# krispy-kenay/WebDGS

Measured on AMD Instinct MI355X. Metric: training iters/sec (fwd+bwd+Adam), 1M Gaussians @1080p SH3, higher is better.
Workload: dtype f32

## Files before the change

bindings/napi/webdgs_napi.cc:

```cpp
#include <node_api.h>

#include <cstdint>
#include <cstring>
#include <string>

#include "../../include/webdgs.h"

#define NAPI_OK(call)                                                         \
    do {                                                                      \
        if ((call) != napi_ok) {                                              \
            napi_throw_error(env, nullptr, "N-API call failed: " #call);      \
            return nullptr;                                                   \
        }                                                                     \
    } while (0)

static napi_value throw_wdgs(napi_env env, int code) {
    std::string msg = "[wdgs " + std::to_string(code) + "] " + wdgs_last_error();
    napi_throw_error(env, code == WDGS_E_CAPACITY ? "WDGS_E_CAPACITY" : (code == WDGS_E_STATE ? "WDGS_E_STATE" : "WDGS_E"), msg.c_str());
    return nullptr;
}
#define WDGS_OK_OR_THROW(expr)                      \
    do {                                            \
        int _rc = (expr);                           \
        if (_rc != WDGS_OK) return throw_wdgs(env, _rc); \
// ... 183 lines not shown
}
static napi_value tiledRasterizerDestroy(napi_env env, napi_callback_info info) { ARGS(1); wdgs_tiled_rasterizer_destroy((wdgs_tiled_rasterizer*)get_ptr(env, argv[0])); return js_undefined(env); }
static napi_value tiledBackwardCreate(napi_env env, napi_callback_info info) {
    ARGS(2);
    wdgs_tiled_backward_config c; std::memset(&c, 0, sizeof(c));
    c.num_points = (uint32_t)prop_f64(env, argv[1], "numPoints", 0);
    c.sh_deg = (uint32_t)prop_f64(env, argv[1], "shDeg", 0);
    c.viewport_width = (uint32_t)prop_f64(env, argv[1], "viewportWidth", 1);
    c.viewport_height = (uint32_t)prop_f64(env, argv[1], "viewportHeight", 1);
    c.training.lambda_l1 = (float)prop_f64(env, argv[1], "lambda_l1", 0.8);
    c.training.lambda_l2 = (float)prop_f64(env, argv[1], "lambda_l2", 0.0);
    c.training.lambda_dssim = (float)prop_f64(env, argv[1], "lambda_dssim", 0.2);
    c.training.c1 = (float)prop_f64(env, argv[1], "c1", 0.0001);
    c.training.c2 = (float)prop_f64(env, argv[1], "c2", 0.0009);
    c.max_splat_radius_px = (float)prop_f64(env, argv[1], "maxSplatRadiusPx", 128.0);
    uint32_t mode = 0;
    if (!prop_dssim_mode(env, argv[1], &mode)) return nullptr;
    wdgs_tiled_backward* op = nullptr;
    WDGS_OK_OR_THROW(wdgs_tiled_backward_create((wdgs_device*)get_ptr(env, argv[0]), &c, &op));
    const int r = wdgs_tiled_backward_set_dssim_mode(op, mode);
    if (r != WDGS_OK) { wdgs_tiled_backward_destroy(op); WDGS_OK_OR_THROW(r); }
    return make_ptr(env, op);
}
static napi_value tiledBackwardEncode(napi_env env, napi_callback_info info) {
    ARGS(5);
    wdgs_tiled_backward_resources r;
    r.splat_buffer = prop_ptr(env, argv[3], "splatBuffer");
    r.tile_offsets_buffer = prop_ptr(env, argv[3], "tileOffsetsBuffer");
    r.tile_indices_buffer = prop_ptr(env, argv[3], "tileIndicesBuffer");
    r.camera_buffer = prop_ptr(env, argv[3], "cameraBuffer");
    r.alpha_texture = prop_ptr(env, argv[3], "alphaTexture");
    r.n_contrib_texture = prop_ptr(env, argv[3], "nContribTexture");
    WDGS_OK_OR_THROW(wdgs_tiled_backward_encode((wdgs_tiled_backward*)get_ptr(env, argv[0]), get_ptr(env, argv[1]), get_ptr(env, argv[2]), &r, get_ptr(env, argv[4])));
    return js_undefined(env);
}
static napi_value tiledBackwardGradients(napi_env env, napi_callback_info info) { ARGS(1); return make_ptr(env, wdgs_tiled_backward_gradients((wdgs_tiled_backward*)get_ptr(env, argv[0]))); }
static napi_value tiledBackwardDestroy(napi_env env, napi_callback_info info) { ARGS(1); wdgs_tiled_backward_destroy((wdgs_tiled_backward*)get_ptr(env, argv[0])); return js_undefined(env); }
static napi_value optimizerCreate(napi_env env, napi_callback_info info) {
    ARGS(4);
    wdgs_optimizer* op = nullptr;
    WDGS_OK_OR_THROW(wdgs_optimizer_create((wdgs_device*)get_ptr(env, argv[0]), get_u32(env, argv[1]), nullptr, get_ptr(env, argv[2]), get_ptr(env, argv[3]), nullptr, 1, 0, &op));
    return make_ptr(env, op);
}
static napi_value optimizerStep(napi_env env, napi_callback_info info) {
    ARGS(5);
    WDGS_OK_OR_THROW(wdgs_optimizer_step((wdgs_optimizer*)get_ptr(env, argv[0]), get_ptr(env, argv[1]), get_ptr(env, argv[2]), get_ptr(env, argv[3]), get_ptr(env, argv[4])));
    return js_undefined(env);
}
static napi_value optimizerGetIteration(napi_env env, napi_callback_info info) { ARGS(1); return make_u32(env, wdgs_optimizer_get_iteration((wdgs_optimizer*)get_ptr(env, argv[0]))); }
static napi_value optimizerDestroy(napi_env env, napi_callback_info info) { ARGS(1); wdgs_optimizer_destroy((wdgs_optimizer*)get_ptr(env, argv[0])); return js_undefined(env); }

static napi_value tiledForwardSet(napi_env env, napi_callback_info info) {
    ARGS(3);
    wdgs_tiled_forward* op = (wdgs_tiled_forward*)get_ptr(env, argv[0]);
    switch (get_u32(env, argv[1])) {
        case 0: WDGS_OK_OR_THROW(wdgs_tiled_forward_set_render_mode(op, get_u32(env, argv[2]))); break;
        case 1: WDGS_OK_OR_THROW(wdgs_tiled_forward_set_point_size(op, (float)get_f64(env, argv[2]))); break;
        default: WDGS_OK_OR_THROW(wdgs_tiled_forward_set_gaussian_scale(op, (float)get_f64(env, argv[2]))); break;
    }
    return js_undefined(env);
}
static napi_value tiledForwardCheck(napi_env env, napi_callback_info info) {
    ARGS(1);
    uint32_t st[4] = {0, 0, 0, 0};
    WDGS_OK_OR_THROW(wdgs_tiled_forward_check((wdgs_tiled_forward*)get_ptr(env, argv[0]), st));
    napi_value o; napi_create_object(env, &o);
    set_prop(env, o, "totalTileEntries", make_u32(env, st[0]));
    set_prop(env, o, "visibleCount", make_u32(env, st[1]));
    return o;
}
static napi_value tiledForwardSetLongLists(napi_env env, napi_callback_info info) {
    ARGS(4);
    WDGS_OK_OR_THROW(wdgs_tiled_forward_set_long_lists((wdgs_tiled_forward*)get_ptr(env, argv[0]), get_u32(env, argv[1]), get_u32(env, argv[2]), get_u32(env, argv[3])));
    return js_undefined(env);
}
static napi_value tiledForwardLongListStats(napi_env env, napi_callback_info info) {
    ARGS(1);
    uint32_t st[12] = {0};
    WDGS_OK_OR_THROW(wdgs_tiled_forward_long_list_stats((wdgs_tiled_forward*)get_ptr(env, argv[0]), st));
    static const char* const keys[12] = {"blocksWanted", "itemsWanted", "forwardQueue", "backwardQueue", "rowsUsed", "rowsWanted", "stalled", nullptr, "maxItems", "maxBlocks", "maxRows", "threshold"};
    napi_value o; napi_create_object(env, &o);
    for (int i = 0; i < 12; i++) if (keys[i]) set_prop(env, o, keys[i], make_u32(env, st[i]));
    return o;
}
static napi_value tiledRasterizerBlit(napi_env env, napi_callback_info info) {
    ARGS(4);
    WDGS_OK_OR_THROW(wdgs_tiled_rasterizer_blit((wdgs_tiled_rasterizer*)get_ptr(env, argv[0]), get_ptr(env, argv[1]), get_u32(env, argv[2]), get_u32(env, argv[3])));
    return js_undefined(env);
}
static napi_value tiledRasterizerEncodeDepth(napi_env env, napi_callback_info info) {
    ARGS(2);
    WDGS_OK_OR_THROW(wdgs_tiled_rasterizer_encode_depth((wdgs_tiled_rasterizer*)get_ptr(env, argv[0]), get_u32(env, argv[1])));
    return js_undefined(env);
}
static napi_value tiledRasterizerGetDepth(napi_env env, napi_callback_info info) {
    ARGS(2);
    void* p = nullptr;
    WDGS_OK_OR_THROW(wdgs_tiled_rasterizer_get_depth((wdgs_tiled_rasterizer*)get_ptr(env, argv[0]), get_u32(env, argv[1]), &p));
    return make_ptr(env, p);
}
static napi_value depthToRgba8(napi_env env, napi_callback_info info) {
    ARGS(7);
    WDGS_OK_OR_THROW(wdgs_depth_to_rgba8((wdgs_device*)get_ptr(env, argv[0]), get_ptr(env, argv[1]), get_u32(env, argv[2]), get_u32(env, argv[3]), (float)get_f64(env, argv[4]),
                                         (float)get_f64(env, argv[5]), get_ptr(env, argv[6])));
    return js_undefined(env);
}
static napi_value bufferClear(napi_env env, napi_callback_info info) {
    ARGS(3);
    WDGS_OK_OR_THROW(wdgs_memset((wdgs_device*)get_ptr(env, argv[0]), get_ptr(env, argv[1]), 0, (size_t)get_f64(env, argv[2])));
    return js_undefined(env);
}
static napi_value encoderBegin(napi_env env, napi_callback_info info) { ARGS(1); WDGS_OK_OR_THROW(wdgs_encoder_begin((wdgs_device*)get_ptr(env, argv[0]))); return js_undefined(env); }
static napi_value encoderFinish(napi_env env, napi_callback_info info) {
    ARGS(1);
    wdgs_command_buffer* c = nullptr;
    WDGS_OK_OR_THROW(wdgs_encoder_finish((wdgs_device*)get_ptr(env, argv[0]), &c));
    return make_ptr(env, c);
}
static napi_value queueSubmit(napi_env env, napi_callback_info info) {
    ARGS(2);
    WDGS_OK_OR_THROW(wdgs_queue_submit((wdgs_device*)get_ptr(env, argv[0]), (wdgs_command_buffer*)get_ptr(env, argv[1])));
    return js_undefined(env);
}
static napi_value commandBufferDestroy(napi_env env, napi_callback_info info) { ARGS(1); wdgs_command_buffer_destroy((wdgs_command_buffer*)get_ptr(env, argv[0])); return js_undefined(env); }

struct DoneCtx { napi_deferred deferred; napi_threadsafe_function tsfn; };
static void done_call_js(napi_env env, napi_value, void* context, void*) {
    DoneCtx* c = static_cast<DoneCtx*>(context);
    if (env) { napi_value u; napi_get_undefined(env, &u); napi_resolve_deferred(env, c->deferred, u); }
    napi_release_threadsafe_function(c->tsfn, napi_tsfn_release);
    delete c;
}
static void done_from_runtime_thread(void* user) {
    DoneCtx* c = static_cast<DoneCtx*>(user);
    napi_call_threadsafe_function(c->tsfn, nullptr, napi_tsfn_blocking);
}
static napi_value queueOnSubmittedWorkDone(napi_env env, napi_callback_info info) {
    ARGS(1);
    DoneCtx* c = new DoneCtx();
    napi_value promise, name;
    NAPI_OK(napi_create_promise(env, &c->deferred, &promise));
    napi_create_string_utf8(env, "wdgs onSubmittedWorkDone", NAPI_AUTO_LENGTH, &name);
    NAPI_OK(napi_create_threadsafe_function(env, nullptr, nullptr, name, 0, 1, nullptr, nullptr, c, done_call_js, &c->tsfn));
    int rc = wdgs_queue_on_done((wdgs_device*)get_ptr(env, argv[0]), done_from_runtime_thread, c);
    if (rc != WDGS_OK) { napi_release_threadsafe_function(c->tsfn, napi_tsfn_abort); delete c; return throw_wdgs(env, rc); }
    return promise;
}

static void read_backward_resources(napi_env env, napi_value o, wdgs_tiled_backward_resources* r) {
    r->splat_buffer = prop_ptr(env, o, "splatBuffer");
    r->tile_offsets_buffer = prop_ptr(env, o, "tileOffsetsBuffer");
    r->tile_indices_buffer = prop_ptr(env, o, "tileIndicesBuffer");
    r->camera_buffer = prop_ptr(env, o, "cameraBuffer");
    r->alpha_texture = prop_ptr(env, o, "alphaTexture");
    r->n_contrib_texture = prop_ptr(env, o, "nContribTexture");
}
static napi_value tiledBackwardMetric(napi_env env, napi_callback_info info) {
    ARGS(5);
    wdgs_tiled_backward* op = (wdgs_tiled_backward*)get_ptr(env, argv[0]);
    switch (get_u32(env, argv[1])) {
        case 0: WDGS_OK_OR_THROW(wdgs_tiled_backward_compute_loss_only(op, get_ptr(env, argv[2]), get_ptr(env, argv[3]))); break;
        case 1: WDGS_OK_OR_THROW(wdgs_tiled_backward_compute_metric_map(op, get_ptr(env, argv[2]), get_ptr(env, argv[3]), (float)get_f64(env, argv[4]))); break;
        case 2: {
            wdgs_tiled_backward_resources r;
            read_backward_resources(env, argv[2], &r);
            WDGS_OK_OR_THROW(wdgs_tiled_backward_compute_metric_counts(op, &r, get_u32(env, argv[3]), (int)get_u32(env, argv[4])));
// ... 407 lines not shown
    uint32_t n = 0;
    napi_get_array_length(env, arr, &n);
    if (n > WDGS_MAX_BATCH_VIEWS) n = WDGS_MAX_BATCH_VIEWS + 1;
    for (uint32_t i = 0; i < n && i < WDGS_MAX_BATCH_VIEWS; i++) { napi_value v; napi_get_element(env, arr, i, &v); out[i] = get_ptr(env, v); }
    return n;
}
static napi_value tiledForwardProjectViews(napi_env env, napi_callback_info info) {
    ARGS(4);
    void* ops[WDGS_MAX_BATCH_VIEWS]; void* cams[WDGS_MAX_BATCH_VIEWS];
    const uint32_t n = read_ptr_array(env, argv[0], ops), m = read_ptr_array(env, argv[1], cams);
    if (n != m || n == 0 || n > WDGS_MAX_BATCH_VIEWS) { napi_throw_range_error(env, nullptr, "projectViews: 1..16 passes and as many cameras"); return nullptr; }
    WDGS_OK_OR_THROW(wdgs_tiled_forward_project_views((wdgs_tiled_forward* const*)ops, (const void* const*)cams, n, get_ptr(env, argv[2]), get_ptr(env, argv[3])));
    return js_undefined(env);
}
static napi_value tiledForwardEncodeProjected(napi_env env, napi_callback_info info) { ARGS(1); WDGS_OK_OR_THROW(wdgs_tiled_forward_encode_projected((wdgs_tiled_forward*)get_ptr(env, argv[0]))); return js_undefined(env); }
static napi_value tiledForwardIsProjected(napi_env env, napi_callback_info info) { ARGS(1); return make_u32(env, (uint32_t)wdgs_tiled_forward_is_projected((const wdgs_tiled_forward*)get_ptr(env, argv[0]))); }
static napi_value tiledBackwardGeometryViews(napi_env env, napi_callback_info info) {
    ARGS(10);
    void* ops[WDGS_MAX_BATCH_VIEWS]; void* cams[WDGS_MAX_BATCH_VIEWS]; void* counts[WDGS_MAX_BATCH_VIEWS]; void* words[WDGS_MAX_BATCH_VIEWS];
    const uint32_t n = read_ptr_array(env, argv[0], ops);
    if (n == 0 || n > WDGS_MAX_BATCH_VIEWS || read_ptr_array(env, argv[1], cams) != n || read_ptr_array(env, argv[2], counts) != n || read_ptr_array(env, argv[3], words) != n) {
        napi_throw_range_error(env, nullptr, "geometryViews: 1..16 passes and as many cameras, tile counts and overflow words");
        return nullptr;
    }
    WDGS_OK_OR_THROW(wdgs_tiled_backward_encode_geometry_views((wdgs_tiled_backward* const*)ops, (const void* const*)cams, (const void* const*)counts, (const void* const*)words, n,
                                                               get_ptr(env, argv[4]), get_ptr(env, argv[5]), get_ptr(env, argv[6]), get_ptr(env, argv[7]),
                                                               (int)get_u32(env, argv[8]), (int)get_u32(env, argv[9])));
    return js_undefined(env);
}
static napi_value deviceLaneMark(napi_env env, napi_callback_info info) {
    ARGS(3);
    WDGS_OK_OR_THROW(wdgs_device_lane_mark((wdgs_device*)get_ptr(env, argv[0]), (int)get_u32(env, argv[1]), (int)get_u32(env, argv[2])));
    return js_undefined(env);
}
static napi_value deviceLaneWaitMark(napi_env env, napi_callback_info info) {
    ARGS(3);
    WDGS_OK_OR_THROW(wdgs_device_lane_wait_mark((wdgs_device*)get_ptr(env, argv[0]), (int)get_u32(env, argv[1]), (int)get_u32(env, argv[2])));
    return js_undefined(env);
}
static napi_value deviceKernelTimes(napi_env env, napi_callback_info info) {
    ARGS(2);
    wdgs_device* d = (wdgs_device*)get_ptr(env, argv[0]);
    const uint32_t op = get_u32(env, argv[1]);
    if (op <= 1) { WDGS_OK_OR_THROW(wdgs_device_set_profiling(d, (int)op)); return js_undefined(env); }
    if (op == 2) { WDGS_OK_OR_THROW(wdgs_device_reset_kernel_times(d)); return js_undefined(env); }
    static wdgs_kernel_time recs[128];
    uint32_t n = 0;
    WDGS_OK_OR_THROW(wdgs_device_get_kernel_times(d, recs, 128, &n));
    napi_value o; napi_create_object(env, &o);
    for (uint32_t i = 0; i < n && i < 128; i++) {
        napi_value r, ms; napi_create_object(env, &r);
        set_prop(env, r, "launches", make_u32(env, recs[i].launches));
        napi_create_double(env, recs[i].total_ms, &ms); set_prop(env, r, "totalMs", ms);
        char name[49]; std::memcpy(name, recs[i].name, 48); name[48] = 0;
        set_prop(env, o, name, r);
    }
    return o;
}
static napi_value copyBufferToBuffer(napi_env env, napi_callback_info info) {
    ARGS(4);
    WDGS_OK_OR_THROW(wdgs_copy_buffer_to_buffer((wdgs_device*)get_ptr(env, argv[0]), get_ptr(env, argv[1]), get_ptr(env, argv[2]), (size_t)get_f64(env, argv[3])));
    return js_undefined(env);
}
static napi_value commGroup(napi_env env, napi_callback_info info) {
    ARGS(1);
    if (get_u32(env, argv[0])) WDGS_OK_OR_THROW(wdgs_comm_group_end()); else WDGS_OK_OR_THROW(wdgs_comm_group_start());
    return js_undefined(env);
}

#define EXPORT_FN(name)                                                              \
    do {                                                                             \
        napi_value fn;                                                               \
        napi_create_function(env, #name, NAPI_AUTO_LENGTH, name, nullptr, &fn);      \
        napi_set_named_property(env, exports, #name, fn);                            \
    } while (0)

static napi_value Init(napi_env env, napi_value exports) {
    EXPORT_FN(abiVersion); EXPORT_FN(deviceCreate); EXPORT_FN(deviceDestroy); EXPORT_FN(deviceSynchronize); EXPORT_FN(deviceMemoryInfo);
    EXPORT_FN(bufferCreate); EXPORT_FN(bufferDestroy); EXPORT_FN(copyToDevice); EXPORT_FN(copyToHost);
    EXPORT_FN(tiledForwardCreate); EXPORT_FN(tiledForwardEncode); EXPORT_FN(tiledForwardSetViewport); EXPORT_FN(tiledForwardGetResources); EXPORT_FN(tiledForwardDestroy);
    EXPORT_FN(tiledRasterizerCreate); EXPORT_FN(tiledRasterizerEncode); EXPORT_FN(tiledRasterizerGet); EXPORT_FN(tiledRasterizerDestroy);
    EXPORT_FN(tiledBackwardCreate); EXPORT_FN(tiledBackwardEncode); EXPORT_FN(tiledBackwardGradients); EXPORT_FN(tiledBackwardDestroy);
    EXPORT_FN(optimizerCreate); EXPORT_FN(optimizerStep); EXPORT_FN(optimizerGetIteration); EXPORT_FN(optimizerDestroy);
    EXPORT_FN(tiledForwardSet); EXPORT_FN(tiledForwardCheck); EXPORT_FN(tiledForwardSetLongLists); EXPORT_FN(tiledForwardLongListStats); EXPORT_FN(tiledRasterizerBlit); EXPORT_FN(bufferClear);
    EXPORT_FN(tiledRasterizerEncodeDepth); EXPORT_FN(tiledRasterizerGetDepth); EXPORT_FN(depthToRgba8);
    EXPORT_FN(encoderBegin); EXPORT_FN(encoderFinish); EXPORT_FN(queueSubmit); EXPORT_FN(commandBufferDestroy); EXPORT_FN(queueOnSubmittedWorkDone);
    EXPORT_FN(tiledBackwardMetric); EXPORT_FN(tiledBackwardGet); EXPORT_FN(downsampleRGBA8); EXPORT_FN(imageSSE); EXPORT_FN(imageSSIM);
    EXPORT_FN(optimizerStateSizes); EXPORT_FN(optimizerCreateWithState); EXPORT_FN(optimizerState); EXPORT_FN(optimizerHyperparameters);
    EXPORT_FN(optimizerAdvanceIteration); EXPORT_FN(optimizerStepF32); EXPORT_FN(accumulateGradients);
    EXPORT_FN(densifyCreate); EXPORT_FN(densifySetConfig); EXPORT_FN(densifyEncodePrepare); EXPORT_FN(densifyReadTotal); EXPORT_FN(densifyEncodeScatter);
    EXPORT_FN(densifyStage);
    EXPORT_FN(densifyDestroy);
    EXPORT_FN(commUniqueId); EXPORT_FN(commCreate); EXPORT_FN(commAllreduceGradients); EXPORT_FN(commAllreduceCounts); EXPORT_FN(commDestroy);
    EXPORT_FN(encoderAbort); EXPORT_FN(hostAlloc); EXPORT_FN(bufferReadAsync); EXPORT_FN(prefixScanner); EXPORT_FN(dynamicSorter);
    EXPORT_FN(optimizerDeferredSH); EXPORT_FN(optimizerFlushSH); EXPORT_FN(tiledForwardSetDcSource);
    EXPORT_FN(optimizerSetGuard); EXPORT_FN(optimizerStepF32Range); EXPORT_FN(optimizerStateChanged); EXPORT_FN(storeGradients); EXPORT_FN(guardAccumulate);
    EXPORT_FN(deviceSelectLane); EXPORT_FN(deviceLaneOrder); EXPORT_FN(queueMark); EXPORT_FN(queueWait); EXPORT_FN(tiledForwardResize); EXPORT_FN(tiledBackwardResize);
    EXPORT_FN(applyRepackedRows); EXPORT_FN(commExchangeGradients); EXPORT_FN(commAllgatherRows); EXPORT_FN(commBroadcast); EXPORT_FN(commInfo);
    EXPORT_FN(optimizerStepWithGeometry); EXPORT_FN(optimizerApplyRepackedRows); EXPORT_FN(tiledBackwardEncodeRaster); EXPORT_FN(tiledBackwardEncodeGeometry);
    EXPORT_FN(tiledBackwardSetGradientOutput); EXPORT_FN(tiledBackwardSetMetricCountsTarget); EXPORT_FN(tiledForwardProjectViews); EXPORT_FN(tiledForwardEncodeProjected); EXPORT_FN(tiledForwardIsProjected);
    EXPORT_FN(tiledBackwardGeometryViews); EXPORT_FN(deviceLaneMark); EXPORT_FN(deviceLaneWaitMark); EXPORT_FN(deviceKernelTimes); EXPORT_FN(commGroup); EXPORT_FN(copyBufferToBuffer);
    return exports;
}
NAPI_MODULE(webdgs_napi, Init)
```

include/webdgs.h:

```cpp
#ifndef WEBDGS_H
#define WEBDGS_H

#include <stddef.h>
#include <stdint.h>

#ifdef __cplusplus
extern "C" {
#endif

#define WDGS_OK 0
#define WDGS_E_INVALID (-1)
#define WDGS_E_HIP (-2)
#define WDGS_E_CAPACITY (-3)
#define WDGS_E_STATE (-4)

typedef struct wdgs_device wdgs_device;
typedef struct wdgs_buffer wdgs_buffer;
typedef struct wdgs_prefix_scanner wdgs_prefix_scanner;
typedef struct wdgs_sorter wdgs_sorter;
typedef struct wdgs_tiled_forward wdgs_tiled_forward;
typedef struct wdgs_tiled_rasterizer wdgs_tiled_rasterizer;
typedef struct wdgs_tiled_backward wdgs_tiled_backward;
typedef struct wdgs_optimizer wdgs_optimizer;
typedef struct wdgs_densify_prune wdgs_densify_prune;
// ... 20 lines not shown
int wdgs_device_lane_order(wdgs_device* dev, int waiter_lane, int signal_lane);
int wdgs_device_lane_mark(wdgs_device* dev, int lane, int mark);
int wdgs_device_lane_wait_mark(wdgs_device* dev, int lane, int mark);

int wdgs_encoder_begin(wdgs_device* dev);
int wdgs_encoder_finish(wdgs_device* dev, wdgs_command_buffer** out);
int wdgs_encoder_abort(wdgs_device* dev);
int wdgs_queue_submit(wdgs_device* dev, wdgs_command_buffer* cmd);
int wdgs_command_buffer_destroy(wdgs_command_buffer* cmd);
typedef void (*wdgs_done_callback)(void* user);
int wdgs_queue_on_done(wdgs_device* dev, wdgs_done_callback fn, void* user);
#define WDGS_TICKET_RING 8
int wdgs_queue_mark(wdgs_device* dev, uint64_t* ticket);
int wdgs_queue_wait(wdgs_device* dev, uint64_t ticket);

int wdgs_copy_to_host(wdgs_device* dev, void* dst_host, const void* src_dev, size_t bytes);
int wdgs_copy_to_device(wdgs_device* dev, void* dst_dev, const void* src_host, size_t bytes);
int wdgs_memset(wdgs_device* dev, void* dst_dev, int value, size_t bytes);
int wdgs_copy_buffer_to_buffer(wdgs_device* dev, void* dst_dev, const void* src_dev, size_t bytes);

int wdgs_buffer_create(wdgs_device* dev, size_t bytes, wdgs_buffer** out);
int wdgs_buffer_destroy(wdgs_buffer* buf);
void* wdgs_buffer_ptr(const wdgs_buffer* buf);
size_t wdgs_buffer_size(const wdgs_buffer* buf);
int wdgs_buffer_write(wdgs_device* dev, wdgs_buffer* buf, size_t offset, const void* src_host, size_t bytes);
int wdgs_buffer_read(wdgs_device* dev, const wdgs_buffer* buf, size_t offset, void* dst_host, size_t bytes);
int wdgs_buffer_read_async(wdgs_device* dev, const wdgs_buffer* buf, size_t offset, void* dst_host, size_t bytes);
int wdgs_host_alloc(size_t bytes, void** out_host);
int wdgs_host_free(void* host);

int wdgs_prefix_scanner_create(wdgs_device* dev, uint32_t max_elements, wdgs_prefix_scanner** out);
int wdgs_prefix_scanner_destroy(wdgs_prefix_scanner* s);
void* wdgs_prefix_scanner_input(wdgs_prefix_scanner* s);
void* wdgs_prefix_scanner_output(wdgs_prefix_scanner* s);
int wdgs_prefix_scanner_set_count(wdgs_prefix_scanner* s, uint32_t count);
int wdgs_prefix_scanner_scan(wdgs_prefix_scanner* s);
int wdgs_prefix_scanner_scan_ptr(wdgs_prefix_scanner* s, const void* in_dev, void* out_dev, uint32_t count);

int wdgs_sorter_create(wdgs_device* dev, uint32_t max_capacity, const void* stats_dev, wdgs_sorter** out);
int wdgs_sorter_destroy(wdgs_sorter* s);
void* wdgs_sorter_keys(wdgs_sorter* s, int ping_pong_index);
void* wdgs_sorter_values(wdgs_sorter* s, int ping_pong_index);
int wdgs_sorter_sort(wdgs_sorter* s, uint32_t key_bits);
int wdgs_sorter_final_out_index(wdgs_sorter* s);
uint32_t wdgs_sorter_capacity(wdgs_sorter* s);

typedef struct wdgs_tiled_forward_config {
    uint32_t num_points;
    uint32_t sh_deg;
    uint32_t viewport_width;
    uint32_t viewport_height;
    float gaussian_scale;
    float point_size_px;
    float max_splat_radius_px;
    uint32_t render_mode;
    uint32_t max_tile_entries;
    uint32_t compat_caps;
} wdgs_tiled_forward_config;

typedef struct wdgs_tiled_forward_resources {
    void* splat_buffer;
    void* depths_buffer;
    void* tile_keys_buffer;
    void* tile_indices_buffer;
    void* tile_offsets_buffer;
    void* tile_counts_buffer;
    void* stats_buffer;
    uint32_t num_tiles_x, num_tiles_y, total_tiles, max_tile_entries;
    float settings[7];
} wdgs_tiled_forward_resources;

int wdgs_tiled_forward_create(wdgs_device* dev, const wdgs_tiled_forward_config* cfg, wdgs_tiled_forward** out);
int wdgs_tiled_forward_destroy(wdgs_tiled_forward* op);
int wdgs_tiled_forward_resize(wdgs_tiled_forward* op, uint32_t num_points);
int wdgs_tiled_forward_encode(wdgs_tiled_forward* op, const void* gaussians_dev, const void* sh_dev, const void* camera_dev, int skip_sort);
int wdgs_tiled_forward_set_viewport(wdgs_tiled_forward* op, uint32_t width, uint32_t height);
int wdgs_tiled_forward_set_render_mode(wdgs_tiled_forward* op, uint32_t render_mode);
int wdgs_tiled_forward_set_point_size(wdgs_tiled_forward* op, float point_size_px);
int wdgs_tiled_forward_set_gaussian_scale(wdgs_tiled_forward* op, float scale);
int wdgs_tiled_forward_get_resources(wdgs_tiled_forward* op, wdgs_tiled_forward_resources* out);
int wdgs_tiled_forward_check(wdgs_tiled_forward* op, uint32_t* stats_out);
int wdgs_tiled_forward_set_long_lists(wdgs_tiled_forward* op, uint32_t threshold, uint32_t max_items, uint32_t max_rows);
int wdgs_tiled_forward_long_list_stats(wdgs_tiled_forward* op, uint32_t stats_out[12]);

int wdgs_tiled_rasterizer_create(wdgs_device* dev, wdgs_tiled_forward* forward, uint32_t compat_caps, wdgs_tiled_rasterizer** out);
int wdgs_tiled_rasterizer_destroy(wdgs_tiled_rasterizer* op);
int wdgs_tiled_rasterizer_encode(wdgs_tiled_rasterizer* op, uint32_t width, uint32_t height);
int wdgs_tiled_rasterizer_get_output(wdgs_tiled_rasterizer* op, void** rgba8_dev);
int wdgs_tiled_rasterizer_get_alpha(wdgs_tiled_rasterizer* op, void** final_t_dev);
int wdgs_tiled_rasterizer_get_n_contrib(wdgs_tiled_rasterizer* op, void** n_contrib_dev);
int wdgs_tiled_rasterizer_get_tile_offsets(wdgs_tiled_rasterizer* op, void** ranges_dev);
int wdgs_tiled_rasterizer_blit(wdgs_tiled_rasterizer* op, void* target_rgba8_dev, uint32_t target_width, uint32_t target_height);

#define WDGS_DEPTH_EXPECTED   1u
#define WDGS_DEPTH_MEDIAN     2u
#define WDGS_DEPTH_WEIGHT_SUM 4u
int wdgs_tiled_rasterizer_encode_depth(wdgs_tiled_rasterizer* op, uint32_t kinds);
int wdgs_tiled_rasterizer_get_depth(wdgs_tiled_rasterizer* op, uint32_t kind, void** f32_dev);
int wdgs_depth_to_rgba8(wdgs_device* dev, const void* depth_f32_dev, uint32_t width, uint32_t height, float near_z, float far_z, void* rgba8_dev);

typedef struct wdgs_training_config {
    float lambda_l1, lambda_l2, lambda_dssim, c1, c2;
} wdgs_training_config;
typedef struct wdgs_tiled_backward_config {
    uint32_t num_points;
    uint32_t sh_deg;
    uint32_t viewport_width, viewport_height;
    wdgs_training_config training;
    float gaussian_scale, point_size_px, max_splat_radius_px;
} wdgs_tiled_backward_config;
typedef struct wdgs_tiled_backward_resources {
    const void* splat_buffer;
    const void* tile_offsets_buffer;
    const void* tile_indices_buffer;
    const void* camera_buffer;
    const void* alpha_texture;
    const void* n_contrib_texture;
} wdgs_tiled_backward_resources;

int wdgs_tiled_backward_create(wdgs_device* dev, const wdgs_tiled_backward_config* cfg, wdgs_tiled_backward** out);
int wdgs_tiled_backward_resize(wdgs_tiled_backward* op, uint32_t num_points);
int wdgs_tiled_backward_destroy(wdgs_tiled_backward* op);
int wdgs_tiled_backward_encode(wdgs_tiled_backward* op, const void* predicted_rgba8_dev, const void* target_rgba8_dev,
                               const wdgs_tiled_backward_resources* res, const void* gaussians_dev);
typedef struct wdgs_view_accumulate {
    void* sums;
    void* visible;
    const void* tile_counts;
    void* guard;
    const void* overflow_word;
    int first;
} wdgs_view_accumulate;
int wdgs_tiled_backward_encode_raster(wdgs_tiled_backward* op, const void* predicted_rgba8_dev, const void* target_rgba8_dev,
                                      const wdgs_tiled_backward_resources* res);
int wdgs_tiled_backward_encode_geometry(wdgs_tiled_backward* op, const void* camera_dev, const void* gaussians_dev, const wdgs_view_accumulate* into);
int wdgs_tiled_backward_compute_loss_only(wdgs_tiled_backward* op, const void* predicted_rgba8_dev, const void* target_rgba8_dev);
int wdgs_tiled_backward_compute_metric_map(wdgs_tiled_backward* op, const void* predicted_rgba8_dev, const void* target_rgba8_dev, float threshold);
int wdgs_tiled_backward_compute_metric_counts(wdgs_tiled_backward* op, const wdgs_tiled_backward_resources* res, uint32_t num_instances, int clear);
int wdgs_tiled_backward_normalize_metric_counts(wdgs_tiled_backward* op, uint32_t divisor);
int wdgs_tiled_backward_set_viewport(wdgs_tiled_backward* op, uint32_t width, uint32_t height);
int wdgs_tiled_backward_set_training_config(wdgs_tiled_backward* op, const wdgs_training_config* cfg);
#define WDGS_DSSIM_REFERENCE 0
#define WDGS_DSSIM_GAUSSIAN 1
int wdgs_tiled_backward_set_dssim_mode(wdgs_tiled_backward* op, uint32_t mode);
int wdgs_tiled_backward_get_dssim_mode(const wdgs_tiled_backward* op, uint32_t* out);
void* wdgs_tiled_backward_gradients(wdgs_tiled_backward* op);
void* wdgs_tiled_backward_metric_counts(wdgs_tiled_backward* op);
int wdgs_tiled_backward_set_metric_counts_target(wdgs_tiled_backward* op, void* counts_dev);
void* wdgs_tiled_backward_loss_image(wdgs_tiled_backward* op);
void* wdgs_tiled_backward_metric_map(wdgs_tiled_backward* op);
int wdgs_tiled_backward_set_gradient_output(wdgs_tiled_backward* op, int enabled);
void* wdgs_tiled_backward_accumulators(wdgs_tiled_backward* op);
void* wdgs_tiled_backward_metric_minmax(wdgs_tiled_backward* op);
int wdgs_downsample_rgba8(wdgs_device* dev, const void* src_dev, uint32_t src_w, uint32_t src_h, void* dst_dev, uint32_t dst_w, uint32_t dst_h);

int wdgs_image_sse_rgb8(wdgs_device* dev, const void* a_rgba8_dev, const void* b_rgba8_dev, uint32_t num_pixels, void* out_u64_dev);

int wdgs_image_ssim_rgb8(wdgs_device* dev, const void* a_rgba8_dev, const void* b_rgba8_dev, uint32_t width, uint32_t height, void* out_f64_dev,
                         void* map_f32_dev);

int wdgs_debug_eval_math(wdgs_device* dev, uint32_t which, uint32_t count, const void* in_u32_dev, void* out_u32_dev);

int wdgs_debug_sort_tiles(wdgs_sorter* s, uint32_t route, uint32_t num_tiles_x, uint32_t num_tiles_y, void* ranges_u32_dev);

typedef struct wdgs_adam_hyperparameters {
    float lr_pos, lr_color, lr_opacity, lr_scale, lr_rot, beta1, beta2, epsilon;
// ... 103 lines not shown
```

webdgs_amd/_lib.py:

```python
from __future__ import annotations

import ctypes as C
import os

_HERE = os.path.dirname(os.path.abspath(__file__))
LIB_PATH = os.environ.get("WDGS_LIB_PATH") or os.path.join(_HERE, "lib", "libwebdgs_hip.so")

WDGS_OK, WDGS_E_INVALID, WDGS_E_HIP, WDGS_E_CAPACITY, WDGS_E_STATE = 0, -1, -2, -3, -4


class WdgsError(RuntimeError):

    def __init__(self, code: int, message: str):
        super().__init__(f"[wdgs {code}] {message}")
        self.code = code


class CapacityError(WdgsError):
    pass


class StateError(WdgsError):
    pass

# ... 77 lines not shown
    "wdgs_device_lane_order": (_I, [_P, _I, _I]),
    "wdgs_device_lane_mark": (_I, [_P, _I, _I]),
    "wdgs_device_lane_wait_mark": (_I, [_P, _I, _I]),
    "wdgs_encoder_begin": (_I, [_P]),
    "wdgs_encoder_finish": (_I, [_P, C.POINTER(_P)]),
    "wdgs_encoder_abort": (_I, [_P]),
    "wdgs_queue_submit": (_I, [_P, _P]),
    "wdgs_command_buffer_destroy": (_I, [_P]),
    "wdgs_queue_on_done": (_I, [_P, DoneCallback, _P]),
    "wdgs_buffer_read_async": (_I, [_P, _P, _Z, _P, _Z]),
    "wdgs_host_alloc": (_I, [_Z, C.POINTER(_P)]),
    "wdgs_host_free": (_I, [_P]),
    "wdgs_tiled_rasterizer_blit": (_I, [_P, _P, _U, _U]),
    "wdgs_densify_prune_encode_decision": (_I, [_P, _U, _P, _P]),
    "wdgs_densify_prune_encode_prefix_sum": (_I, [_P, _U]),
    "wdgs_densify_prune_encode_cap_to_max": (_I, [_P, _U, _U]),
    "wdgs_densify_prune_encode_total_out": (_I, [_P, _U]),
    "wdgs_densify_prune_compute_max_out_points": (_I, [_P, _U, C.POINTER(_U)]),
    "wdgs_densify_prune_get_buffers": (_I, [_P, C.POINTER(DensifyPrepared)]),
    "wdgs_debug_eval_math": (_I, [_P, _U, _U, _P, _P]),
    "wdgs_debug_sort_tiles": (_I, [_P, _U, _U, _U, _P]),
    "wdgs_comm_get_unique_id": (_I, [C.POINTER(C.c_uint8)]),
    "wdgs_comm_create": (_I, [_P, C.POINTER(C.c_uint8), _I, _I, C.POINTER(_P)]),
    "wdgs_comm_destroy": (_I, [_P]),
    "wdgs_comm_world_size": (_I, [_P]),
    "wdgs_comm_rank": (_I, [_P]),
    "wdgs_comm_allreduce_gradients": (_I, [_P, _P, _P, _U]),
    "wdgs_comm_allreduce_counts": (_I, [_P, _P, _U]),
    "wdgs_comm_exchange_gradients": (_I, [_P, _P, _P, _P, _U]),
    "wdgs_comm_allgather_rows": (_I, [_P, _P, _U]),
    "wdgs_comm_broadcast": (_I, [_P, _P, _Z, _I]),
    "wdgs_comm_group_start": (_I, []),
    "wdgs_comm_group_end": (_I, []),
    "wdgs_optimizer_step_f32_range": (_I, [_P, _P, _P, _P, _P, _U, _U, _P]),
    "wdgs_apply_repacked_rows": (_I, [_P, _U, _P, _U, _U, _P, _P, _P]),
    "wdgs_optimizer_set_guard": (_I, [_P, _P]),
    "wdgs_optimizer_set_deferred_sh": (_I, [_P, _P, _I]),
    "wdgs_optimizer_dc_words": (_P, [_P]),
    "wdgs_optimizer_flush_sh": (_I, [_P, _P]),
    "wdgs_optimizer_apply_repacked_rows": (_I, [_P, _P, _U, _U, _P, _P, _P]),
    "wdgs_tiled_forward_set_dc_source": (_I, [_P, _P]),
    "wdgs_tiled_forward_project_views": (_I, [_P, _P, _U, _P, _P]),
    "wdgs_tiled_forward_encode_projected": (_I, [_P]),
    "wdgs_tiled_forward_is_projected": (_I, [_P]),
    "wdgs_tiled_backward_encode_geometry_views": (_I, [_P, _P, _P, _P, _U, _P, _P, _P, _P, _I, _I]),
    "wdgs_guard_accumulate": (_I, [_P, _P, _P, _I]),
    "wdgs_optimizer_state_changed": (_I, [_P]),
    "wdgs_copy_to_host": (_I, [_P, _P, _P, _Z]),
    "wdgs_copy_to_device": (_I, [_P, _P, _P, _Z]),
    "wdgs_memset": (_I, [_P, _P, _I, _Z]),
    "wdgs_copy_buffer_to_buffer": (_I, [_P, _P, _P, _Z]),
    "wdgs_buffer_create": (_I, [_P, _Z, C.POINTER(_P)]),
    "wdgs_buffer_destroy": (_I, [_P]),
    "wdgs_buffer_ptr": (_P, [_P]),
    "wdgs_buffer_size": (_Z, [_P]),
    "wdgs_buffer_write": (_I, [_P, _P, _Z, _P, _Z]),
    "wdgs_buffer_read": (_I, [_P, _P, _Z, _P, _Z]),
    "wdgs_prefix_scanner_create": (_I, [_P, _U, C.POINTER(_P)]),
    "wdgs_prefix_scanner_destroy": (_I, [_P]),
    "wdgs_prefix_scanner_input": (_P, [_P]),
    "wdgs_prefix_scanner_output": (_P, [_P]),
    "wdgs_prefix_scanner_set_count": (_I, [_P, _U]),
    "wdgs_prefix_scanner_scan": (_I, [_P]),
    "wdgs_prefix_scanner_scan_ptr": (_I, [_P, _P, _P, _U]),
    "wdgs_sorter_create": (_I, [_P, _U, _P, C.POINTER(_P)]),
    "wdgs_sorter_destroy": (_I, [_P]),
    "wdgs_sorter_keys": (_P, [_P, _I]),
    "wdgs_sorter_values": (_P, [_P, _I]),
    "wdgs_sorter_sort": (_I, [_P, _U]),
    "wdgs_sorter_final_out_index": (_I, [_P]),
    "wdgs_sorter_capacity": (_U, [_P]),
    "wdgs_tiled_forward_create": (_I, [_P, C.POINTER(TiledForwardConfig), C.POINTER(_P)]),
    "wdgs_tiled_forward_destroy": (_I, [_P]),
    "wdgs_tiled_forward_resize": (_I, [_P, _U]),
    "wdgs_tiled_forward_encode": (_I, [_P, _P, _P, _P, _I]),
    "wdgs_tiled_forward_set_viewport": (_I, [_P, _U, _U]),
    "wdgs_tiled_forward_set_render_mode": (_I, [_P, _U]),
    "wdgs_tiled_forward_set_point_size": (_I, [_P, _F]),
    "wdgs_tiled_forward_set_gaussian_scale": (_I, [_P, _F]),
    "wdgs_tiled_forward_get_resources": (_I, [_P, C.POINTER(TiledForwardResources)]),
    "wdgs_tiled_forward_check": (_I, [_P, C.POINTER(_U)]),
    "wdgs_tiled_forward_set_long_lists": (_I, [_P, _U, _U, _U]),
    "wdgs_tiled_forward_long_list_stats": (_I, [_P, C.POINTER(_U)]),
    "wdgs_tiled_rasterizer_create": (_I, [_P, _P, _U, C.POINTER(_P)]),
    "wdgs_tiled_rasterizer_destroy": (_I, [_P]),
    "wdgs_tiled_rasterizer_encode": (_I, [_P, _U, _U]),
    "wdgs_tiled_rasterizer_get_output": (_I, [_P, C.POINTER(_P)]),
    "wdgs_tiled_rasterizer_get_alpha": (_I, [_P, C.POINTER(_P)]),
    "wdgs_tiled_rasterizer_get_n_contrib": (_I, [_P, C.POINTER(_P)]),
    "wdgs_tiled_rasterizer_get_tile_offsets": (_I, [_P, C.POINTER(_P)]),
    "wdgs_tiled_rasterizer_encode_depth": (_I, [_P, _U]),
    "wdgs_tiled_rasterizer_get_depth": (_I, [_P, _U, C.POINTER(_P)]),
    "wdgs_depth_to_rgba8": (_I, [_P, _P, _U, _U, _F, _F, _P]),
    "wdgs_tiled_backward_create": (_I, [_P, C.POINTER(TiledBackwardConfig), C.POINTER(_P)]),
    "wdgs_tiled_backward_resize": (_I, [_P, _U]),
    "wdgs_tiled_backward_destroy": (_I, [_P]),
    "wdgs_tiled_backward_encode": (_I, [_P, _P, _P, C.POINTER(TiledBackwardResources), _P]),
    "wdgs_tiled_backward_encode_raster": (_I, [_P, _P, _P, C.POINTER(TiledBackwardResources)]),
    "wdgs_tiled_backward_encode_geometry": (_I, [_P, _P, _P, C.POINTER(ViewAccumulate)]),
    "wdgs_tiled_backward_compute_loss_only": (_I, [_P, _P, _P]),
    "wdgs_tiled_backward_compute_metric_map": (_I, [_P, _P, _P, _F]),
    "wdgs_tiled_backward_compute_metric_counts": (_I, [_P, C.POINTER(TiledBackwardResources), _U, _I]),
    "wdgs_tiled_backward_normalize_metric_counts": (_I, [_P, _U]),
    "wdgs_tiled_backward_set_viewport": (_I, [_P, _U, _U]),
    "wdgs_tiled_backward_set_training_config": (_I, [_P, C.POINTER(TrainingConfig)]),
    "wdgs_tiled_backward_set_dssim_mode": (_I, [_P, _U]),
    "wdgs_tiled_backward_get_dssim_mode": (_I, [_P, C.POINTER(_U)]),
    "wdgs_tiled_backward_gradients": (_P, [_P]),
    "wdgs_tiled_backward_metric_counts": (_P, [_P]),
    "wdgs_tiled_backward_set_metric_counts_target": (_I, [_P, _P]),
    "wdgs_tiled_backward_loss_image": (_P, [_P]),
    "wdgs_tiled_backward_metric_map": (_P, [_P]),
    "wdgs_tiled_backward_accumulators": (_P, [_P]),
    "wdgs_tiled_backward_set_gradient_output": (_I, [_P, _I]),
    "wdgs_tiled_backward_metric_minmax": (_P, [_P]),
    "wdgs_downsample_rgba8": (_I, [_P, _P, _U, _U, _P, _U, _U]),
    "wdgs_image_sse_rgb8": (_I, [_P, _P, _P, _U, _P]),
    "wdgs_image_ssim_rgb8": (_I, [_P, _P, _P, _U, _U, _P, _P]),
    "wdgs_optimizer_state_sizes": (_I, [_U, C.POINTER(_Z * 6)]),
    "wdgs_optimizer_create": (_I, [_P, _U, C.POINTER(AdamHyperparameters), _P, _P, C.POINTER(OptimizerState), _I, _U, C.POINTER(_P)]),
    "wdgs_optimizer_destroy": (_I, [_P]),
    "wdgs_optimizer_init_from_point_cloud": (_I, [_P, _P, _P]),
    "wdgs_optimizer_step": (_I, [_P, _P, _P, _P, _P]),
    "wdgs_optimizer_step_with_geometry": (_I, [_P, _P, _P, _P, _P, _P]),
    "wdgs_optimizer_step_f32": (_I, [_P, _P, _P, _P, _P]),
    "wdgs_accumulate_gradients": (_I, [_P, _U, _P, _P, _P, _P]),
    "wdgs_store_gradients": (_I, [_P, _U, _P, _P, _P, _P]),
    "wdgs_optimizer_get_iteration": (_U, [_P]),
    "wdgs_optimizer_advance_iteration": (_I, [_P, _U]),
    "wdgs_optimizer_get_hyperparameters": (_I, [_P, C.POINTER(AdamHyperparameters)]),
    "wdgs_optimizer_set_hyperparameters": (_I, [_P, C.POINTER(AdamHyperparameters)]),
    "wdgs_optimizer_get_state": (_I, [_P, C.POINTER(OptimizerState)]),
    "wdgs_optimizer_release_state": (_I, [_P, C.POINTER(OptimizerState)]),
    "wdgs_densify_prune_create": (_I, [_P, C.POINTER(DensifyConfig), C.POINTER(_P)]),
    "wdgs_densify_prune_destroy": (_I, [_P]),
    "wdgs_densify_prune_set_config": (_I, [_P, C.POINTER(DensifyConfig)]),
    "wdgs_densify_prune_ensure_size": (_I, [_P, _U]),
    "wdgs_densify_prune_encode_prepare": (_I, [_P, _U, _P, _P, C.POINTER(DensifyPrepared)]),
    "wdgs_densify_prune_read_total": (_I, [_P, C.POINTER(_U)]),
    "wdgs_densify_prune_encode_scatter": (_I, [_P, _U, _P, _P, C.POINTER(OptimizerState), _U, _I, _P, _P, C.POINTER(OptimizerState)]),
}

_lib = None


def load() -> C.CDLL:
    global _lib
    if _lib is not None:
        return _lib
    if not os.path.exists(LIB_PATH):
        raise ImportError(f"{LIB_PATH} is missing: build it with `python -c 'import __graft_entry__ as g; g.build()'` "
                          "or `make -C webdgs_amd/csrc` (hipcc --offload-arch=gfx950). There is no CPU fallback.")
    lib = C.CDLL(LIB_PATH)
    for name, (res, args) in SIGNATURES.items():
        fn = getattr(lib, name)
        fn.restype = res
        fn.argtypes = args
    _lib = lib
    return lib


def check(code: int) -> None:
    if code == WDGS_OK:
        return
    msg = load().wdgs_last_error().decode("utf-8", "replace")
    if code == WDGS_E_CAPACITY:
# ... 5 lines not shown
```

webdgs_amd/csrc/api.hip:

```cpp
#include <cstdarg>
#include <cstdio>
#include <cstdlib>
#include <cstring>
#include <algorithm>
#include <mutex>
#include <map>
#include <set>
#include <unordered_map>
#include <vector>

#include "common.h"
#include "alloc_cache.h"
#include "longlist.h"

int launch_project_count(wdgs_device*, u32, const void*, const void*, const void*, const RenderSettings&, const TileInfo&, void*, void*, void*, void*, void*, void*,
                         const void*, void*, const void*);
int launch_emit_scatter(wdgs_device*, u32, const void*, const void*, const void*, void*, const void*, const RenderSettings&, const TileInfo&, const void*, const void*, void*, void*, u32);
int sorter_sort_rows(wdgs_sorter* s, u32 num_tiles_x, u32 num_tiles_y, u32* ranges, const LongWork* lw);
extern "C" void sorter_set_final_out_index(wdgs_sorter* s, int i);
int launch_update_stats(wdgs_device*, u32, const void*, const void*, u32, void*, void*, void*);
int launch_emit(wdgs_device*, u32, const void*, const void*, const void*, void*, const void*, const RenderSettings&, const TileInfo&, void*, void*, u32);
int launch_tile_ranges(wdgs_device*, const void*, const void*, u32, void*);
int launch_depth_composite(wdgs_device*, const RenderSettings&, const TileInfo&, const void*, u32, const void*, const void*, const void*, const void*, const void*, u32,
                           void*, void*, void*, const void*, const void*);
// ... 62 lines not shown
        if (cur != device && hipSetDevice(device) != hipSuccess) return nullptr;
        void* p = nullptr;
        const hipError_t e = hipMalloc(&p, bytes);
        if (cur != device) (void)hipSetDevice(cur);
        if (e != hipSuccess) { (void)hipGetLastError(); return nullptr; }
        return p;
    }
    void free(void* p) { (void)hipFree(p); }
    bool sync(int device) {
        int cur = 0;
        if (hipGetDevice(&cur) != hipSuccess) return false;
        if (cur != device && hipSetDevice(device) != hipSuccess) return false;
        const hipError_t e = hipDeviceSynchronize();
        if (cur != device) (void)hipSetDevice(cur);
        return e == hipSuccess;
    }
};
wdgs::AllocCache<HipBackend> g_alloc_cache;
size_t g_cache_limit = 0;
std::mutex g_cache_limit_mutex;
bool alloc_cache_enabled() {
    static const bool on = !(std::getenv("WDGS_ALLOC_CACHE") && std::getenv("WDGS_ALLOC_CACHE")[0] == '0');
    return on;
}
}

int wdgs_alloc(void** p, size_t bytes, bool zero, hipStream_t stream) {
    *p = nullptr;
    if (bytes == 0) bytes = 16;
    if (!alloc_cache_enabled()) {
        WDGS_CHECK_HIP(hipMalloc(p, bytes));
    } else {
        int device = 0;
        WDGS_CHECK_HIP(hipGetDevice(&device));
        hipStreamCaptureStatus capture = hipStreamCaptureStatusNone;
        const bool recording = stream && hipStreamIsCapturing(stream, &capture) == hipSuccess && capture != hipStreamCaptureStatusNone;
        *p = g_alloc_cache.alloc(device, bytes, !recording);
        WDGS_REQUIRE(*p, WDGS_E_HIP, "device allocation of %zu bytes failed (device %d)", bytes, device);
    }
    if (zero) WDGS_CHECK_HIP(hipMemsetAsync(*p, 0, bytes, stream));
    return WDGS_OK;
}

void wdgs_free(void* p) {
    if (!p) return;
    if (alloc_cache_enabled()) {
        size_t limit;
        {
            std::lock_guard<std::mutex> lock(g_cache_limit_mutex);
            if (g_cache_limit == 0) {
                size_t free_b = 0, total_b = 0;
                g_cache_limit = (hipMemGetInfo(&free_b, &total_b) == hipSuccess && total_b) ? total_b / 4 : ((size_t)8 << 30);
            }
            limit = g_cache_limit;
        }
        if (g_alloc_cache.free(p, limit)) return;
    }
    (void)hipFree(p);
}
static void free_dev(void* p) { wdgs_free(p); }

struct wdgs_buffer {
    void* ptr;
    size_t size;
};

struct wdgs_prefix_scanner {
    wdgs_device* dev;
    u32 max_elements, count;
    u32 *input, *output;
    ScanScratch scratch;
};

struct wdgs_tiled_forward {
    wdgs_device* dev;
    wdgs_tiled_forward_config cfg;
    RenderSettings settings;
    TileInfo tile_info;
    u32* stats;
    u32* nf_stamp;
    u32 nf_capacity;
    LongWork long_lists;
    u32 long_flags_capacity;
    u32* host_stats;
    u32* splats;
    u32* depths;
    u32* block_counts;
    u32* column_counts;
    u32* column_totals;
    const void* dc_source;
    u32 points_capacity;
    wdgs_prefix_scanner* scanner;
    wdgs_sorter* sorter;
    u32* ranges;
    u32 ranges_capacity;
    bool ranges_valid;
    bool encoded;
    bool projected;
    bool projected_columns;
};

constexpr u32 FRAME_WORD = 4u + 64u;
constexpr size_t FORWARD_STATS_BYTES = 16 + 64 * 4 + 16;

struct wdgs_tiled_rasterizer {
    wdgs_device* dev;
    wdgs_tiled_forward* fwd;
    u32 compat_caps;
    u32 width, height;
    u32 ranges_capacity;
    u32* ranges;
    u32* ranges_used;
    u32* rgba8;
    float* alpha;
    u32* n_contrib;
    bool encoded;
    float* depth[3];
    u32 depth_width, depth_height;
    u32 depth_encoded;
};

struct wdgs_tiled_backward {
    wdgs_device* dev;
    wdgs_tiled_backward_config cfg;
    RenderSettings settings;
    int* acc;
    u32* acc_dirty;
    u32* gradients;
    bool gradient_output;
    float* loss_image;
    u32 dssim_mode;
    u32* metric_counts;
    u32* metric_counts_into;
    u32* metric_err;
    u32* metric_flags;
    u32* metric_minmax;
    u32 img_capacity;
    u32 points_capacity;
};

struct wdgs_optimizer {
    wdgs_device* dev;
    u32 num_points;
    wdgs_adam_hyperparameters params;
    wdgs_optimizer_state state;
    bool owns_state;
    u32 iteration;
    float* dc;
    static u32 cs_pitch(u32 n) { return (std::max(n, 1u) + 15u) & ~15u; }
    CsView cs() const { return CsView{reinterpret_cast<float4*>(dc), cs_pitch(num_points)}; }
    bool dc_dirty;
    const void* guard;
    u32* dc_words;
    bool deferred_sh;
    bool sh_stale;
};

static int optimizer_flush_dc(wdgs_optimizer* op) {
    if (!op->dc_dirty) return WDGS_OK;
    WDGS_TRY(launch_cs_flush(op->dev, op->num_points, op->cs(), op->state));
    op->dc_dirty = false;
    return WDGS_OK;
}

extern "C" {

// ... 137 lines not shown
}

int wdgs_queue_wait(wdgs_device* d, uint64_t ticket) {
    WDGS_REQUIRE(d, WDGS_E_INVALID, "wdgs_queue_wait: null device");
    WDGS_REQUIRE(ticket != 0 && ticket < d->ticket_next, WDGS_E_INVALID, "wdgs_queue_wait: ticket %llu was never issued", (unsigned long long)ticket);
    WDGS_REQUIRE(!d->capturing, WDGS_E_STATE, "wdgs_queue_wait while recording a command buffer");
    WDGS_CHECK_HIP(hipEventSynchronize(d->ticket_events[ticket % WDGS_TICKET_RING]));
    if (!d->pending.empty()) collect_profile(d);
    return deferred_checks(d);
}

int wdgs_device_memory_info(wdgs_device* d, size_t* free_bytes, size_t* total_bytes, size_t* cached_bytes) {
    WDGS_REQUIRE(d, WDGS_E_INVALID, "wdgs_device_memory_info: null device");
    size_t f = 0, t = 0;
    WDGS_CHECK_HIP(hipSetDevice(d->ordinal));
    WDGS_CHECK_HIP(hipMemGetInfo(&f, &t));
    if (free_bytes) *free_bytes = f;
    if (total_bytes) *total_bytes = t;
    if (cached_bytes) *cached_bytes = g_alloc_cache.held(d->ordinal);
    return WDGS_OK;
}
static void reap_command_buffers(wdgs_device* d, size_t at_most);
int wdgs_device_destroy(wdgs_device* d) {
    if (!d) return WDGS_OK;
    {
        std::lock_guard<std::mutex> lock(g_live_mutex);
        if (!g_live_devices.erase(d)) return WDGS_OK;
    }
    (void)hipSetDevice(d->ordinal);
    if (d->capturing) {
        hipGraph_t g = nullptr;
        (void)hipStreamEndCapture(d->stream, &g);
        if (g) (void)hipGraphDestroy(g);
        d->capturing = false;
    }
    (void)wdgs_sync_lanes(d);
    collect_profile(d);
    reap_command_buffers(d, (size_t)-1);
    g_alloc_cache.release(d->ordinal);
    for (hipEvent_t e : d->event_pool) (void)hipEventDestroy(e);
    for (hipEvent_t e : d->lane_events) if (e) (void)hipEventDestroy(e);
    for (hipEvent_t e : d->lane_marks) if (e) (void)hipEventDestroy(e);
    for (hipEvent_t e : d->ticket_events) if (e) (void)hipEventDestroy(e);
    if (d->host_guard) (void)hipHostFree(d->host_guard);
    if (d->ssim_partials) (void)hipFree(d->ssim_partials);
    for (int l = 1; l < WDGS_MAX_LANES; l++)
        if (d->lanes[l]) (void)hipStreamDestroy(d->lanes[l]);
    if (d->own_stream) (void)hipStreamDestroy(d->lanes[0]);
    delete d;
    return WDGS_OK;
}

int wdgs_device_set_profiling(wdgs_device* d, int enabled) {
    WDGS_REQUIRE(d, WDGS_E_INVALID, "null device");
    d->profiling = enabled != 0;
    return WDGS_OK;
}

int wdgs_device_get_kernel_times(wdgs_device* d, wdgs_kernel_time* out, uint32_t cap, uint32_t* count) {
    WDGS_REQUIRE(d && count, WDGS_E_INVALID, "null argument");
    if (!d->pending.empty() && !d->capturing) collect_profile(d);
    u32 i = 0;
    for (auto& kv : d->totals) {
        if (out && i < cap) {
            std::memset(&out[i], 0, sizeof(out[i]));
            std::strncpy(out[i].name, kv.first.c_str(), sizeof(out[i].name) - 1);
            out[i].launches = kv.second.launches;
            out[i].total_ms = kv.second.ms;
        }
        i++;
    }
    *count = i;
    return WDGS_OK;
}

int wdgs_device_reset_kernel_times(wdgs_device* d) {
    WDGS_REQUIRE(d, WDGS_E_INVALID, "null device");
    d->totals.clear();
    return WDGS_OK;
}

static bool forward_holds_projection(const wdgs_tiled_forward* f);
static void forward_consume_projection(wdgs_tiled_forward* f);
struct wdgs_command_buffer_impl { hipGraph_t graph; hipGraphExec_t exec; std::vector<wdgs_tiled_forward*> consumes; wdgs_device* dev; };
static void command_buffer_release(wdgs_command_buffer_impl* c) {
    (void)hipGraphExecDestroy(c->exec);
    (void)hipGraphDestroy(c->graph);
    delete c;
}
static void reap_command_buffers(wdgs_device* d, size_t at_most) {
    while (at_most-- && !d->dead_command_buffers.empty()) {
        command_buffer_release(static_cast<wdgs_command_buffer_impl*>(d->dead_command_buffers.back()));
        d->dead_command_buffers.pop_back();
    }
}

int wdgs_encoder_begin(wdgs_device* d) {
    WDGS_REQUIRE(d, WDGS_E_INVALID, "null device");
    WDGS_REQUIRE(!d->capturing, WDGS_E_STATE, "wdgs_encoder_begin: a recording is already open on this device");
    WDGS_CHECK_HIP(hipStreamBeginCapture(d->stream, hipStreamCaptureModeRelaxed));
    d->capturing = true;
    d->capture_consumes.clear();
    return WDGS_OK;
}
int wdgs_encoder_finish(wdgs_device* d, wdgs_command_buffer** out) {
    WDGS_REQUIRE(d && out, WDGS_E_INVALID, "null argument");
    WDGS_REQUIRE(d->capturing, WDGS_E_STATE, "wdgs_encoder_finish without wdgs_encoder_begin");
    d->capturing = false;
    hipGraph_t graph = nullptr;
    WDGS_CHECK_HIP(hipStreamEndCapture(d->stream, &graph));
    hipGraphExec_t exec = nullptr;
    hipError_t e = hipGraphInstantiate(&exec, graph, nullptr, nullptr, 0);
    if (e != hipSuccess) { (void)hipGraphDestroy(graph); d->capture_consumes.clear(); wdgs_set_error("hipGraphInstantiate failed: %s", hipGetErrorString(e)); return WDGS_E_HIP; }
    auto* c = new wdgs_command_buffer_impl{graph, exec, std::move(d->capture_consumes), d};
    d->capture_consumes.clear();
    *out = reinterpret_cast<wdgs_command_buffer*>(c);
    return WDGS_OK;
}
int wdgs_encoder_abort(wdgs_device* d) {
    WDGS_REQUIRE(d, WDGS_E_INVALID, "null device");
    if (!d->capturing) return WDGS_OK;
    d->capturing = false;
    d->capture_consumes.clear();
    hipGraph_t graph = nullptr;
    const hipError_t e = hipStreamEndCapture(d->stream, &graph);
    if (graph) (void)hipGraphDestroy(graph);
    (void)hipGetLastError();
    (void)e;
    return WDGS_OK;
}
int wdgs_queue_submit(wdgs_device* d, wdgs_command_buffer* cmd) {
    WDGS_REQUIRE(d && cmd, WDGS_E_INVALID, "null argument");
    WDGS_REQUIRE(!d->capturing, WDGS_E_STATE, "wdgs_queue_submit while recording");
    auto* c = reinterpret_cast<wdgs_command_buffer_impl*>(cmd);
    for (wdgs_tiled_forward* f : c->consumes) {
        WDGS_REQUIRE(std::find(d->forwards.begin(), d->forwards.end(), f) != d->forwards.end(), WDGS_E_STATE,
                     "wdgs_queue_submit: the command buffer was recorded against a forward pass that has been destroyed");
        WDGS_REQUIRE(forward_holds_projection(f), WDGS_E_STATE,
                     "wdgs_queue_submit: the command buffer starts at the scan of a projected forward pass (wdgs_tiled_forward_encode_projected), but the pass holds no "
                     "projection: run wdgs_tiled_forward_project_views before every submit, and no other encode of the pass in between");
    }
    WDGS_CHECK_HIP(hipGraphLaunch(c->exec, d->stream));
    for (wdgs_tiled_forward* f : c->consumes) forward_consume_projection(f);
    reap_command_buffers(d, 1);
    return WDGS_OK;
}
namespace {
struct DoneThunk { wdgs_done_callback fn; void* user; };
void done_trampoline(void* p) {
    DoneThunk* t = static_cast<DoneThunk*>(p);
    t->fn(t->user);
    delete t;
}
}
int wdgs_queue_on_done(wdgs_device* d, wdgs_done_callback fn, void* user) {
    WDGS_REQUIRE(d && fn, WDGS_E_INVALID, "wdgs_queue_on_done: null argument");
    WDGS_REQUIRE(!d->capturing, WDGS_E_STATE, "wdgs_queue_on_done while recording a command buffer");
    DoneThunk* t = new DoneThunk{fn, user};
    hipError_t e = hipLaunchHostFunc(d->stream, done_trampoline, t);
    if (e != hipSuccess) { delete t; wdgs_set_error("hipLaunchHostFunc failed: %s", hipGetErrorString(e)); return WDGS_E_HIP; }
    return WDGS_OK;
}
int wdgs_command_buffer_destroy(wdgs_command_buffer* cmd) {
    if (!cmd) return WDGS_OK;
    auto* c = reinterpret_cast<wdgs_command_buffer_impl*>(cmd);
    static const bool lazy = !(std::getenv("WDGS_LAZY_GRAPH_DESTROY") && std::getenv("WDGS_LAZY_GRAPH_DESTROY")[0] == '0');
    if (lazy && wdgs_device_alive(c->dev)) {
        c->dev->dead_command_buffers.push_back(c);
        if (c->dev->dead_command_buffers.size() > 64u) reap_command_buffers(c->dev, 32u);
    } else command_buffer_release(c);
    return WDGS_OK;
}

int wdgs_copy_to_host(wdgs_device* d, void* dst, const void* src, size_t bytes) {
    WDGS_REQUIRE(d && (bytes == 0 || (dst && src)), WDGS_E_INVALID, "wdgs_copy_to_host: null argument");
    WDGS_REQUIRE(!d->capturing, WDGS_E_STATE, "wdgs_copy_to_host while recording a command buffer");
    if (bytes == 0) return WDGS_OK;
    WDGS_CHECK_HIP(hipMemcpyAsync(dst, src, bytes, hipMemcpyDeviceToHost, d->stream));
    WDGS_CHECK_HIP(wdgs_sync_lanes(d));
    return WDGS_OK;
}

int wdgs_copy_to_device(wdgs_device* d, void* dst, const void* src, size_t bytes) {
    WDGS_REQUIRE(d && (bytes == 0 || (dst && src)), WDGS_E_INVALID, "wdgs_copy_to_device: null argument");
    WDGS_REQUIRE(!d->capturing, WDGS_E_STATE, "wdgs_copy_to_device while recording a command buffer");
    if (bytes == 0) return WDGS_OK;
    WDGS_CHECK_HIP(hipMemcpyAsync(dst, src, bytes, hipMemcpyHostToDevice, d->stream));
    return WDGS_OK;
}

int wdgs_memset(wdgs_device* d, void* dst, int value, size_t bytes) {
    WDGS_REQUIRE(d && (bytes == 0 || dst), WDGS_E_INVALID, "wdgs_memset: null argument");
    if (bytes == 0) return WDGS_OK;
    WDGS_CHECK_HIP(hipMemsetAsync(dst, value, bytes, d->stream));
    return WDGS_OK;
}

int wdgs_copy_buffer_to_buffer(wdgs_device* d, void* dst, const void* src, size_t bytes) {
    WDGS_REQUIRE(d && (bytes == 0 || (dst && src)), WDGS_E_INVALID, "wdgs_copy_buffer_to_buffer: null argument");
    if (bytes == 0) return WDGS_OK;
    WDGS_CHECK_HIP(hipMemcpyAsync(dst, src, bytes, hipMemcpyDeviceToDevice, d->stream));
    return WDGS_OK;
}

int wdgs_buffer_create(wdgs_device* d, size_t bytes, wdgs_buffer** out) {
    WDGS_REQUIRE(d && out, WDGS_E_INVALID, "wdgs_buffer_create: null argument");
    wdgs_buffer* b = new wdgs_buffer{nullptr, bytes};
    int r = wdgs_alloc(&b->ptr, bytes, true, d->stream);
    if (r != WDGS_OK) { delete b; return r; }
    *out = b;
    return WDGS_OK;
}
int wdgs_buffer_destroy(wdgs_buffer* b) {
    if (!b) return WDGS_OK;
    free_dev(b->ptr);
    delete b;
    return WDGS_OK;
}
void* wdgs_buffer_ptr(const wdgs_buffer* b) { return b ? b->ptr : nullptr; }
size_t wdgs_buffer_size(const wdgs_buffer* b) { return b ? b->size : 0; }
int wdgs_buffer_write(wdgs_device* d, wdgs_buffer* b, size_t off, const void* src, size_t bytes) {
    WDGS_REQUIRE(d && b, WDGS_E_INVALID, "wdgs_buffer_write: null argument");
    WDGS_REQUIRE(off + bytes <= b->size, WDGS_E_INVALID, "wdgs_buffer_write: range [%zu, %zu) exceeds buffer size %zu", off, off + bytes, b->size);
    return wdgs_copy_to_device(d, (char*)b->ptr + off, src, bytes);
// ... 24 lines not shown
int wdgs_prefix_scanner_create(wdgs_device* d, uint32_t max_elements, wdgs_prefix_scanner** out) {
    WDGS_REQUIRE(d && out, WDGS_E_INVALID, "wdgs_prefix_scanner_create: null argument");
    wdgs_prefix_scanner* s = new wdgs_prefix_scanner();
    s->dev = d;
    s->max_elements = max_elements > 0 ? max_elements : 1;
    s->count = s->max_elements;
    s->input = s->output = nullptr;
    int r = wdgs_alloc((void**)&s->input, sizeof(u32) * (size_t)s->max_elements, true, d->stream);
    if (r == WDGS_OK) r = wdgs_alloc((void**)&s->output, sizeof(u32) * (size_t)s->max_elements, true, d->stream);
    if (r == WDGS_OK) r = scan_scratch_create(&s->scratch, s->max_elements);
    if (r != WDGS_OK) { wdgs_prefix_scanner_destroy(s); return r; }
    *out = s;
    return WDGS_OK;
}
int wdgs_prefix_scanner_destroy(wdgs_prefix_scanner* s) {
    if (!s) return WDGS_OK;
    free_dev(s->input);
    free_dev(s->output);
    scan_scratch_destroy(&s->scratch);
    delete s;
    return WDGS_OK;
}
void* wdgs_prefix_scanner_input(wdgs_prefix_scanner* s) { return s ? s->input : nullptr; }
void* wdgs_prefix_scanner_output(wdgs_prefix_scanner* s) { return s ? s->output : nullptr; }
int wdgs_prefix_scanner_set_count(wdgs_prefix_scanner* s, uint32_t count) {
    WDGS_REQUIRE(s, WDGS_E_INVALID, "null scanner");
    WDGS_REQUIRE(count <= s->max_elements, WDGS_E_CAPACITY, "scan count %u exceeds max_elements %u", count, s->max_elements);
    s->count = count;
    return WDGS_OK;
}
int wdgs_prefix_scanner_scan(wdgs_prefix_scanner* s) {
    WDGS_REQUIRE(s, WDGS_E_INVALID, "null scanner");
    return scan_exclusive_u32(s->dev, &s->scratch, s->input, s->output, s->count, nullptr);
}
int wdgs_prefix_scanner_scan_ptr(wdgs_prefix_scanner* s, const void* in, void* out, uint32_t count) {
    WDGS_REQUIRE(s && in && out, WDGS_E_INVALID, "null argument");
    WDGS_REQUIRE(count <= s->max_elements, WDGS_E_CAPACITY, "scan count %u exceeds max_elements %u", count, s->max_elements);
    return scan_exclusive_u32(s->dev, &s->scratch, (const u32*)in, (u32*)out, count, nullptr);
}

static uint64_t forward_tile_entry_cap(const wdgs_tiled_forward_config& cfg, u32 n) {
    uint64_t cap;
    if (cfg.compat_caps) {
        uint64_t base = std::min<uint64_t>((uint64_t)n * 30, (uint64_t)n * 2048);
        cap = std::min<uint64_t>(std::min<uint64_t>(base, 32ull * 1024 * 1024), 2097152ull);
        cap = (cap + 3839) / 3840 * 3840;
    } else if (cfg.max_tile_entries) {
        cap = cfg.max_tile_entries;
    } else {
        cap = std::max<uint64_t>((uint64_t)n * 30, 1ull << 20);
    }
    return std::min<uint64_t>(align_up(cap, 4096), 0xFFFFF000ull);
}
static int forward_alloc_per_point(wdgs_tiled_forward* op, u32 capacity) {
    wdgs_device* d = op->dev;
    int r = wdgs_alloc((void**)&op->splats, (size_t)24 * capacity, true, d->stream);
    if (r == WDGS_OK) r = wdgs_alloc((void**)&op->depths, (size_t)4 * capacity, true, d->stream);
    if (r == WDGS_OK) r = wdgs_alloc((void**)&op->block_counts, (size_t)4 * (ceil_div(capacity, 256) + 1), true, d->stream);
    if (r == WDGS_OK) r = wdgs_alloc((void**)&op->column_counts, (size_t)4 * 256 * (ceil_div(capacity, 256) + 1), true, d->stream);
    if (r == WDGS_OK && !op->column_totals) r = wdgs_alloc((void**)&op->column_totals, (size_t)4 * 256, true, d->stream);
    if (r == WDGS_OK) r = wdgs_prefix_scanner_create(d, capacity, &op->scanner);
    if (r == WDGS_OK) op->points_capacity = capacity;
    return r;
}
static void forward_set_viewport(wdgs_tiled_forward* op, u32 w, u32 h) {
    op->cfg.viewport_width = w;
    op->cfg.viewport_height = h;
    op->settings.viewport_x = (float)w;
    op->settings.viewport_y = (float)h;
    op->tile_info.num_tiles_x = ceil_div(w, 16);
    op->tile_info.num_tiles_y = ceil_div(h, 16);
    op->tile_info.total_tiles = op->tile_info.num_tiles_x * op->tile_info.num_tiles_y;
}
static int forward_alloc_nf_stamp(wdgs_tiled_forward* op) {
    if (op->tile_info.total_tiles <= op->nf_capacity) return WDGS_OK;
    free_dev(op->nf_stamp);
    op->nf_stamp = nullptr;
    op->nf_capacity = 0;
    WDGS_TRY(wdgs_alloc((void**)&op->nf_stamp, sizeof(u32) * (size_t)op->tile_info.total_tiles, true, op->dev->stream));
    op->nf_capacity = op->tile_info.total_tiles;
    return WDGS_OK;
}

static void forward_free_long_lists(wdgs_tiled_forward* op) {
    LongWork& lw = op->long_lists;
    free_dev(lw.hdr);
    free_dev(lw.flags);
    lw = LongWork{};
    op->long_flags_capacity = 0;
}
static int forward_alloc_long_lists(wdgs_tiled_forward* op, u32 threshold, u32 items, u32 rows) {
    wdgs_device* d = op->dev;
    forward_free_long_lists(op);
    if (threshold == 0u) return WDGS_OK;
    LongWork lw{};
    lw.threshold = threshold;
    lw.max_items = std::max(items, 64u);
    lw.max_blocks = std::max(lw.max_items / 8u, 16u) & ~3u;
    lw.max_rows = std::max(rows, 64u);
    const u32 tiles = std::max(op->tile_info.total_tiles, 1u);
    const size_t I = lw.max_items, B = lw.max_blocks, R = lw.max_rows;
    const size_t sizes[12] = {256, sizeof(LongBlock) * B, sizeof(LongSync) * B, sizeof(u32) * I, sizeof(u32) * I, sizeof(u32) * 64 * B, sizeof(u32) * 64 * B,
                              sizeof(u32) * 64 * I, sizeof(u32) * 64 * I, sizeof(float4) * 192 * I, sizeof(u32) * 256 * R, 0};
    size_t at[12], total = 0, zeroed = 0;
    for (int i = 0; i < 11; i++) { at[i] = total; total += align_up(sizes[i], 256); if (i == 6) zeroed = total; }
    char* base = nullptr;
    WDGS_TRY(wdgs_alloc((void**)&base, total, false, d->stream));
    if (hipMemsetAsync(base, 0, zeroed, d->stream) != hipSuccess) { free_dev(base); wdgs_set_error("hipMemsetAsync failed"); return WDGS_E_HIP; }
    lw.hdr = (u32*)(base + at[0]); lw.blocks = (LongBlock*)(base + at[1]); lw.sync = (LongSync*)(base + at[2]); lw.item_block = (u32*)(base + at[3]); lw.nlist = (u32*)(base + at[4]);
    lw.total = (u32*)(base + at[5]); lw.jlast = (u32*)(base + at[6]); lw.cnt = (u32*)(base + at[7]); lw.off = (u32*)(base + at[8]); lw.records = (float4*)(base + at[9]);
    lw.rows = (u32*)(base + at[10]);
    lw.nf_stamp = op->nf_stamp;
    lw.nf_frame = op->stats + FRAME_WORD;
    op->long_lists = lw;
    const int r = wdgs_alloc((void**)&op->long_lists.flags, sizeof(u32) * (size_t)tiles, true, d->stream);
    if (r != WDGS_OK) { forward_free_long_lists(op); return r; }
    op->long_flags_capacity = tiles;
    return WDGS_OK;
}
constexpr u32 LONG_LIST_THRESHOLD = 2048u, LONG_LIST_ITEMS = 1024u, LONG_LIST_ROWS = 8192u;

int wdgs_tiled_forward_create(wdgs_device* d, const wdgs_tiled_forward_config* cfg, wdgs_tiled_forward** out) {
    WDGS_REQUIRE(d && cfg && out, WDGS_E_INVALID, "wdgs_tiled_forward_create: null argument");
    WDGS_REQUIRE(cfg->viewport_width > 0 && cfg->viewport_height > 0, WDGS_E_INVALID, "viewport must be non-empty");
    WDGS_REQUIRE(cfg->sh_deg <= 3, WDGS_E_INVALID, "sh_deg %u > 3", cfg->sh_deg);
    const uint64_t tiles = (uint64_t)ceil_div(cfg->viewport_width, 16) * ceil_div(cfg->viewport_height, 16);
    WDGS_REQUIRE(tiles + 1 <= 0xFFFFu, WDGS_E_CAPACITY, "%llu tiles do not fit the 16-bit tile field of the sort key", (unsigned long long)tiles);
    wdgs_tiled_forward* op = new wdgs_tiled_forward();
    op->dev = d;
    op->cfg = *cfg;
    op->stats = op->splats = op->depths = op->block_counts = op->column_counts = op->column_totals = nullptr;
    op->dc_source = nullptr;
    op->nf_stamp = nullptr;
    op->nf_capacity = 0;
    op->long_lists = LongWork{};
    op->long_flags_capacity = 0;
    op->host_stats = nullptr;
    op->scanner = nullptr;
    op->sorter = nullptr;
    op->ranges = nullptr;
    op->ranges_capacity = 0;
    op->ranges_valid = false;
    op->encoded = false;
    op->projected = op->projected_columns = false;
    const u32 n = cfg->num_points;
    const uint64_t cap = forward_tile_entry_cap(*cfg, n);
    op->points_capacity = std::max(n, 1u);
    op->settings = RenderSettings{cfg->gaussian_scale != 0.f ? cfg->gaussian_scale : 1.0f, (float)cfg->sh_deg, 0.f, 0.f,
                                  cfg->point_size_px != 0.f ? cfg->point_size_px : 3.0f, cfg->render_mode ? 1.0f : 0.0f,
                                  cfg->max_splat_radius_px != 0.f ? cfg->max_splat_radius_px : 128.0f};
    op->tile_info.max_tile_entries = (u32)cap;
    forward_set_viewport(op, cfg->viewport_width, cfg->viewport_height);
    int r = wdgs_alloc((void**)&op->stats, FORWARD_STATS_BYTES, true, d->stream);
    if (r == WDGS_OK && hipMemsetD32Async((hipDeviceptr_t)(op->stats + FRAME_WORD), 1, 1, d->stream) != hipSuccess) { wdgs_set_error("hipMemsetD32Async failed"); r = WDGS_E_HIP; }
    if (r == WDGS_OK) r = forward_alloc_nf_stamp(op);
    if (r == WDGS_OK && !cfg->compat_caps) r = forward_alloc_long_lists(op, LONG_LIST_THRESHOLD, LONG_LIST_ITEMS, LONG_LIST_ROWS);
    if (r == WDGS_OK && hipHostMalloc((void**)&op->host_stats, 16, hipHostMallocDefault) != hipSuccess) { wdgs_set_error("hipHostMalloc(16) failed"); r = WDGS_E_HIP; }
    if (r == WDGS_OK) std::memset(op->host_stats, 0, 16);
    if (r == WDGS_OK) r = forward_alloc_per_point(op, std::max(n, 1u));
    if (r == WDGS_OK) r = wdgs_sorter_create(d, (u32)cap, op->stats, &op->sorter);
    if (r != WDGS_OK) { wdgs_tiled_forward_destroy(op); return r; }
    d->forwards.push_back(op);
    *out = op;
    return WDGS_OK;
}

int wdgs_tiled_forward_destroy(wdgs_tiled_forward* op) {
    if (!op) return WDGS_OK;
    if (wdgs_device_alive(op->dev)) {
        auto& v = op->dev->forwards;
        v.erase(std::remove(v.begin(), v.end(), op), v.end());
    }
    sync_if_alive(op->dev);
    if (op->ranges && wdgs_device_alive(op->dev)) op->dev->range_tables.erase(op->ranges);
    free_dev(op->stats);
    free_dev(op->nf_stamp);
    forward_free_long_lists(op);
    if (op->host_stats) (void)hipHostFree(op->host_stats);
    free_dev(op->splats);
    free_dev(op->depths);
    free_dev(op->block_counts);
    free_dev(op->column_counts);
    free_dev(op->column_totals);
    free_dev(op->ranges);
    wdgs_prefix_scanner_destroy(op->scanner);
    wdgs_sorter_destroy(op->sorter);
    delete op;
    return WDGS_OK;
}

int wdgs_tiled_forward_resize(wdgs_tiled_forward* op, uint32_t n) {
    WDGS_REQUIRE(op, WDGS_E_INVALID, "wdgs_tiled_forward_resize: null op");
    wdgs_device* d = op->dev;
    WDGS_REQUIRE(!d->capturing, WDGS_E_STATE, "wdgs_tiled_forward_resize while recording a command buffer");
    WDGS_CHECK_HIP(hipSetDevice(d->ordinal));
    WDGS_CHECK_HIP(wdgs_sync_lanes(d));
    const u32 need = std::max(n, 1u);
    if (need > op->points_capacity) {
        free_dev(op->splats); free_dev(op->depths); free_dev(op->block_counts); free_dev(op->column_counts);
        op->splats = op->depths = op->block_counts = op->column_counts = nullptr;
        wdgs_prefix_scanner_destroy(op->scanner);
        op->scanner = nullptr;
        op->points_capacity = 0;
        WDGS_TRY(forward_alloc_per_point(op, (u32)std::min<uint64_t>((uint64_t)need + need / 4, 0xFFFFFFFFull)));
    } else {
        WDGS_CHECK_HIP(hipMemsetAsync(op->splats, 0, (size_t)24 * need, d->stream));
        WDGS_CHECK_HIP(hipMemsetAsync(op->depths, 0, (size_t)4 * need, d->stream));
        WDGS_CHECK_HIP(hipMemsetAsync(op->block_counts, 0, (size_t)4 * (ceil_div(need, 256) + 1), d->stream));
        WDGS_CHECK_HIP(hipMemsetAsync(op->scanner->input, 0, (size_t)4 * need, d->stream));
        WDGS_CHECK_HIP(hipMemsetAsync(op->scanner->output, 0, (size_t)4 * need, d->stream));
    }
    const uint64_t cap = forward_tile_entry_cap(op->cfg, n);
    if (cap > wdgs_sorter_capacity(op->sorter)) {
        wdgs_sorter_destroy(op->sorter);
        op->sorter = nullptr;
        const uint64_t roomy = op->cfg.compat_caps || op->cfg.max_tile_entries ? cap : std::min<uint64_t>(align_up(cap + cap / 4, 4096), 0xFFFFF000ull);
        WDGS_TRY(wdgs_sorter_create(d, (u32)roomy, op->stats, &op->sorter));
    }
    op->tile_info.max_tile_entries = (u32)cap;
    op->cfg.num_points = n;
    WDGS_CHECK_HIP(hipMemsetAsync(op->stats, 0, 16 + 64 * 4, d->stream));
    std::memset(op->host_stats, 0, 16);
    op->encoded = false;
    op->ranges_valid = false;
    op->projected = false;
    return WDGS_OK;
}

static bool forward_uses_columns(const wdgs_tiled_forward* op, int skip_sort) {
    const TileInfo& ti = op->tile_info;
    return !skip_sort && !op->cfg.compat_caps && op->cfg.num_points > 0 && ti.num_tiles_x >= 2u && ti.num_tiles_x <= 256u && ti.num_tiles_y <= 256u;
}

static int forward_encode_rest(wdgs_tiled_forward* op, int skip_sort, bool columns) {
    wdgs_device* d = op->dev;
    const u32 n = op->cfg.num_points;
    const TileInfo& ti = op->tile_info;
    const ScanStatsEpilogue ep{op->stats, op->stats + 4, op->host_stats, op->tile_info.max_tile_entries, op->stats + FRAME_WORD, op->long_lists.hdr};
    if (columns) {
        WDGS_TRY(forward_scan(d, op->block_counts, ceil_div(n, 256), op->column_counts, op->column_totals, ti.num_tiles_x, ep));
    } else if (n > 0) {
        WDGS_TRY(scan_block_sums_inplace(d, op->block_counts, ceil_div(n, 256), ep));
    } else {
        WDGS_TRY(launch_update_stats(d, n, op->scanner->output, op->scanner->input, op->tile_info.max_tile_entries, op->stats, op->stats + 4, op->host_stats));
    }
    op->ranges_valid = false;
    if (!skip_sort && !op->cfg.compat_caps) {
        const u32 tiles = op->tile_info.total_tiles;
        if (tiles + 1 > op->ranges_capacity) {
            WDGS_REQUIRE(!d->capturing, WDGS_E_STATE, "TiledForwardPass.encode allocates its range table on first use: run one eager encode before recording");
            (void)wdgs_sync_lanes(d);
            if (op->ranges) d->range_tables.erase(op->ranges);
            free_dev(op->ranges);
            op->ranges = nullptr;
            WDGS_TRY(wdgs_alloc((void**)&op->ranges, sizeof(u32) * (size_t)(tiles + 1), true, d->stream));
            op->ranges_capacity = tiles + 1;
            d->range_tables[op->ranges] = op;
        }
    }
    if (columns) {
        WDGS_TRY(launch_emit_scatter(d, n, op->splats, op->depths, op->scanner->input, op->scanner->output, op->block_counts, op->settings, op->tile_info,
                                     op->column_counts, op->column_totals, wdgs_sorter_keys(op->sorter, 0), wdgs_sorter_values(op->sorter, 0), op->tile_info.max_tile_entries));
        WDGS_TRY(sorter_sort_rows(op->sorter, ti.num_tiles_x, ti.num_tiles_y, op->ranges, op->long_lists.hdr ? &op->long_lists : nullptr));
        op->ranges_valid = true;
    } else {
        WDGS_TRY(launch_emit(d, n, op->splats, op->depths, op->scanner->input, op->scanner->output, op->block_counts, op->settings, op->tile_info,
                             wdgs_sorter_keys(op->sorter, 0), wdgs_sorter_values(op->sorter, 0), op->tile_info.max_tile_entries));
        if (skip_sort) sorter_set_final_out_index(op->sorter, 0);
        if (!skip_sort) {
            if (op->cfg.compat_caps) {
                WDGS_TRY(wdgs_sorter_sort(op->sorter, 32u));
            } else {
                WDGS_TRY(sorter_sort_segmented(op->sorter, bits_for(op->tile_info.total_tiles), op->tile_info.total_tiles, op->ranges, op->long_lists.hdr ? &op->long_lists : nullptr));
                op->ranges_valid = true;
            }
        }
    }
    op->encoded = true;
    return WDGS_OK;
}

int wdgs_tiled_forward_encode(wdgs_tiled_forward* op, const void* gaussians, const void* sh, const void* camera, int skip_sort) {
    WDGS_REQUIRE(op && gaussians && sh && camera, WDGS_E_INVALID, "wdgs_tiled_forward_encode: null argument");
    wdgs_device* d = op->dev;
    const u32 n = op->cfg.num_points;
    const bool columns = forward_uses_columns(op, skip_sort);
    op->projected = false;
    WDGS_TRY(launch_project_count(d, n, gaussians, sh, camera, op->settings, op->tile_info, op->splats, op->depths, op->scanner->input, op->stats + 4,
                                  op->block_counts, columns ? op->column_counts : nullptr, op->dc_source, op->nf_stamp, op->stats + FRAME_WORD));
    return forward_encode_rest(op, skip_sort, columns);
}

int wdgs_tiled_forward_project_views(wdgs_tiled_forward* const* ops, const void* const* cameras, uint32_t count, const void* gaussians, const void* sh) {
    WDGS_REQUIRE(ops && cameras && gaussians && sh && count > 0 && count <= WDGS_MAX_BATCH_VIEWS, WDGS_E_INVALID, "wdgs_tiled_forward_project_views: invalid argument");
    wdgs_tiled_forward* f0 = ops[0];
    WDGS_REQUIRE(f0, WDGS_E_INVALID, "wdgs_tiled_forward_project_views: null pass");
    const bool columns = forward_uses_columns(f0, 0);
    void *splats[WDGS_MAX_BATCH_VIEWS], *depths[WDGS_MAX_BATCH_VIEWS], *counts[WDGS_MAX_BATCH_VIEWS], *shards[WDGS_MAX_BATCH_VIEWS], *blocks[WDGS_MAX_BATCH_VIEWS],
        *cols[WDGS_MAX_BATCH_VIEWS], *stamps[WDGS_MAX_BATCH_VIEWS];
    const void* frames[WDGS_MAX_BATCH_VIEWS];
    for (u32 v = 0; v < count; v++) {
        wdgs_tiled_forward* f = ops[v];
        WDGS_REQUIRE(f && cameras[v], WDGS_E_INVALID, "wdgs_tiled_forward_project_views: null pass or camera %u", v);
        for (u32 u = 0; u < v; u++) WDGS_REQUIRE(ops[u] != f, WDGS_E_INVALID, "wdgs_tiled_forward_project_views: pass %u is given twice (every view needs buffers of its own)", v);
        WDGS_REQUIRE(f->dev == f0->dev && f->cfg.num_points == f0->cfg.num_points && f->cfg.sh_deg == f0->cfg.sh_deg && f->cfg.compat_caps == f0->cfg.compat_caps &&
                         std::memcmp(&f->settings, &f0->settings, sizeof(RenderSettings)) == 0 && f->tile_info.num_tiles_x == f0->tile_info.num_tiles_x &&
                         f->tile_info.num_tiles_y == f0->tile_info.num_tiles_y && f->dc_source == f0->dc_source,
                     WDGS_E_STATE, "wdgs_tiled_forward_project_views: pass %u differs from pass 0 (cloud size, SH degree, viewport, settings or dc source)", v);
        splats[v] = f->splats; depths[v] = f->depths; counts[v] = f->scanner->input; shards[v] = f->stats + 4; blocks[v] = f->block_counts; cols[v] = f->column_counts;
        stamps[v] = f->nf_stamp; frames[v] = f->stats + FRAME_WORD;
    }
    WDGS_TRY(launch_project_count_views(f0->dev, f0->cfg.num_points, count, gaussians, sh, cameras, f0->settings, f0->tile_info, splats, depths, counts, shards, blocks,
                                        columns ? cols : nullptr, f0->dc_source, stamps, frames));
    for (u32 v = 0; v < count; v++) { ops[v]->projected = true; ops[v]->projected_columns = columns; }
    return WDGS_OK;
}
int wdgs_tiled_forward_encode_projected(wdgs_tiled_forward* op) {
    WDGS_REQUIRE(op, WDGS_E_INVALID, "wdgs_tiled_forward_encode_projected: null op");
    if (op->dev->capturing) {
        op->dev->capture_consumes.push_back(op);
        return forward_encode_rest(op, 0, forward_uses_columns(op, 0));
    }
    WDGS_REQUIRE(op->projected, WDGS_E_STATE,
                 "wdgs_tiled_forward_encode_projected: the pass holds no projection (wdgs_tiled_forward_project_views), or a later encode has consumed or overwritten it");
    op->projected = false;
    return forward_encode_rest(op, 0, op->projected_columns);
}
static bool forward_holds_projection(const wdgs_tiled_forward* f) { return f->projected; }
static void forward_consume_projection(wdgs_tiled_forward* f) { f->projected = false; }

int wdgs_tiled_forward_is_projected(const wdgs_tiled_forward* op) { return (op && op->projected) ? 1 : 0; }

int wdgs_tiled_forward_set_viewport(wdgs_tiled_forward* op, uint32_t w, uint32_t h) {
    WDGS_REQUIRE(op && w > 0 && h > 0, WDGS_E_INVALID, "wdgs_tiled_forward_set_viewport: invalid argument");
    WDGS_REQUIRE((uint64_t)ceil_div(w, 16) * ceil_div(h, 16) + 1 <= 0xFFFFu, WDGS_E_CAPACITY, "viewport %ux%u has too many tiles for the 16-bit tile field", w, h);
    WDGS_REQUIRE(!op->dev->capturing, WDGS_E_STATE, "wdgs_tiled_forward_set_viewport while recording a command buffer");
    forward_set_viewport(op, w, h);
    if (op->tile_info.total_tiles > op->nf_capacity) { (void)wdgs_sync_lanes(op->dev); WDGS_TRY(forward_alloc_nf_stamp(op)); op->long_lists.nf_stamp = op->long_lists.hdr ? op->nf_stamp : nullptr; }
    if (op->long_lists.hdr && op->tile_info.total_tiles > op->long_flags_capacity) {
        (void)wdgs_sync_lanes(op->dev);
        free_dev(op->long_lists.flags);
        op->long_lists.flags = nullptr;
        WDGS_TRY(wdgs_alloc((void**)&op->long_lists.flags, sizeof(u32) * (size_t)op->tile_info.total_tiles, true, op->dev->stream));
        op->long_flags_capacity = op->tile_info.total_tiles;
    }
    return WDGS_OK;
}
int wdgs_tiled_forward_set_render_mode(wdgs_tiled_forward* op, uint32_t mode) {
    WDGS_REQUIRE(op, WDGS_E_INVALID, "null op");
    op->cfg.render_mode = mode;
    op->settings.gaussian_mode = mode ? 1.0f : 0.0f;
    return WDGS_OK;
}
int wdgs_tiled_forward_set_point_size(wdgs_tiled_forward* op, float v) {
    WDGS_REQUIRE(op, WDGS_E_INVALID, "null op");
    op->settings.point_size_px = v;
    return WDGS_OK;
}
int wdgs_tiled_forward_set_gaussian_scale(wdgs_tiled_forward* op, float v) {
    WDGS_REQUIRE(op, WDGS_E_INVALID, "null op");
    op->settings.gaussian_scaling = v;
    return WDGS_OK;
}

int wdgs_tiled_forward_get_resources(wdgs_tiled_forward* op, wdgs_tiled_forward_resources* out) {
    WDGS_REQUIRE(op && out, WDGS_E_INVALID, "null argument");
    const int fo = wdgs_sorter_final_out_index(op->sorter);
    out->splat_buffer = op->splats;
    out->depths_buffer = op->depths;
    out->tile_keys_buffer = wdgs_sorter_keys(op->sorter, fo);
    out->tile_indices_buffer = wdgs_sorter_values(op->sorter, fo);
    out->tile_offsets_buffer = op->scanner->output;
    out->tile_counts_buffer = op->scanner->input;
    out->stats_buffer = op->stats;
    out->num_tiles_x = op->tile_info.num_tiles_x;
    out->num_tiles_y = op->tile_info.num_tiles_y;
    out->total_tiles = op->tile_info.total_tiles;
    out->max_tile_entries = op->tile_info.max_tile_entries;
    std::memcpy(out->settings, &op->settings, sizeof(float) * 7);
    return WDGS_OK;
}

int wdgs_tiled_forward_check(wdgs_tiled_forward* op, uint32_t* stats_out) {
    WDGS_REQUIRE(op, WDGS_E_INVALID, "null op");
    WDGS_REQUIRE(!op->dev->capturing, WDGS_E_STATE, "wdgs_tiled_forward_check while recording a command buffer");
    WDGS_CHECK_HIP(wdgs_sync_lanes(op->dev));
    u32 st[4];
    for (int i = 0; i < 4; i++) st[i] = ((const volatile u32*)op->host_stats)[i];
    st[2] = __atomic_exchange_n(op->host_stats + 2, 0u, __ATOMIC_ACQ_REL);
    if (stats_out) std::memcpy(stats_out, st, sizeof(st));
    WDGS_REQUIRE(st[2] == 0u, WDGS_E_CAPACITY, "tile entries overflow: %u entries needed, max_tile_entries = %u (forward pass %p)", st[2], op->tile_info.max_tile_entries, (void*)op);
    return WDGS_OK;
}

int wdgs_tiled_forward_set_long_lists(wdgs_tiled_forward* op, uint32_t threshold, uint32_t max_items, uint32_t max_rows) {
    WDGS_REQUIRE(op, WDGS_E_INVALID, "wdgs_tiled_forward_set_long_lists: null op");
    wdgs_device* d = op->dev;
    WDGS_REQUIRE(!d->capturing, WDGS_E_STATE, "wdgs_tiled_forward_set_long_lists while recording a command buffer");
    WDGS_REQUIRE(!op->cfg.compat_caps || threshold == 0u, WDGS_E_STATE, "wdgs_tiled_forward_set_long_lists: a pass with compat_caps truncates its lists as the reference does");
    WDGS_CHECK_HIP(hipSetDevice(d->ordinal));
    WDGS_CHECK_HIP(wdgs_sync_lanes(d));
    const LongWork& now = op->long_lists;
    return forward_alloc_long_lists(op, threshold, max_items ? max_items : (now.hdr ? now.max_items : LONG_LIST_ITEMS), max_rows ? max_rows : (now.hdr ? now.max_rows : LONG_LIST_ROWS));
}
int wdgs_tiled_forward_long_list_stats(wdgs_tiled_forward* op, uint32_t stats_out[12]) {
    WDGS_REQUIRE(op && stats_out, WDGS_E_INVALID, "wdgs_tiled_forward_long_list_stats: null argument");
    std::memset(stats_out, 0, sizeof(uint32_t) * 12);
    const LongWork& lw = op->long_lists;
    if (!lw.hdr) return WDGS_OK;
    WDGS_TRY(wdgs_copy_to_host(op->dev, stats_out, lw.hdr, sizeof(u32) * LL_HDR_WORDS));
    stats_out[8] = lw.max_items; stats_out[9] = lw.max_blocks; stats_out[10] = lw.max_rows; stats_out[11] = lw.threshold;
    return WDGS_OK;
}

int wdgs_tiled_rasterizer_create(wdgs_device* d, wdgs_tiled_forward* fwd, uint32_t compat_caps, wdgs_tiled_rasterizer** out) {
    WDGS_REQUIRE(d && fwd && out, WDGS_E_INVALID, "wdgs_tiled_rasterizer_create: null argument");
    wdgs_tiled_rasterizer* op = new wdgs_tiled_rasterizer();
    std::memset(op, 0, sizeof(*op));
    op->dev = d;
    op->fwd = fwd;
    op->compat_caps = compat_caps;
    *out = op;
    return WDGS_OK;
}
int wdgs_tiled_rasterizer_destroy(wdgs_tiled_rasterizer* op) {
    if (!op) return WDGS_OK;
    sync_if_alive(op->dev);
    free_dev(op->ranges);
    free_dev(op->rgba8);
    free_dev(op->alpha);
    free_dev(op->n_contrib);
    for (float* img : op->depth) free_dev(img);
    delete op;
    return WDGS_OK;
}
int wdgs_tiled_rasterizer_encode(wdgs_tiled_rasterizer* op, uint32_t width, uint32_t height) {
    WDGS_REQUIRE(op && width > 0 && height > 0, WDGS_E_INVALID, "wdgs_tiled_rasterizer_encode: invalid argument");
    wdgs_tiled_forward* f = op->fwd;
    WDGS_REQUIRE(f->encoded, WDGS_E_STATE, "rasterizer encode before the forward pass was encoded");
    WDGS_REQUIRE(width == f->cfg.viewport_width && height == f->cfg.viewport_height, WDGS_E_STATE,
                 "rasterizer size %ux%u differs from the forward pass viewport %ux%u", width, height, f->cfg.viewport_width, f->cfg.viewport_height);
    wdgs_device* d = op->dev;
    const TileInfo& ti = f->tile_info;
    if (width != op->width || height != op->height) {
        WDGS_REQUIRE(!d->capturing, WDGS_E_STATE, "TiledRasterizer.encode allocates its textures on first use: run one eager encode before recording");
        (void)wdgs_sync_lanes(d);
        free_dev(op->rgba8); free_dev(op->alpha); free_dev(op->n_contrib);
        op->rgba8 = nullptr; op->alpha = nullptr; op->n_contrib = nullptr;
        const size_t px = (size_t)width * height;
        WDGS_TRY(wdgs_alloc((void**)&op->rgba8, px * 4, true, d->stream));
        WDGS_TRY(wdgs_alloc((void**)&op->alpha, px * 4, true, d->stream));
        WDGS_TRY(wdgs_alloc((void**)&op->n_contrib, px * 4, true, d->stream));
        op->width = width;
        op->height = height;
    }
    const int fo = wdgs_sorter_final_out_index(f->sorter);
    const void* keys = wdgs_sorter_keys(f->sorter, fo);
    const void* vals = wdgs_sorter_values(f->sorter, fo);
    if (f->ranges_valid) {
        op->ranges_used = f->ranges;
    } else {
        if (ti.total_tiles + 1 > op->ranges_capacity) {
            WDGS_REQUIRE(!d->capturing, WDGS_E_STATE, "TiledRasterizer.encode allocates its range table on first use: run one eager encode before recording");
            (void)wdgs_sync_lanes(d);
            free_dev(op->ranges);
            op->ranges = nullptr;
            WDGS_TRY(wdgs_alloc((void**)&op->ranges, sizeof(u32) * (size_t)(ti.total_tiles + 1), true, d->stream));
            op->ranges_capacity = ti.total_tiles + 1;
        }
        WDGS_TRY(launch_tile_ranges(d, keys, f->stats, ti.total_tiles, op->ranges));
        op->ranges_used = op->ranges;
    }
    WDGS_TRY(launch_rasterize(d, f->settings, ti, f->splats, f->cfg.num_points, op->ranges_used, keys, vals, f->stats, op->compat_caps ? 32u : 0u, op->rgba8,
                              op->alpha, op->n_contrib, f->nf_stamp, f->stats + FRAME_WORD,
                              (f->ranges_valid && f->long_lists.hdr && !op->compat_caps) ? &f->long_lists : nullptr));
    op->encoded = true;
    return WDGS_OK;
}

int wdgs_tiled_rasterizer_encode_depth(wdgs_tiled_rasterizer* op, uint32_t kinds) {
    WDGS_REQUIRE(op, WDGS_E_INVALID, "wdgs_tiled_rasterizer_encode_depth: null op");
    constexpr uint32_t all = WDGS_DEPTH_EXPECTED | WDGS_DEPTH_MEDIAN | WDGS_DEPTH_WEIGHT_SUM;
    WDGS_REQUIRE(kinds != 0u && (kinds & ~all) == 0u, WDGS_E_INVALID, "wdgs_tiled_rasterizer_encode_depth: kinds 0x%x is not a non-empty set of WDGS_DEPTH_* bits", kinds);
    wdgs_tiled_forward* f = op->fwd;
    WDGS_REQUIRE(op->encoded && f->encoded && op->ranges_used, WDGS_E_STATE, "TiledRasterizer.encodeDepth before encode: depth is composited from the frame encode rasterized");
    WDGS_REQUIRE(op->width == f->cfg.viewport_width && op->height == f->cfg.viewport_height, WDGS_E_STATE,
                 "TiledRasterizer.encodeDepth: the forward pass viewport changed to %ux%u since the last encode (%ux%u)", f->cfg.viewport_width, f->cfg.viewport_height,
                 op->width, op->height);
    WDGS_REQUIRE(f->settings.gaussian_mode >= 0.5f, WDGS_E_STATE, "TiledRasterizer.encodeDepth: the forward pass is in point-cloud render mode, which has no weights");
    wdgs_device* d = op->dev;
    if (op->depth_width != op->width || op->depth_height != op->height) {
        bool any = false;
        for (float* img : op->depth) any = any || img != nullptr;
        if (any) {
            WDGS_REQUIRE(!d->capturing, WDGS_E_STATE, "TiledRasterizer.encodeDepth re-allocates its images after a size change: run one eager encodeDepth before recording");
            (void)wdgs_sync_lanes(d);
            for (float*& img : op->depth) { free_dev(img); img = nullptr; }
        }
        op->depth_width = op->width;
        op->depth_height = op->height;
    }
    for (u32 k = 0; k < 3u; k++) {
        if (!((kinds >> k) & 1u) || op->depth[k]) continue;
        WDGS_REQUIRE(!d->capturing, WDGS_E_STATE, "TiledRasterizer.encodeDepth allocates a depth image on first use of its kind: run one eager encodeDepth before recording");
        WDGS_TRY(wdgs_alloc((void**)&op->depth[k], (size_t)op->width * op->height * 4, true, d->stream));
    }
    const int fo = wdgs_sorter_final_out_index(f->sorter);
    WDGS_TRY(launch_depth_composite(d, f->settings, f->tile_info, f->splats, f->cfg.num_points, f->depths, op->ranges_used, wdgs_sorter_keys(f->sorter, fo),
                                    wdgs_sorter_values(f->sorter, fo), f->stats, op->compat_caps ? 32u : 0u, (kinds & WDGS_DEPTH_WEIGHT_SUM) ? op->depth[2] : nullptr,
                                    (kinds & WDGS_DEPTH_EXPECTED) ? op->depth[0] : nullptr, (kinds & WDGS_DEPTH_MEDIAN) ? op->depth[1] : nullptr, f->nf_stamp,
                                    f->stats + FRAME_WORD));
    op->depth_encoded = kinds;
    return WDGS_OK;
}
int wdgs_tiled_rasterizer_get_depth(wdgs_tiled_rasterizer* op, uint32_t kind, void** out) {
    WDGS_REQUIRE(op && out, WDGS_E_INVALID, "wdgs_tiled_rasterizer_get_depth: null argument");
    WDGS_REQUIRE(kind == WDGS_DEPTH_EXPECTED || kind == WDGS_DEPTH_MEDIAN || kind == WDGS_DEPTH_WEIGHT_SUM, WDGS_E_INVALID,
                 "wdgs_tiled_rasterizer_get_depth: kind 0x%x is not one WDGS_DEPTH_* bit", kind);
    const u32 k = kind == WDGS_DEPTH_EXPECTED ? 0u : kind == WDGS_DEPTH_MEDIAN ? 1u : 2u;
    WDGS_REQUIRE((op->depth_encoded & kind) && op->depth[k], WDGS_E_STATE, "TiledRasterizer: depth image of this kind not encoded yet (call encodeDepth with it first)");
    *out = op->depth[k];
    return WDGS_OK;
}
#define RASTER_GETTER(fn, field, what)                                                                            \
    int fn(wdgs_tiled_rasterizer* op, void** out) {                                                               \
        WDGS_REQUIRE(op && out, WDGS_E_INVALID, #fn ": null argument");                                           \
        WDGS_REQUIRE(op->encoded && op->field, WDGS_E_STATE, "TiledRasterizer: " what " not created yet (call encode first)"); \
        *out = op->field;                                                                                         \
        return WDGS_OK;                                                                                           \
    }
RASTER_GETTER(wdgs_tiled_rasterizer_get_output, rgba8, "output texture")
RASTER_GETTER(wdgs_tiled_rasterizer_get_alpha, alpha, "alpha texture")
RASTER_GETTER(wdgs_tiled_rasterizer_get_n_contrib, n_contrib, "n_contrib texture")
RASTER_GETTER(wdgs_tiled_rasterizer_get_tile_offsets, ranges_used, "tile offsets")
#undef RASTER_GETTER

int wdgs_tiled_rasterizer_blit(wdgs_tiled_rasterizer* op, void* target, uint32_t tw, uint32_t th) {
    WDGS_REQUIRE(op && target, WDGS_E_INVALID, "wdgs_tiled_rasterizer_blit: null argument");
    WDGS_REQUIRE(op->encoded && op->rgba8, WDGS_E_STATE, "TiledRasterizer: no output texture to blit from. Call encode() first.");
    WDGS_REQUIRE(tw > 0 && th > 0, WDGS_E_INVALID, "wdgs_tiled_rasterizer_blit: empty target %ux%u", tw, th);
    return launch_downsample(op->dev, op->rgba8, op->width, op->height, target, tw, th);
}

static int backward_alloc_images(wdgs_tiled_backward* op, u32 w, u32 h) {
    const u32 px = w * h;
    if (px <= op->img_capacity) return WDGS_OK;
    (void)wdgs_sync_lanes(op->dev);
    free_dev(op->loss_image); free_dev(op->metric_err); free_dev(op->metric_flags);
    op->loss_image = nullptr; op->metric_err = nullptr; op->metric_flags = nullptr;
    WDGS_TRY(wdgs_alloc((void**)&op->loss_image, (size_t)px * 16, true, op->dev->stream));
    WDGS_TRY(wdgs_alloc((void**)&op->metric_err, (size_t)px * 4, true, op->dev->stream));
    WDGS_TRY(wdgs_alloc((void**)&op->metric_flags, (size_t)px * 4, true, op->dev->stream));
    op->img_capacity = px;
    return WDGS_OK;
}

static int backward_alloc_per_point(wdgs_tiled_backward* op, u32 capacity) {
    wdgs_device* d = op->dev;
    int r = wdgs_alloc((void**)&op->acc, (size_t)capacity * 48 + 16, true, d->stream);
    if (r == WDGS_OK) op->acc_dirty = reinterpret_cast<u32*>(reinterpret_cast<char*>(op->acc) + (size_t)capacity * 48);
    if (r == WDGS_OK) r = wdgs_alloc((void**)&op->gradients, (size_t)capacity * 32, true, d->stream);
    if (r == WDGS_OK) r = wdgs_alloc((void**)&op->metric_counts, (size_t)capacity * 4, true, d->stream);
    if (r == WDGS_OK) op->points_capacity = capacity;
    return r;
}
int wdgs_tiled_backward_resize(wdgs_tiled_backward* op, uint32_t n) {
    WDGS_REQUIRE(op, WDGS_E_INVALID, "wdgs_tiled_backward_resize: null op");
    wdgs_device* d = op->dev;
    WDGS_REQUIRE(!d->capturing, WDGS_E_STATE, "wdgs_tiled_backward_resize while recording a command buffer");
    WDGS_CHECK_HIP(hipSetDevice(d->ordinal));
    WDGS_CHECK_HIP(wdgs_sync_lanes(d));
    const u32 need = std::max(n, 1u);
    if (need > op->points_capacity) {
        free_dev(op->acc); free_dev(op->gradients); free_dev(op->metric_counts);
        op->acc = nullptr; op->gradients = nullptr; op->metric_counts = nullptr;
        op->points_capacity = 0;
        WDGS_TRY(backward_alloc_per_point(op, (u32)std::min<uint64_t>((uint64_t)need + need / 4, 0xFFFFFFFFull)));
    } else {
        WDGS_CHECK_HIP(hipMemsetAsync(op->acc, 0, (size_t)need * 48, d->stream));
        WDGS_CHECK_HIP(hipMemsetAsync(op->acc_dirty, 0, 16, d->stream));
        WDGS_CHECK_HIP(hipMemsetAsync(op->gradients, 0, (size_t)need * 32, d->stream));
        WDGS_CHECK_HIP(hipMemsetAsync(op->metric_counts, 0, (size_t)need * 4, d->stream));
    }
    op->cfg.num_points = n;
    return WDGS_OK;
}
int wdgs_tiled_backward_create(wdgs_device* d, const wdgs_tiled_backward_config* cfg, wdgs_tiled_backward** out) {
    WDGS_REQUIRE(d && cfg && out, WDGS_E_INVALID, "wdgs_tiled_backward_create: null argument");
    WDGS_REQUIRE(cfg->viewport_width > 0 && cfg->viewport_height > 0, WDGS_E_INVALID, "viewport must be non-empty");
    wdgs_tiled_backward* op = new wdgs_tiled_backward();
    std::memset(op, 0, sizeof(*op));
    op->dev = d;
    op->cfg = *cfg;
    op->gradient_output = true;
    if (op->cfg.training.c1 == 0.f) op->cfg.training.c1 = 0.01f * 0.01f;
    if (op->cfg.training.c2 == 0.f) op->cfg.training.c2 = 0.03f * 0.03f;
    op->settings = RenderSettings{cfg->gaussian_scale != 0.f ? cfg->gaussian_scale : 1.0f, (float)cfg->sh_deg, (float)cfg->viewport_width,
                                  (float)cfg->viewport_height, cfg->point_size_px != 0.f ? cfg->point_size_px : 3.0f, 0.0f,
                                  cfg->max_splat_radius_px != 0.f ? cfg->max_splat_radius_px : 128.0f};
    int r = backward_alloc_per_point(op, std::max(cfg->num_points, 1u));
    if (r == WDGS_OK) r = wdgs_alloc((void**)&op->metric_minmax, 4096, true, d->stream);
    if (r == WDGS_OK) r = backward_alloc_images(op, cfg->viewport_width, cfg->viewport_height);
    if (r != WDGS_OK) { wdgs_tiled_backward_destroy(op); return r; }
    *out = op;
    return WDGS_OK;
}
int wdgs_tiled_backward_destroy(wdgs_tiled_backward* op) {
    if (!op) return WDGS_OK;
    sync_if_alive(op->dev);
    free_dev(op->acc); free_dev(op->gradients); free_dev(op->loss_image); free_dev(op->metric_counts);
    free_dev(op->metric_err); free_dev(op->metric_flags); free_dev(op->metric_minmax);
    delete op;
    return WDGS_OK;
}
int wdgs_tiled_backward_set_gradient_output(wdgs_tiled_backward* op, int enabled) {
    WDGS_REQUIRE(op, WDGS_E_INVALID, "wdgs_tiled_backward_set_gradient_output: null op");
    op->gradient_output = enabled != 0;
    return WDGS_OK;
}
static int backward_loss(wdgs_tiled_backward* op, const void* pred, const void* targ, void* acc, u32 acc_rows, const void* acc_dirty) {
    const u32 w = op->cfg.viewport_width, h = op->cfg.viewport_height;
    if (op->dssim_mode == WDGS_DSSIM_GAUSSIAN) return launch_dssim_grad(op->dev, w, h, pred, targ, op->cfg.training, op->loss_image, acc, acc_rows, acc_dirty);
    return launch_loss_grad(op->dev, w, h, pred, targ, op->cfg.training, op->loss_image, acc, acc_rows, acc_dirty);
}
int wdgs_tiled_backward_compute_loss_only(wdgs_tiled_backward* op, const void* pred, const void* targ) {
    WDGS_REQUIRE(op && pred && targ, WDGS_E_INVALID, "wdgs_tiled_backward_compute_loss_only: null argument");
    return backward_loss(op, pred, targ, nullptr, 0u, nullptr);
}
static int backward_encode_raster(wdgs_tiled_backward* op, const void* pred, const void* targ, const wdgs_tiled_backward_resources* res) {
    wdgs_device* d = op->dev;
    const u32 w = op->cfg.viewport_width, h = op->cfg.viewport_height, n = op->cfg.num_points;
    if (w > 0 && h > 0) WDGS_TRY(backward_loss(op, pred, targ, op->acc, std::max(n, 1u), op->acc_dirty));
    else WDGS_TRY(launch_acc_clear_if_dirty(d, op->acc, n, op->acc_dirty));
    const LongWork* lw = nullptr;
    auto owner = d->range_tables.find(res->tile_offsets_buffer);
    if (owner != d->range_tables.end() && owner->second->ranges_valid && owner->second->long_lists.hdr) lw = &owner->second->long_lists;
    return launch_backward_rasterize(d, op->settings, ceil_div(w, 16), ceil_div(h, 16), res->tile_offsets_buffer, res->tile_indices_buffer, res->splat_buffer,
                                     res->alpha_texture, res->n_contrib_texture, op->loss_image, op->acc, op->acc_dirty, lw);
}
int wdgs_tiled_backward_encode(wdgs_tiled_backward* op, const void* pred, const void* targ, const wdgs_tiled_backward_resources* res,
                               const void* gaussians) {
    WDGS_REQUIRE(op && pred && targ && res && gaussians, WDGS_E_INVALID, "wdgs_tiled_backward_encode: null argument");
    WDGS_REQUIRE(res->splat_buffer && res->tile_offsets_buffer && res->tile_indices_buffer && res->camera_buffer && res->alpha_texture && res->n_contrib_texture,
                 WDGS_E_INVALID, "wdgs_tiled_backward_encode: incomplete resources");
    WDGS_TRY(backward_encode_raster(op, pred, targ, res));
    return launch_geometry_backward(op->dev, op->cfg.num_points, res->camera_buffer, op->settings, gaussians, op->acc, op->gradients);
}
int wdgs_tiled_backward_encode_raster(wdgs_tiled_backward* op, const void* pred, const void* targ, const wdgs_tiled_backward_resources* res) {
    WDGS_REQUIRE(op && pred && targ && res, WDGS_E_INVALID, "wdgs_tiled_backward_encode_raster: null argument");
    WDGS_REQUIRE(res->splat_buffer && res->tile_offsets_buffer && res->tile_indices_buffer && res->alpha_texture && res->n_contrib_texture, WDGS_E_INVALID,
                 "wdgs_tiled_backward_encode_raster: incomplete resources");
    return backward_encode_raster(op, pred, targ, res);
}
int wdgs_tiled_backward_encode_geometry(wdgs_tiled_backward* op, const void* camera, const void* gaussians, const wdgs_view_accumulate* into) {
    WDGS_REQUIRE(op && camera && gaussians, WDGS_E_INVALID, "wdgs_tiled_backward_encode_geometry: null argument");
    if (!into) return launch_geometry_backward(op->dev, op->cfg.num_points, camera, op->settings, gaussians, op->acc, op->gradients);
    WDGS_REQUIRE(into->sums && into->visible && into->tile_counts && into->guard && into->overflow_word, WDGS_E_INVALID,
                 "wdgs_tiled_backward_encode_geometry: incomplete accumulate target");
    return launch_geometry_backward_accumulate(op->dev, op->cfg.num_points, camera, op->settings, gaussians, op->acc, op->acc_dirty, op->gradients, into->sums, into->visible,
                                               into->tile_counts, into->guard, into->overflow_word, into->first ? 1u : 2u);
}
int wdgs_tiled_backward_encode_geometry_views(wdgs_tiled_backward* const* ops, const void* const* cameras, const void* const* tile_counts, const void* const* overflow_words,
                                              uint32_t count, const void* gaussians, void* sums, void* visible, void* guard, int write_gradients, int continues) {
    WDGS_REQUIRE(ops && cameras && tile_counts && overflow_words && gaussians && sums && visible && guard && count > 0 && count <= WDGS_MAX_BATCH_VIEWS, WDGS_E_INVALID,
                 "wdgs_tiled_backward_encode_geometry_views: invalid argument");
    wdgs_tiled_backward* b0 = ops[0];
    WDGS_REQUIRE(b0, WDGS_E_INVALID, "wdgs_tiled_backward_encode_geometry_views: null pass");
    void *accs[WDGS_MAX_BATCH_VIEWS], *dirty[WDGS_MAX_BATCH_VIEWS], *grads[WDGS_MAX_BATCH_VIEWS];
    for (u32 v = 0; v < count; v++) {
        wdgs_tiled_backward* b = ops[v];
        WDGS_REQUIRE(b && cameras[v] && tile_counts[v] && overflow_words[v], WDGS_E_INVALID, "wdgs_tiled_backward_encode_geometry_views: null argument for view %u", v);
        for (u32 u = 0; u < v; u++) WDGS_REQUIRE(ops[u] != b, WDGS_E_INVALID, "wdgs_tiled_backward_encode_geometry_views: pass %u is given twice (every view has accumulators of its own)", v);
        WDGS_REQUIRE(b->dev == b0->dev && b->cfg.num_points == b0->cfg.num_points && std::memcmp(&b->settings, &b0->settings, sizeof(RenderSettings)) == 0, WDGS_E_STATE,
                     "wdgs_tiled_backward_encode_geometry_views: pass %u differs from pass 0 (cloud size, viewport or settings)", v);
        accs[v] = b->acc; dirty[v] = b->acc_dirty; grads[v] = b->gradients;
    }
    return launch_geometry_backward_views(b0->dev, b0->cfg.num_points, count, cameras, b0->settings, gaussians, accs, dirty, tile_counts, overflow_words,
                                          write_gradients ? grads : nullptr, sums, visible, guard, continues ? 1u : 0u);
}
int wdgs_tiled_backward_compute_metric_map(wdgs_tiled_backward* op, const void* pred, const void* targ, float threshold) {
    WDGS_REQUIRE(op && pred && targ, WDGS_E_INVALID, "wdgs_tiled_backward_compute_metric_map: null argument");
    return launch_metric_map(op->dev, op->cfg.viewport_width, op->cfg.viewport_height, pred, targ, 1000000.0f, threshold, op->metric_err, op->metric_minmax,
                             op->metric_minmax + 2, op->metric_flags);
}
int wdgs_tiled_backward_compute_metric_counts(wdgs_tiled_backward* op, const wdgs_tiled_backward_resources* res, uint32_t num_instances, int clear) {
    WDGS_REQUIRE(op && res && res->splat_buffer && res->tile_offsets_buffer && res->tile_indices_buffer && res->n_contrib_texture, WDGS_E_INVALID,
                 "wdgs_tiled_backward_compute_metric_counts: incomplete resources");
    const u32 n = op->cfg.num_points;
    u32* const counts = op->metric_counts_into ? op->metric_counts_into : op->metric_counts;
    if (clear) WDGS_CHECK_HIP(hipMemsetAsync(counts, 0, (size_t)std::max(n, 1u) * 4, op->dev->stream));
    return launch_metric_count(op->dev, op->settings, ceil_div(op->cfg.viewport_width, 16), ceil_div(op->cfg.viewport_height, 16), res->tile_offsets_buffer,
                               res->tile_indices_buffer, num_instances, res->splat_buffer, n, op->metric_flags, res->n_contrib_texture, counts, n);
}
int wdgs_tiled_backward_normalize_metric_counts(wdgs_tiled_backward* op, uint32_t divisor) {
    WDGS_REQUIRE(op, WDGS_E_INVALID, "null op");
    return launch_metric_normalize(op->dev, op->cfg.num_points, divisor, op->metric_counts);
}
int wdgs_tiled_backward_set_viewport(wdgs_tiled_backward* op, uint32_t w, uint32_t h) {
    WDGS_REQUIRE(op && w > 0 && h > 0, WDGS_E_INVALID, "wdgs_tiled_backward_set_viewport: invalid argument");
    op->cfg.viewport_width = w;
    op->cfg.viewport_height = h;
    op->settings.viewport_x = (float)w;
    op->settings.viewport_y = (float)h;
    return backward_alloc_images(op, w, h);
}
int wdgs_tiled_backward_set_training_config(wdgs_tiled_backward* op, const wdgs_training_config* cfg) {
    WDGS_REQUIRE(op && cfg, WDGS_E_INVALID, "null argument");
    op->cfg.training = *cfg;
    if (op->cfg.training.c1 == 0.f) op->cfg.training.c1 = 0.01f * 0.01f;
    if (op->cfg.training.c2 == 0.f) op->cfg.training.c2 = 0.03f * 0.03f;
    return WDGS_OK;
}
int wdgs_tiled_backward_set_dssim_mode(wdgs_tiled_backward* op, uint32_t mode) {
    WDGS_REQUIRE(op, WDGS_E_INVALID, "wdgs_tiled_backward_set_dssim_mode: null op");
    WDGS_REQUIRE(mode == WDGS_DSSIM_REFERENCE || mode == WDGS_DSSIM_GAUSSIAN, WDGS_E_INVALID, "wdgs_tiled_backward_set_dssim_mode: unknown mode %u", mode);
    op->dssim_mode = mode;
    return WDGS_OK;
}
int wdgs_tiled_backward_get_dssim_mode(const wdgs_tiled_backward* op, uint32_t* out) {
// ... 221 lines not shown
```

webdgs_amd/csrc/common.h:

```cpp
#pragma once
#include <hip/hip_runtime.h>

#include <cstdint>
#include <cstdio>
#include <map>
#include <string>
#include <vector>

#include "../../include/webdgs.h"

typedef uint32_t u32;
typedef int32_t i32;

void wdgs_set_error(const char* fmt, ...);

#define WDGS_CHECK_HIP(expr)                                                                      \
    do {                                                                                          \
        hipError_t _e = (expr);                                                                   \
        if (_e != hipSuccess) {                                                                   \
            wdgs_set_error("%s failed: %s (%s:%d)", #expr, hipGetErrorString(_e), __FILE__, __LINE__); \
            return WDGS_E_HIP;                                                                    \
        }                                                                                         \
    } while (0)

#define WDGS_REQUIRE(cond, code, ...)  \
    do {                               \
        if (!(cond)) {                 \
            wdgs_set_error(__VA_ARGS__); \
            return (code);             \
        }                              \
    } while (0)

#define WDGS_TRY(expr)                 \
    do {                               \
        int _r = (expr);               \
        if (_r != WDGS_OK) return _r;  \
    } while (0)

struct wdgs_device {
    int ordinal = 0;
    hipStream_t stream = nullptr;
    bool own_stream = false;
    hipStream_t lanes[WDGS_MAX_LANES] = {};
    hipEvent_t lane_events[WDGS_MAX_LANES] = {};
    hipEvent_t lane_marks[WDGS_MAX_BATCH_VIEWS] = {};
    int lane = 0;
    hipEvent_t ticket_events[WDGS_TICKET_RING] = {};
    uint64_t ticket_next = 1;
    u32* host_guard = nullptr;
    bool profiling = false;
    bool capturing = false;
    struct Pending { const char* name; hipEvent_t a, b; };
    std::vector<Pending> pending;
    std::vector<hipEvent_t> event_pool;
    struct Total { u32 launches = 0; float ms = 0.f; };
    std::map<std::string, Total> totals;
    std::vector<wdgs_tiled_forward*> forwards;
    std::map<const void*, wdgs_tiled_forward*> range_tables;
    std::vector<wdgs_tiled_forward*> capture_consumes;
    std::vector<void*> dead_command_buffers;
    int num_cus = 256;
    double* ssim_partials = nullptr;
    u32 ssim_partials_count = 0;
};

inline hipError_t wdgs_sync_lanes(wdgs_device* d) {
    for (int l = 1; l < WDGS_MAX_LANES; l++) {
        if (!d->lanes[l]) continue;
        const hipError_t e = hipStreamSynchronize(d->lanes[l]);
        if (e != hipSuccess) return e;
    }
    return hipStreamSynchronize(d->lanes[0] ? d->lanes[0] : d->stream);
}

struct KernelScope {
    wdgs_device* d;
    const char* name;
    hipEvent_t a = nullptr, b = nullptr;
    KernelScope(wdgs_device* dev, const char* n) : d(dev), name(n) {
        if (d->profiling && !d->capturing) {
            a = take(); b = take();
            (void)hipEventRecord(a, d->stream);
        }
    }
    ~KernelScope() {
        if (a) {
            (void)hipEventRecord(b, d->stream);
            d->pending.push_back({name, a, b});
        }
    }
    hipEvent_t take() {
        if (!d->event_pool.empty()) { hipEvent_t e = d->event_pool.back(); d->event_pool.pop_back(); return e; }
        hipEvent_t e; (void)hipEventCreate(&e); return e;
    }
};

#define WDGS_LAUNCH(dev, kname, kernel, grid, block, shmem, ...)                           \
    do {                                                                                   \
        KernelScope _ks((dev), (kname));                                                   \
        hipLaunchKernelGGL(kernel, (grid), (block), (shmem), (dev)->stream, __VA_ARGS__);  \
    } while (0)

constexpr u32 CS_PLANES = 7;
struct CsView {
    float4* planes;
    u32 pitch;
    __device__ __forceinline__ float4& quad(u32 k, u32 idx) const { return planes[(size_t)k * pitch + idx]; }
};

__device__ __forceinline__ u32 xcd_contiguous(u32 b, u32 g) {
    const u32 k = b & 7u, j = b >> 3, q = g >> 3, r = g & 7u;
    return k * q + min(k, r) + j;
}

static inline u32 ceil_div(u32 a, u32 b) { return (a + b - 1u) / b; }
static inline u32 bits_for(u32 v) {
    u32 b = 0;
    while (v) { b++; v >>= 1; }
    return b;
}

constexpr u32 SSIM_WG_PER_CU = 2;
constexpr u32 SSIM_TAPS = 11;
struct SsimWindow { float g[SSIM_TAPS]; };
const SsimWindow& ssim_window();
static inline size_t align_up(size_t a, size_t b) { return (a + b - 1) / b * b; }

int wdgs_alloc(void** p, size_t bytes, bool zero, hipStream_t stream);
void wdgs_free(void* p);
bool wdgs_device_alive(const wdgs_device* d);

struct ScanScratch { u32* block_sums = nullptr; u32 capacity_blocks = 0; };
int scan_scratch_create(ScanScratch* s, u32 max_elements);
void scan_scratch_destroy(ScanScratch* s);
int scan_exclusive_u32(wdgs_device* dev, ScanScratch* s, const u32* in, u32* out, u32 count, u32* total_out);
struct ScanStatsEpilogue { u32* stats; u32* visible_shards; u32* host_mirror; u32 capacity; u32* frame = nullptr; u32* long_hdr = nullptr; };
int scan_exclusive_u32_stats(wdgs_device* dev, ScanScratch* s, const u32* in, u32* out, u32 count, u32* total_out, const ScanStatsEpilogue& ep);

int scan_block_sums_inplace(wdgs_device* dev, u32* block_sums, u32 num_blocks, const ScanStatsEpilogue& ep);
int forward_scan(wdgs_device* dev, u32* block_sums, u32 num_blocks, u32* column_counts, u32* column_totals, u32 columns, const ScanStatsEpilogue& ep);

struct RenderSettings { float gaussian_scaling, sh_deg, viewport_x, viewport_y, point_size_px, gaussian_mode, max_splat_radius_px; };
// ... 2 lines not shown
```

webdgs_amd/csrc/longlist.h:

```cpp
#pragma once
#include "common.h"
#include "dmath.h"

constexpr u32 LL_BLOCKS = 0u;
constexpr u32 LL_ITEMS = 1u;
constexpr u32 LL_FWD_HEAD = 2u;
constexpr u32 LL_BWD_HEAD = 3u;
constexpr u32 LL_ROWS = 4u;
constexpr u32 LL_ROWS_WANTED = 5u;
constexpr u32 LL_STALLED = 6u;
constexpr u32 LL_HDR_WORDS = 8u;

constexpr u32 LL_NO_ROWS = 0xFFFFFFFFu;

struct LongBlock { u32 tile, sub, first_item, chunks; };
struct LongSync {
    u32 counted;
    u32 row_base;
    u32 scanned;
    u32 filled;
    u32 rows;
    u32 walked;
    u32 pad0, pad1;
};

struct LongWork {
    u32* hdr;
    u32* flags;
    LongBlock* blocks;
    LongSync* sync;
    u32* item_block;
    u32* nlist;
    u32* cnt;
    u32* off;
    u32* total;
    u32* jlast;
    float4* records;
    u32* rows;
    u32 max_blocks, max_items, max_rows, threshold;
    const u32 *nf_stamp, *nf_frame;
};

WD_DEV void ll_st(u32* p, u32 v) { __hip_atomic_store(p, v, __ATOMIC_RELAXED, __HIP_MEMORY_SCOPE_AGENT); }
WD_DEV u32 ll_ld(const u32* p) { return __hip_atomic_load(p, __ATOMIC_RELAXED, __HIP_MEMORY_SCOPE_AGENT); }
WD_DEV bool ll_wait(const u32* p, u32 target, u32* hdr, u32 code) {
    for (u32 spins = 0; spins < (1u << 19); spins++) {
        if ((u32)__builtin_amdgcn_readfirstlane((int)ll_ld(p)) >= target) {
            __builtin_amdgcn_fence(__ATOMIC_ACQUIRE, "workgroup");
            return true;
        }
        __builtin_amdgcn_s_sleep(8);
    }
    atomicMax(&hdr[LL_STALLED], code);
    return false;
}
WD_DEV void ll_signal(u32* p, u32 lane) {
    __builtin_amdgcn_fence(__ATOMIC_RELEASE, "workgroup");
    __hip_atomic_fetch_add(p, lane == 0u ? 1u : 0u, __ATOMIC_RELAXED, __HIP_MEMORY_SCOPE_AGENT);
}
WD_DEV u32 ll_pull(u32* head, u32 n_tasks, u32 batch, u32 lane) {
    if ((u32)__builtin_amdgcn_readfirstlane((int)ll_ld(head)) >= n_tasks) return 0xFFFFFFFFu;
    const u32 t = (u32)__builtin_amdgcn_readfirstlane((int)__hip_atomic_fetch_add(head, lane == 0u ? batch : 0u, __ATOMIC_RELAXED, __HIP_MEMORY_SCOPE_AGENT));
    return t < n_tasks ? t : 0xFFFFFFFFu;
}
WD_DEV u32 ll_batch(u32 n_tasks) { return min(max(n_tasks >> 11, 1u), 8u); }
WD_DEV bool ll_frame_on(const LongWork& lw, u32 blocks_wanted, u32 items_wanted) { return blocks_wanted != 0u && blocks_wanted <= lw.max_blocks && items_wanted <= lw.max_items; }
```

webdgs_amd/csrc/sort.hip:

```cpp
#include <algorithm>

#include "common.h"
#include "longlist.h"

namespace {

constexpr u32 SORT_THREADS = 256;
constexpr u32 SORT_ITEMS_MAX = 16;
constexpr u32 SORT_TILE_MAX = SORT_THREADS * SORT_ITEMS_MAX;
constexpr u32 RADIX = 256;

struct DigitOf {
    u32 shift, dmask, row_inv;
    __device__ __forceinline__ u32 operator()(u32 key) const { return row_inv ? min(__umulhi((key >> 16u) - 1u, row_inv), dmask) : ((key >> shift) & dmask); }
};

template <u32 ITEMS>
__global__ __launch_bounds__(SORT_THREADS) void sort_hist_kernel(const u32* __restrict__ keys, const u32* __restrict__ count_ptr, DigitOf digit_of,
                                                                 u32 num_parts, u32* __restrict__ counts , u32* __restrict__ ranges_init,
                                                                 u32 total_tiles, u32* __restrict__ marks_init) {
    constexpr u32 TILE = SORT_THREADS * ITEMS;
    __shared__ u32 lh[SORT_THREADS / 64][RADIX];
    const u32 count = *count_ptr;
    const u32 part = blockIdx.x;
// ... 357 lines not shown
    for (u32 c0 = 0; c0 < n; c0 += 4u * SEG_THREADS) {
        u32 kn[4], vn[4];
#pragma unroll
        for (u32 j = 0; j < 4u; j++) {
            const u32 i_next = c0 + (4u + j) * SEG_THREADS + threadIdx.x;
            kn[j] = (i_next < n) ? src_k[i_next] : 0xFFFFFFFFu;
            vn[j] = (i_next < n) ? src_v[i_next] : 0u;
        }
        my_counts[0] = make_uint4(0u, 0u, 0u, 0u);
        my_counts[1] = make_uint4(0u, 0u, 0u, 0u);
        u32 below[4], group[4];
#pragma unroll
        for (u32 j = 0; j < 4u; j++) {
            const bool valid = c0 + j * SEG_THREADS + threadIdx.x < n;
            const u32 digit = (kq[j] >> shift) & (RADIX - 1u);
            unsigned long long m = __ballot(valid);
#pragma unroll
            for (u32 b = 0; b < 8; b++) {
                const bool bit = (digit >> b) & 1u;
                const unsigned long long bal = __ballot(bit);
                m &= bit ? bal : ~bal;
            }
            below[j] = (u32)__popcll(m & lt_mask);
            group[j] = (valid && below[j] == 0u) ? (u32)__popcll(m) : 0u;
        }
        lds_barrier();
#pragma unroll
        for (u32 j = 0; j < 4u; j++)
            if (group[j] != 0u) cnt16[((kq[j] >> shift) & (RADIX - 1u)) * 16u + j * 4u + wave] = (seg_hist_t)group[j];
        lds_barrier();
        u32 trip_total = 0u;
        {
            uint4 q[2] = {my_counts[0], my_counts[1]};
            u32* const w = reinterpret_cast<u32*>(q);
#pragma unroll
            for (u32 x = 0; x < 8u; x++) {
                const u32 lo = w[x] & 0xFFFFu, hi = w[x] >> 16u;
                w[x] = trip_total | ((trip_total + lo) << 16u);
                trip_total += lo + hi;
            }
            my_counts[0] = q[0];
            my_counts[1] = q[1];
        }
        lds_barrier();
#pragma unroll
        for (u32 j = 0; j < 4u; j++) {
            if (c0 + j * SEG_THREADS + threadIdx.x < n) {
                const u32 digit = (kq[j] >> shift) & (RADIX - 1u);
                const u32 pos = s_base[digit] + cnt16[digit * 16u + j * 4u + wave] + below[j];
                dst_k[pos] = kq[j];
                dst_v[pos] = vq[j];
            }
        }
        lds_barrier();
        s_base[threadIdx.x] += trip_total;
#pragma unroll
        for (u32 j = 0; j < 4u; j++) { kq[j] = kn[j]; vq[j] = vn[j]; }
    }
    __syncthreads();
}

__device__ void long_list_build(const LongWork& lw, u32 t, u32 n) {
    __shared__ u32 s_first, s_lb;
    const bool want = lw.threshold != 0u && n > lw.threshold && !(lw.nf_stamp && lw.nf_stamp[t] == *lw.nf_frame);
    if (!want) return;
    const u32 chunks = (n + 63u) >> 6, need = 4u * chunks;
    if (threadIdx.x == 0u) {
        s_first = atomicAdd(&lw.hdr[LL_ITEMS], need);
        s_lb = atomicAdd(&lw.hdr[LL_BLOCKS], 4u);
    }
    __syncthreads();
    const u32 first = s_first, lb = s_lb;
    const bool items_fit = first + need <= lw.max_items && first + need >= first, blocks_fit = lb + 4u <= lw.max_blocks;
    const bool ok = items_fit && blocks_fit;
    for (u32 i = threadIdx.x; i < need && first + i < lw.max_items && first + i >= first; i += SEG_THREADS) lw.item_block[first + i] = ok ? lb + i / chunks : 0xFFFFFFFFu;
    if (threadIdx.x < 4u && lb + threadIdx.x < lw.max_blocks) {
        const u32 b = lb + threadIdx.x;
        lw.blocks[b] = LongBlock{t, threadIdx.x, first + threadIdx.x * chunks, ok ? chunks : 0u};
        lw.sync[b] = LongSync{0u, LL_NO_ROWS, 0u, 0u, 0u, 0u, 0u, 0u};
    }
    if (threadIdx.x == 0u && ok) lw.flags[t] = 0xFu;
}

__global__ __launch_bounds__(SEG_THREADS, 6) void segment_sort_kernel(u32* __restrict__ cur_k, u32* __restrict__ cur_v, u32* __restrict__ alt_k,
                                                                    u32* __restrict__ alt_v, const u32* __restrict__ ranges, u32 total_tiles, LongWork lw) {
    __shared__ u32 a_k[SEG_CAP], a_v[SEG_CAP];
    __shared__ seg_hist_t whist[SEG_THREADS / 64][SEG_BINS];
    __shared__ u32 s_base[RADIX];
    __shared__ u32 s_wsum[SEG_THREADS / 64];
    __shared__ u32 s_min[SEG_THREADS / 64], s_max[SEG_THREADS / 64];
    const u32 t = blockIdx.x;
    const u32 start = ranges[t];
    u32 end = ranges[t + 1u];
    if (start == 0xFFFFFFFFu) return;
    for (u32 nx = t + 1u; end == 0xFFFFFFFFu && nx < total_tiles;) { nx++; end = ranges[nx]; }
    if (lw.flags) long_list_build(lw, t, (end != 0xFFFFFFFFu && end > start) ? end - start : 0u);
    if (end <= start + 1u || end == 0xFFFFFFFFu) return;
    const u32 n = end - start;
    if (n <= SEG_CAP) {
        const u32 lane = threadIdx.x & 63u, wave = threadIdx.x >> 6;
        const u32 per_wave = ((n + 3u) / 4u + 63u) & ~63u;
        const u32 rounds = per_wave / 64u;
        u32 kk[SEG_ROUNDS], vv[SEG_ROUNDS];
#pragma unroll
        for (u32 j = 0; j < SEG_ROUNDS; j++) {
            const u32 i = wave * per_wave + j * 64u + lane;
            const bool valid = j < rounds && i < n;
            kk[j] = valid ? cur_k[start + i] : 0xFFFFFFFFu;
            vv[j] = valid ? cur_v[start + i] : 0u;
        }
        u32 lo16 = 0xFFFFu, hi16 = 0u;
#pragma unroll
        for (u32 j = 0; j < SEG_ROUNDS; j++) {
            const u32 i = wave * per_wave + j * 64u + lane;
            if (j < rounds && i < n) { lo16 = min(lo16, kk[j] & 0xFFFFu); hi16 = max(hi16, kk[j] & 0xFFFFu); }
        }
#pragma unroll
        for (u32 d = 32; d >= 1; d >>= 1) {
            lo16 = min(lo16, (u32)__shfl_xor((int)lo16, (int)d, 64));
            hi16 = max(hi16, (u32)__shfl_xor((int)hi16, (int)d, 64));
        }
        if (lane == 0u) { s_min[wave] = lo16; s_max[wave] = hi16; }
        __syncthreads();
        lo16 = min(min(s_min[0], s_min[1]), min(s_min[2], s_min[3]));
        hi16 = max(max(s_max[0], s_max[1]), max(s_max[2], s_max[3]));
        if (hi16 - lo16 < (1u << 8)) {
            seg_pass_regs<8>(kk, vv, a_k, a_v, n, per_wave, lo16, 0u, whist, s_wsum);
        } else if (hi16 - lo16 < (1u << 9)) {
            seg_pass_regs<9>(kk, vv, a_k, a_v, n, per_wave, lo16, 0u, whist, s_wsum);
        } else if (hi16 - lo16 < SEG_BINS) {
            seg_pass_regs<SEG_WIDE_BITS>(kk, vv, a_k, a_v, n, per_wave, lo16, 0u, whist, s_wsum);
        } else {
            seg_pass_regs<8>(kk, vv, a_k, a_v, n, per_wave, 0u, 0u, whist, s_wsum);
#pragma unroll
            for (u32 j = 0; j < SEG_ROUNDS; j++) {
                const u32 i = wave * per_wave + j * 64u + lane;
                const bool valid = j < rounds && i < n;
                kk[j] = valid ? a_k[i] : 0xFFFFFFFFu;
                vv[j] = valid ? a_v[i] : 0u;
            }
            __syncthreads();
            seg_pass_regs<8>(kk, vv, a_k, a_v, n, per_wave, 0u, 8u, whist, s_wsum);
        }
        for (u32 i = threadIdx.x; i < n; i += SEG_THREADS) { cur_k[start + i] = a_k[i]; cur_v[start + i] = a_v[i]; }
    } else {
        seg_pass_global(cur_k + start, cur_v + start, alt_k + start, alt_v + start, n, 0u, whist, s_base, s_wsum);
        __syncthreads();
        seg_pass_global(alt_k + start, alt_v + start, cur_k + start, cur_v + start, n, 8u, whist, s_base, s_wsum);
    }
}

}

struct wdgs_sorter {
    wdgs_device* dev;
    u32 capacity;
    u32 items;
    u32 num_parts;
    const u32* count_ptr;
    u32* keys[2];
    u32* vals[2];
    u32* counts;
    u32* totals;
    int final_out_index;
};

extern "C" {

int wdgs_sorter_create(wdgs_device* dev, uint32_t max_capacity, const void* stats_dev, wdgs_sorter** out) {
    WDGS_REQUIRE(dev && out && stats_dev, WDGS_E_INVALID, "wdgs_sorter_create: null argument");
    WDGS_REQUIRE(max_capacity <= 0xFFFFF000u, WDGS_E_CAPACITY, "sorter capacity %u too large", max_capacity);
    wdgs_sorter* s = new wdgs_sorter();
    s->dev = dev;
    s->capacity = (u32)align_up(max_capacity > 0 ? max_capacity : 1, SORT_TILE_MAX);
    s->items = s->capacity <= (8u << 20) ? 4u : SORT_ITEMS_MAX;
    s->num_parts = s->capacity / (SORT_THREADS * s->items);
    s->count_ptr = (const u32*)stats_dev;
    s->final_out_index = 0;
    for (int i = 0; i < 2; i++) { s->keys[i] = nullptr; s->vals[i] = nullptr; }
    s->counts = nullptr;
    s->totals = nullptr;
    int r = WDGS_OK;
    for (int i = 0; i < 2 && r == WDGS_OK; i++) {
        r = wdgs_alloc((void**)&s->keys[i], sizeof(u32) * (size_t)s->capacity, true, dev->stream);
        if (r == WDGS_OK) r = wdgs_alloc((void**)&s->vals[i], sizeof(u32) * (size_t)s->capacity, true, dev->stream);
    }
    if (r == WDGS_OK) r = wdgs_alloc((void**)&s->counts, sizeof(u32) * (size_t)RADIX * s->num_parts, true, dev->stream);
    if (r == WDGS_OK) r = wdgs_alloc((void**)&s->totals, sizeof(u32) * RADIX, true, dev->stream);
    if (r != WDGS_OK) { wdgs_sorter_destroy(s); return r; }
    *out = s;
    return WDGS_OK;
}

int wdgs_sorter_destroy(wdgs_sorter* s) {
    if (!s) return WDGS_OK;
    for (int i = 0; i < 2; i++) {
        if (s->keys[i]) wdgs_free(s->keys[i]);
        if (s->vals[i]) wdgs_free(s->vals[i]);
    }
    if (s->counts) wdgs_free(s->counts);
    if (s->totals) wdgs_free(s->totals);
    delete s;
    return WDGS_OK;
}

void* wdgs_sorter_keys(wdgs_sorter* s, int i) { return s ? s->keys[i & 1] : nullptr; }
void* wdgs_sorter_values(wdgs_sorter* s, int i) { return s ? s->vals[i & 1] : nullptr; }
int wdgs_sorter_final_out_index(wdgs_sorter* s) { return s ? s->final_out_index : 0; }
void sorter_set_final_out_index(wdgs_sorter* s, int i) { if (s) s->final_out_index = i & 1; }
uint32_t wdgs_sorter_capacity(wdgs_sorter* s) { return s ? s->capacity : 0; }

}

int sorter_sort_segmented(wdgs_sorter* s, u32 segment_bits, u32 num_segments, u32* ranges, const LongWork* lw) {
    wdgs_device* dev = s->dev;
    const u32 bits = std::min(segment_bits, 16u);
    const u32 passes = (bits + 7u) / 8u;
    int src = 0;
    u32 shift = 16u, left = bits;
    for (u32 p = 0; p < passes; p++) {
        const u32 width = left / (passes - p);
        left -= width;
        const u32 dmask = (1u << width) - 1u;
        u32* const marks = (p == 0u && lw) ? lw->flags : nullptr;
        if (s->items == 4u) {
            WDGS_LAUNCH(dev, "sort_hist", sort_hist_kernel<4u>, dim3(s->num_parts), dim3(SORT_THREADS), 0, s->keys[src], s->count_ptr, (DigitOf{shift, dmask, 0u}), s->num_parts,
                        s->counts, (u32*)nullptr, num_segments, marks);
        } else {
            WDGS_LAUNCH(dev, "sort_hist", sort_hist_kernel<SORT_ITEMS_MAX>, dim3(s->num_parts), dim3(SORT_THREADS), 0, s->keys[src], s->count_ptr, (DigitOf{shift, dmask, 0u}), s->num_parts,
                        s->counts, (u32*)nullptr, num_segments, marks);
        }
        if (s->items == 4u) {
            WDGS_LAUNCH(dev, "sort_scan_rows", sort_scan_rows_kernel<4u>, dim3(dmask + 1u), dim3(256), 0, s->counts, s->count_ptr, s->num_parts, s->totals);
        } else {
            WDGS_LAUNCH(dev, "sort_scan_rows", sort_scan_rows_kernel<SORT_ITEMS_MAX>, dim3(dmask + 1u), dim3(256), 0, s->counts, s->count_ptr, s->num_parts, s->totals);
        }
        const u32 ranges_mode = (passes == 2u) ? p + 1u : 0u;
        if (s->items == 4u) {
            WDGS_LAUNCH(dev, "sort_scatter", sort_scatter_kernel<4u>, dim3(s->num_parts), dim3(SORT_THREADS), 0, s->keys[src], s->vals[src], s->keys[src ^ 1],
                        s->vals[src ^ 1], s->count_ptr, (DigitOf{shift, dmask, 0u}), s->num_parts, s->counts, s->totals, ranges, ranges_mode, num_segments);
        } else {
            WDGS_LAUNCH(dev, "sort_scatter", sort_scatter_kernel<SORT_ITEMS_MAX>, dim3(s->num_parts), dim3(SORT_THREADS), 0, s->keys[src], s->vals[src], s->keys[src ^ 1],
                        s->vals[src ^ 1], s->count_ptr, (DigitOf{shift, dmask, 0u}), s->num_parts, s->counts, s->totals, ranges, ranges_mode, num_segments);
        }
        src ^= 1;
        shift += width;
    }
    if (passes != 2u)
        WDGS_LAUNCH(dev, "tile_ranges", tile_ranges_kernel, dim3(ceil_div(num_segments + 1, 4)), dim3(256), 0, s->keys[src], s->count_ptr, num_segments, ranges);
    if (num_segments > 0)
        WDGS_LAUNCH(dev, "sort_segments", segment_sort_kernel, dim3(num_segments), dim3(SEG_THREADS), 0, s->keys[src], s->vals[src], s->keys[src ^ 1],
                    s->vals[src ^ 1], ranges, num_segments, lw ? *lw : LongWork{});
    WDGS_CHECK_HIP(hipGetLastError());
    s->final_out_index = src;
    return WDGS_OK;
}

int sorter_sort_rows(wdgs_sorter* s, u32 num_tiles_x, u32 num_tiles_y, u32* ranges, const LongWork* lw) {
    wdgs_device* dev = s->dev;
    const u32 tiles = num_tiles_x * num_tiles_y;
    const DigitOf rows{0u, num_tiles_y - 1u, 0xFFFFFFFFu / num_tiles_x + 1u};
    if (s->items == 4u) {
        WDGS_LAUNCH(dev, "sort_hist", sort_hist_kernel<4u>, dim3(s->num_parts), dim3(SORT_THREADS), 0, s->keys[0], s->count_ptr, rows, s->num_parts, s->counts, ranges, tiles, lw ? lw->flags : (u32*)nullptr);
    } else {
        WDGS_LAUNCH(dev, "sort_hist", sort_hist_kernel<SORT_ITEMS_MAX>, dim3(s->num_parts), dim3(SORT_THREADS), 0, s->keys[0], s->count_ptr, rows, s->num_parts, s->counts, ranges, tiles, lw ? lw->flags : (u32*)nullptr);
    }
    if (s->items == 4u) {
        WDGS_LAUNCH(dev, "sort_scan_rows", sort_scan_rows_kernel<4u>, dim3(num_tiles_y), dim3(256), 0, s->counts, s->count_ptr, s->num_parts, s->totals);
    } else {
        WDGS_LAUNCH(dev, "sort_scan_rows", sort_scan_rows_kernel<SORT_ITEMS_MAX>, dim3(num_tiles_y), dim3(256), 0, s->counts, s->count_ptr, s->num_parts, s->totals);
    }
    if (s->items == 4u) {
        WDGS_LAUNCH(dev, "sort_scatter", sort_scatter_kernel<4u>, dim3(s->num_parts), dim3(SORT_THREADS), 0, s->keys[0], s->vals[0], s->keys[1], s->vals[1], s->count_ptr, rows,
                    s->num_parts, s->counts, s->totals, ranges, 2u, tiles);
    } else {
        WDGS_LAUNCH(dev, "sort_scatter", sort_scatter_kernel<SORT_ITEMS_MAX>, dim3(s->num_parts), dim3(SORT_THREADS), 0, s->keys[0], s->vals[0], s->keys[1], s->vals[1], s->count_ptr, rows,
                    s->num_parts, s->counts, s->totals, ranges, 2u, tiles);
    }
    WDGS_LAUNCH(dev, "sort_segments", segment_sort_kernel, dim3(tiles), dim3(SEG_THREADS), 0, s->keys[1], s->vals[1], s->keys[0], s->vals[0], ranges, tiles, lw ? *lw : LongWork{});
    WDGS_CHECK_HIP(hipGetLastError());
    s->final_out_index = 1;
    return WDGS_OK;
}

extern "C" {

int wdgs_sorter_sort(wdgs_sorter* s, uint32_t key_bits) {
    WDGS_REQUIRE(s, WDGS_E_INVALID, "wdgs_sorter_sort: null sorter");
    if (key_bits == 0 || key_bits > 32) key_bits = 32;
    const u32 passes = (key_bits + 7u) / 8u;
    wdgs_device* dev = s->dev;
    int src = 0;
    for (u32 p = 0; p < passes; p++) {
        const u32 shift = p * 8u;
        if (s->items == 4u) {
            WDGS_LAUNCH(dev, "sort_hist", sort_hist_kernel<4u>, dim3(s->num_parts), dim3(SORT_THREADS), 0, s->keys[src], s->count_ptr, (DigitOf{shift, RADIX - 1u, 0u}), s->num_parts,
                        s->counts, (u32*)nullptr, 0u, (u32*)nullptr);
        } else {
            WDGS_LAUNCH(dev, "sort_hist", sort_hist_kernel<SORT_ITEMS_MAX>, dim3(s->num_parts), dim3(SORT_THREADS), 0, s->keys[src], s->count_ptr, (DigitOf{shift, RADIX - 1u, 0u}), s->num_parts,
                        s->counts, (u32*)nullptr, 0u, (u32*)nullptr);
        }
        if (s->items == 4u) {
            WDGS_LAUNCH(dev, "sort_scan_rows", sort_scan_rows_kernel<4u>, dim3(RADIX), dim3(256), 0, s->counts, s->count_ptr, s->num_parts, s->totals);
        } else {
            WDGS_LAUNCH(dev, "sort_scan_rows", sort_scan_rows_kernel<SORT_ITEMS_MAX>, dim3(RADIX), dim3(256), 0, s->counts, s->count_ptr, s->num_parts, s->totals);
        }
        if (s->items == 4u) {
            WDGS_LAUNCH(dev, "sort_scatter", sort_scatter_kernel<4u>, dim3(s->num_parts), dim3(SORT_THREADS), 0, s->keys[src], s->vals[src], s->keys[src ^ 1],
                        s->vals[src ^ 1], s->count_ptr, (DigitOf{shift, RADIX - 1u, 0u}), s->num_parts, s->counts, s->totals, (u32*)nullptr, 0u, 0u);
        } else {
            WDGS_LAUNCH(dev, "sort_scatter", sort_scatter_kernel<SORT_ITEMS_MAX>, dim3(s->num_parts), dim3(SORT_THREADS), 0, s->keys[src], s->vals[src], s->keys[src ^ 1],
                        s->vals[src ^ 1], s->count_ptr, (DigitOf{shift, RADIX - 1u, 0u}), s->num_parts, s->counts, s->totals, (u32*)nullptr, 0u, 0u);
        }
        src ^= 1;
    }
    WDGS_CHECK_HIP(hipGetLastError());
    s->final_out_index = src;
    return WDGS_OK;
}

}

int launch_tile_ranges(wdgs_device* dev, const void* sorted_keys, const void* count_ptr, u32 total_tiles, void* ranges) {
    WDGS_LAUNCH(dev, "tile_ranges", tile_ranges_kernel, dim3(ceil_div(total_tiles + 1, 4)), dim3(256), 0, (const u32*)sorted_keys, (const u32*)count_ptr,
                total_tiles, (u32*)ranges);
    WDGS_CHECK_HIP(hipGetLastError());
    return WDGS_OK;
}

extern "C" int wdgs_debug_sort_tiles(wdgs_sorter* s, uint32_t route, uint32_t num_tiles_x, uint32_t num_tiles_y, void* ranges_u32_dev) {
    WDGS_REQUIRE(s && ranges_u32_dev, WDGS_E_INVALID, "wdgs_debug_sort_tiles: null argument");
    WDGS_REQUIRE(route <= 2u, WDGS_E_INVALID, "wdgs_debug_sort_tiles: unknown route %u", route);
    const unsigned long long tiles = (unsigned long long)num_tiles_x * num_tiles_y;
    WDGS_REQUIRE(tiles >= 1ull && tiles <= 65534ull, WDGS_E_INVALID, "wdgs_debug_sort_tiles: %u x %u tiles (1..65534)", num_tiles_x, num_tiles_y);
    const u32 total = (u32)tiles;
    if (route == 0u) return sorter_sort_segmented(s, bits_for(total), total, (u32*)ranges_u32_dev, nullptr);
    if (route == 1u) {
        WDGS_REQUIRE(num_tiles_x >= 2u && num_tiles_x <= 256u && num_tiles_y <= 256u, WDGS_E_INVALID,
                     "wdgs_debug_sort_tiles: the row route takes 2..256 tile columns and at most 256 tile rows, not %u x %u", num_tiles_x, num_tiles_y);
        return sorter_sort_rows(s, num_tiles_x, num_tiles_y, (u32*)ranges_u32_dev, nullptr);
    }
    s->final_out_index = 0;
    return launch_tile_ranges(s->dev, s->keys[0], s->count_ptr, total, ranges_u32_dev);
}
```

webdgs_amd/ops.py:

```python
from __future__ import annotations

import ctypes as C
import dataclasses
import re
from typing import Optional

import numpy as np
import torch

from . import _lib
from ._lib import CapacityError, StateError, WdgsError, check


MAX_LANES = 4
MAX_BATCH_VIEWS = 16


class HipBuffer:

    def __init__(self, device: "HipDevice", ptr: int, size: int, owner: Optional[torch.Tensor] = None, label: str = ""):
        self.device, self.ptr, self.size, self._owner, self.label = device, int(ptr or 0), int(size), owner, label
        self.destroyed = False
        self.before_read = None

# ... 306 lines not shown
            point_size_px=float(config.get("pointSizePx", 3.0)), max_splat_radius_px=float(config.get("maxSplatRadiusPx", 128.0)),
            render_mode=1 if config.get("renderMode", "gaussian") == "gaussian" else 0,
            max_tile_entries=int(config.get("maxTileEntries", 0)), compat_caps=1 if config.get("compatCaps", False) else 0)
        h = C.c_void_p()
        check(device.lib.wdgs_tiled_forward_create(device.handle, C.byref(cfg), C.byref(h)))
        self.handle = h
        self._dc_source: Optional[HipBuffer] = None

    def syncDcSource(self) -> None:
        want = getattr(self.pointCloud, "dc_words", None)
        if want is not getattr(self, "_dc_source", None):
            self.setDcSource(want)

    def encode(self, encoder: Optional[HipEncoder] = None, options: Optional[dict] = None) -> None:
        skip = 1 if (options or {}).get("skipSort") else 0
        self.syncDcSource()
        check(self.device.lib.wdgs_tiled_forward_encode(self.handle, self.pointCloud.gaussian_3d_buffer.ptr, self.pointCloud.sh_buffer.ptr,
                                                        self.cameraBuffer.ptr, skip))

    def encodeProjected(self, encoder: Optional["HipEncoder"] = None) -> None:
        check(self.device.lib.wdgs_tiled_forward_encode_projected(self.handle))

    def isProjected(self) -> bool:
        return bool(self.device.lib.wdgs_tiled_forward_is_projected(self.handle))

    def setCameraBuffer(self, buffer: HipBuffer) -> None:
        self.cameraBuffer = buffer

    def setDcSource(self, dcWords: Optional[HipBuffer]) -> None:
        self._dc_source = dcWords
        check(self.device.lib.wdgs_tiled_forward_set_dc_source(self.handle, dcWords.ptr if dcWords is not None else None))

    def setPointCloud(self, pointCloud: PointCloud) -> bool:
        if pointCloud.sh_deg != self.pointCloud.sh_deg:
            return False
        check(self.device.lib.wdgs_tiled_forward_resize(self.handle, pointCloud.num_points))
        self.pointCloud = pointCloud
        return True

    def setGaussianScale(self, value: float) -> None:
        check(self.device.lib.wdgs_tiled_forward_set_gaussian_scale(self.handle, float(value)))

    def setPointSize(self, value: float) -> None:
        check(self.device.lib.wdgs_tiled_forward_set_point_size(self.handle, float(value)))

    def setRenderMode(self, mode: str) -> None:
        check(self.device.lib.wdgs_tiled_forward_set_render_mode(self.handle, 1 if mode == "gaussian" else 0))

    def setViewport(self, width: int, height: int) -> None:
        check(self.device.lib.wdgs_tiled_forward_set_viewport(self.handle, int(width), int(height)))

    def _res(self) -> _lib.TiledForwardResources:
        r = _lib.TiledForwardResources()
        check(self.device.lib.wdgs_tiled_forward_get_resources(self.handle, C.byref(r)))
        return r

    def getResources(self) -> dict:
        r, d, n = self._res(), self.device, max(1, self.pointCloud.num_points)
        return dict(splatBuffer=d.view(r.splat_buffer, 24 * n), depthsBuffer=d.view(r.depths_buffer, 4 * n),
                    tileKeysBuffer=d.view(r.tile_keys_buffer, 4 * r.max_tile_entries), tileIndicesBuffer=d.view(r.tile_indices_buffer, 4 * r.max_tile_entries),
                    tileOffsetsBuffer=d.view(r.tile_offsets_buffer, 4 * n), tileCountsBuffer=d.view(r.tile_counts_buffer, 4 * n),
                    statsBuffer=d.view(r.stats_buffer, 16), numTilesX=r.num_tiles_x, numTilesY=r.num_tiles_y, totalTiles=r.total_tiles,
                    maxTileEntries=r.max_tile_entries, settings=np.array(list(r.settings), np.float32))

    def getSortedIndicesBuffer(self) -> HipBuffer:
        return self.getResources()["tileIndicesBuffer"]

    def getSortedKeysBuffer(self) -> HipBuffer:
        return self.getResources()["tileKeysBuffer"]

    def getTileOffsetsBuffer(self) -> HipBuffer:
        return self.getResources()["tileOffsetsBuffer"]

    def getStatsBuffer(self) -> HipBuffer:
        return self.getResources()["statsBuffer"]

    def check(self) -> np.ndarray:
        st = (C.c_uint32 * 4)()
        check(self.device.lib.wdgs_tiled_forward_check(self.handle, st))
        return np.array(list(st), np.uint32)

    def setLongLists(self, threshold: int, maxItems: int = 0, maxRows: int = 0) -> None:
        check(self.device.lib.wdgs_tiled_forward_set_long_lists(self.handle, int(threshold), int(maxItems), int(maxRows)))

    def longListStats(self) -> dict:
        st = (C.c_uint32 * 12)()
        check(self.device.lib.wdgs_tiled_forward_long_list_stats(self.handle, st))
        keys = ("blocksWanted", "itemsWanted", "forwardQueue", "backwardQueue", "rowsUsed", "rowsWanted", "stalled", "_", "maxItems", "maxBlocks", "maxRows", "threshold")
        return {k: int(v) for k, v in zip(keys, st) if k != "_"}

    def destroy(self) -> None:
        if self.destroyed:
            return
        self.destroyed = True
        self.device.lib.wdgs_tiled_forward_destroy(self.handle)
        self.handle = None


DEPTH_KINDS = {"expected": 1, "median": 2, "weight_sum": 4}


def _depth_mask(kinds) -> int:
    mask = 0
    for k in ((kinds,) if isinstance(kinds, str) else kinds):
        if k not in DEPTH_KINDS:
            raise ValueError(f"unknown depth kind {k!r}: one of {sorted(DEPTH_KINDS)}")
        mask |= DEPTH_KINDS[k]
    return mask


class TiledRasterizer:

    def __init__(self, config: dict):
        self.device: HipDevice = config["device"]
        self.forwardPass: TiledForwardPass = config["forwardPass"]
        self.destroyed = False
        self.width = self.height = 0
        h = C.c_void_p()
        check(self.device.lib.wdgs_tiled_rasterizer_create(self.device.handle, self.forwardPass.handle, 1 if config.get("compatCaps") else 0, C.byref(h)))
        self.handle = h

    def encode(self, encoder: Optional[HipEncoder], width: int, height: int) -> None:
        check(self.device.lib.wdgs_tiled_rasterizer_encode(self.handle, int(width), int(height)))
        self.width, self.height = int(width), int(height)

    def _get(self, fn, nbytes: int) -> HipBuffer:
        p = C.c_void_p()
        check(fn(self.handle, C.byref(p)))
        return self.device.view(p.value, nbytes)

    def getOutputTextureView(self) -> HipBuffer:
        return self._get(self.device.lib.wdgs_tiled_rasterizer_get_output, 4 * self.width * self.height)

    def getAlphaTextureView(self) -> HipBuffer:
        return self._get(self.device.lib.wdgs_tiled_rasterizer_get_alpha, 4 * self.width * self.height)

    def getNContribTextureView(self) -> HipBuffer:
        return self._get(self.device.lib.wdgs_tiled_rasterizer_get_n_contrib, 4 * self.width * self.height)

    def getTileOffsetsBuffer(self) -> HipBuffer:
        tiles = ((self.width + 15) // 16) * ((self.height + 15) // 16)
        return self._get(self.device.lib.wdgs_tiled_rasterizer_get_tile_offsets, 4 * (tiles + 1))

    def encodeDepth(self, encoder: Optional[HipEncoder], kinds=("expected",)) -> None:
        mask = int(kinds) if isinstance(kinds, (int, np.integer)) else _depth_mask(kinds)
        check(self.device.lib.wdgs_tiled_rasterizer_encode_depth(self.handle, mask))

    def getDepthTextureView(self, kind: str = "expected") -> HipBuffer:
        p = C.c_void_p()
        check(self.device.lib.wdgs_tiled_rasterizer_get_depth(self.handle, _depth_mask((kind,)), C.byref(p)))
        return self.device.view(p.value, 4 * self.width * self.height)

    def blitToTexture(self, encoder: Optional[HipEncoder], target: HipBuffer, width: Optional[int] = None, height: Optional[int] = None) -> None:
        w, h = int(width or self.width), int(height or self.height)
        if self.handle is not None and w * h * 4 > target.size:
            raise _lib.WdgsError(_lib.WDGS_E_INVALID, f"blitToTexture: target of {target.size} bytes is smaller than {w}x{h} rgba8")
        check(self.device.lib.wdgs_tiled_rasterizer_blit(self.handle, target.ptr, max(w, 0), max(h, 0)))

    def destroy(self) -> None:
        if self.destroyed:
            return
        self.destroyed = True
        self.device.lib.wdgs_tiled_rasterizer_destroy(self.handle)
        self.handle = None


# ... 434 lines not shown
```

webdgs_amd/trainer.py:

```python
from __future__ import annotations

import math
import os
import random
import time
from typing import Optional

import numpy as np
import torch

from . import loaders, ops, parallel


class Trainer:
    def __init__(self, device: ops.HipDevice, trainingConfig: Optional[dict] = None, seed: int = 0, world_size: int = 1, rank: int = 0,
                 views_per_rank: int = 1, maxTileEntries: int = 0, use_command_buffers: bool = True, exchange: Optional[parallel.Exchange] = None,
                 overlap_views: Optional[bool] = None, pipeline_depth: int = 1, batch_views: Optional[bool] = None):
        ops.dssim_mode(trainingConfig)
        self.device = device
        self.trainingConfig = dict(trainingConfig or dict(lambda_l1=0.8, lambda_l2=0.0, lambda_dssim=0.2))
        self.optimizerHyperparameters = dict(ops.DEFAULT_ADAM_HYPERPARAMETERS)
        self.world_size, self.rank, self.views_per_rank = int(world_size), int(rank), max(1, int(views_per_rank))
        self.maxTileEntries = int(maxTileEntries)
        self._grown_tile_entries = 0
        self._foreign_overflow_warned = False
        self.exchange = exchange if exchange is not None else (parallel.default_exchange(device, self.world_size) if self.world_size > 1 else parallel.Exchange())
        self._sliced = self.world_size > 1 or bool(getattr(self.exchange, "force", False))
        if self.world_size > 1 and (self.exchange.world_size, self.exchange.rank) != (self.world_size, self.rank):
            raise ValueError(f"exchange is rank {self.exchange.rank} of {self.exchange.world_size}, trainer is rank {self.rank} of {self.world_size}")
        self.use_command_buffers = bool(use_command_buffers)
        self._cmd_cache: dict = {}
        self._eager_steps = 0
        if overlap_views is None:
            overlap_views = int(os.environ.get("WDGS_LANES", self.DEFAULT_LANES))
        elif isinstance(overlap_views, bool):
            overlap_views = self.DEFAULT_LANES if overlap_views else 1
        self._lanes = max(1, min(int(overlap_views), self.views_per_rank, ops.MAX_LANES))
        self.batch_views = self.views_per_rank > 1 and (os.environ.get("WDGS_BATCH_VIEWS", "1") != "0" if batch_views is None else bool(batch_views))
        self._op_sets = min(self.views_per_rank, ops.MAX_BATCH_VIEWS) if self.batch_views else self._lanes
        self.view_group = int(os.environ.get("WDGS_VIEW_GROUP", "0"))
        self._camera_buffers: list = []
        self._rng = random.Random(seed)

        self.forwardPass = self.rasterizer = self.backwardPass = self.optimizer = None
        self.pipeline_depth = max(1, min(int(pipeline_depth), 4))
        self.reuse_passes = True
        self.fuse_geometry_adam = True
        self.keep_gradients = os.environ.get("WDGS_KEEP_GRADIENTS", "0") == "1"
        self.deferred_sh = os.environ.get("WDGS_DEFERRED_SH", "1") != "0"
        self._dc_words: Optional[ops.HipBuffer] = None
        self._gradient_output_applied: Optional[bool] = None
        self._tickets: list = []
        self._more_op_sets: list = []
        self.metricsForwardPass = self.metricsRasterizer = self.metricsPass = None
        self.metricsViewportWidth = self.metricsViewportHeight = 0
        self.metricsTarget: Optional[ops.HipBuffer] = None
        self.metric_lanes = max(1, min(int(os.environ.get("WDGS_METRIC_LANES", self.DEFAULT_LANES)), ops.MAX_LANES))
        self._more_metric_sets: list = []
        self.pointCloud: Optional[ops.PointCloud] = None
        self.cameraBuffer = device.createBuffer(272, "camera uniform")
        self.metricsCameraBuffer = device.createBuffer(272, "metrics camera uniform")

        self.isTraining = False
        self.iteration = 0
        self.maxIterations = 10_000
        self.stepItersPerSec = 0.0
        self.stepMs = 0.0
        self.lastDensifyPruneIteration: Optional[int] = None
        self.lastViewportWidth = self.lastViewportHeight = 1
        self.pendingPointCloudSwap: Optional[dict] = None
        self.trainCameras: list = []
        self.images: list = []
        self.evalCameras: list = []
        self.evalImages: list = []
        self._eval_camera_buffers: list = []
        self._eval_sets: dict = {}
        self.evalMaxTileEntries = 0
        self._eval_tile_entries = 0
        self._eval_long_lists: Optional[dict] = None

        self.densifyPruneConfig = dict(
            schedule=dict(enabled=True, warmupIterations=500, interval=100, stopIterations=15_000),
            metricViews=10, metricDownscale=2, metricThreshold=0.5, maxBufferBytes=128 * 1024 * 1024, maxNewPointsPerStep=5000,
            pruneOpacity=0.01, cloneThresholdCount=500, splitScaleThreshold=1.0)
        self.densifyPrune = ops.DensifyPrunePass(device, self._densify_op_config())
        self._dp_grad: Optional[ops.HipBuffer] = None
        self._dp_visible: Optional[ops.HipBuffer] = None
        self._dp_rows: Optional[ops.HipBuffer] = None
        self._dp_flag: Optional[ops.HipBuffer] = None
        self._agree_word: Optional[ops.HipBuffer] = None
        self.longLists: Optional[dict] = None
        self._state_sliced = False
        self.exchange_timing = False
        self._exchange_events: list = []

    DEFAULT_LANES = 3
    _OP_NAMES = ("forwardPass", "rasterizer", "backwardPass", "metricsForwardPass", "metricsRasterizer", "metricsPass", "optimizer")

    def _destroy_more_metric_sets(self) -> None:
        for more in self._more_metric_sets:
            for op in more[:3]:
                op.destroy()
        self._more_metric_sets = []

    def _destroy_more_op_sets(self) -> None:
        for ops_of_lane in self._more_op_sets:
            for op in ops_of_lane:
                op.destroy()
        self._more_op_sets = []

    def _densify_op_config(self) -> dict:
        c = self.densifyPruneConfig
        return dict(strategy="gpu_rebuild", numViews=c["metricViews"], maxBufferBytes=c["maxBufferBytes"], maxNewPointsPerStep=c["maxNewPointsPerStep"],
                    pruneThreshold=c["pruneOpacity"], cloneThreshold=c["cloneThresholdCount"], splitThreshold=c["splitScaleThreshold"])

    def setPointCloud(self, pointCloud: ops.PointCloud) -> None:
        self.applyPointCloudSwap(dict(pointCloud=pointCloud))

    def requestPointCloudSwap(self, pointCloud: ops.PointCloud, optimizerInitialState: Optional[dict] = None) -> None:
        self.pendingPointCloudSwap = dict(pointCloud=pointCloud, optimizerInitialState=optimizerInitialState)

    def consumePointCloudSwapRequest(self) -> Optional[dict]:
        req, self.pendingPointCloudSwap = self.pendingPointCloudSwap, None
        return req

    def requestResizeTo(self, numPoints: int) -> None:
        if self.pointCloud is None:
            return
        self.requestPointCloudSwap(ops.allocatePointCloudLike(self.device, self.pointCloud, dict(numPoints=numPoints)))

    def applyPointCloudSwap(self, request: dict) -> None:
        self.drain()
        self._synchronize()
        oldParams = self.optimizer.getHyperparameters() if self.optimizer else None
        if self.optimizer is not None:
            self.optimizer.destroy()
            self.optimizer = None
        old = self.pointCloud
        self.pointCloud = request["pointCloud"]
        self._invalidate_command_buffers()
        passes = [self.forwardPass, self.backwardPass, self.metricsForwardPass, self.metricsPass] + [op for more in self._more_op_sets + self._more_metric_sets for op in (more[0], more[2])]
        kept = self.reuse_passes and old is not None and all(p.setPointCloud(self.pointCloud) for p in passes if p is not None)
        if not kept:
            for name in self._OP_NAMES:
                op = getattr(self, name)
                if op is not None:
                    op.destroy()
                setattr(self, name, None)
            self._destroy_more_op_sets()
            self._destroy_more_metric_sets()
        self.optimizer = ops.Optimizer(self.device, self.pointCloud, oldParams or self.optimizerHyperparameters, request.get("optimizerInitialState"))
        self.optimizerHyperparameters = dict(self.optimizer.getHyperparameters())
        self._dc_words = self.optimizer.setDeferredSH(self.pointCloud, True) if self.deferred_sh else None
        for fw in self._forward_passes():
            fw.setDcSource(self._dc_words)
        if old is not None and old is not self.pointCloud:
            old.gaussian_3d_buffer.destroy()
            old.sh_buffer.destroy()
        self._dp_grad = self._dp_visible = self._dp_rows = self._dp_flag = None
        self._state_sliced = False
        self.ensurePipelines(self.lastViewportWidth, self.lastViewportHeight)

    def _forward_passes(self) -> list:
        return [p for p in [self.forwardPass, self.metricsForwardPass] + [more[0] for more in self._more_op_sets + self._more_metric_sets] if p is not None]

    def flushPointCloud(self) -> None:
        if self.optimizer is not None and self.pointCloud is not None:
            self.optimizer.flushSH(self.pointCloud)

    def _invalidate_command_buffers(self) -> None:
        deferred = None
        if self._tickets and self.device.handle:
            self._tickets = []
            try:
                self._synchronize()
            except ops.CapacityError as e:
                deferred = e
        for c in self._cmd_cache.values():
            c.destroy()
        self._cmd_cache = {}
        self._eager_steps = 0
        if deferred is not None:
            raise deferred

    def setDataset(self, cameras: list, images: list) -> None:
        self.trainCameras, self.images = self._views(cameras, images)
        self._camera_buffers = [self.device.bufferFrom(np.asarray(c["camera"], np.float32)) for c in self.trainCameras]
        self._invalidate_command_buffers()

    def _views(self, cameras: list, images: list) -> tuple:
        cameras, images = list(cameras), list(images)
        images = [im if isinstance(im, dict) else dict(name=im.name, width=im.width, height=im.height,
                                                       texture=im.texture if im.texture is not None else self.device.bufferFrom(im.bitmap))
                  for im in images]
        cameras = [c if "camera" in c else dict(c, camera=loaders.cameraUniforms(c, im["width"], im["height"])) for c, im in zip(cameras, images)]
        return cameras, images

    def getTrainingConfig(self) -> dict:
        return dict(self.trainingConfig)

    def setTrainingConfig(self, next_cfg: dict) -> None:
        ops.dssim_mode(dict(self.trainingConfig, **{k: v for k, v in next_cfg.items() if v is not None}))
        self.trainingConfig.update({k: v for k, v in next_cfg.items() if v is not None})
        self._invalidate_command_buffers()
        for p in [self.backwardPass, self.metricsPass] + [more[2] for more in self._more_op_sets + self._more_metric_sets]:
            if p is not None:
                p.setTrainingConfig(next_cfg)

    def getOptimizerHyperparameters(self) -> dict:
        return dict(self.optimizer.getHyperparameters() if self.optimizer else self.optimizerHyperparameters)

    def setOptimizerHyperparameters(self, next_params: dict) -> None:
        self.optimizerHyperparameters.update(next_params)
        self._invalidate_command_buffers()
        if self.optimizer:
            self.optimizer.setHyperparameters(next_params)

    def setDensifyPruneConfig(self, next_cfg: dict) -> None:
        sched = {**self.densifyPruneConfig["schedule"], **(next_cfg.get("schedule") or {})}
        self.densifyPruneConfig = {**self.densifyPruneConfig, **next_cfg, "schedule": sched}
        self.densifyPrune.setConfig(self._densify_op_config())

    def start(self) -> None:
        if self.pointCloud is None or not self.trainCameras:
            print("Cannot start training: Missing point cloud or dataset.")
            return
        self.isTraining = True
        self.iteration = 0
        self.stepItersPerSec = 0.0
        self.stepMs = 0.0
        self.lastDensifyPruneIteration = None
        for k in range(1, max(self._lanes, self.metric_lanes)):
            self.device.laneOrder(k, 0)
            self.device.laneOrder(0, k)

    def stop(self) -> None:
        self.isTraining = False
        if self.device.handle and self._tickets:
            self.drain()

    def getIsTraining(self) -> bool:
        return self.isTraining

    def setMaxIterations(self, n: int) -> None:
        self.maxIterations = max(1, int(n))

    def getMaxIterations(self) -> int:
        return self.maxIterations

    def getIteration(self) -> int:
        return self.iteration

    def getPointCount(self) -> int:
        return self.pointCloud.num_points if self.pointCloud else 0

    def getLastStepMs(self) -> float:
        return self.stepMs

    def getItersPerSec(self) -> float:
        return self.stepItersPerSec

    def getLastDensifyPruneIteration(self) -> Optional[int]:
        return self.lastDensifyPruneIteration

    def getNextDensifyPruneIteration(self) -> Optional[int]:
        s = self.densifyPruneConfig["schedule"]
        if not s["enabled"]:
            return None
        warmup, interval, stop, i = s["warmupIterations"], max(1, s["interval"]), s["stopIterations"], self.iteration
        if i >= stop:
            return None
        if i < warmup:
            return min(warmup, stop)
        nxt = warmup + math.ceil((i + 1 - warmup) / interval) * interval
        return nxt if nxt <= stop else None

    def _new_forward_pass(self, cameraBuffer, w: int, h: int, maxTileEntries: Optional[int] = None) -> ops.TiledForwardPass:
        entries = self._tile_entries() if maxTileEntries is None else int(maxTileEntries)
        fw = ops.TiledForwardPass(self.device, self.pointCloud, cameraBuffer, dict(viewportWidth=w, viewportHeight=h, renderMode="gaussian", maxTileEntries=entries))
        fw.setDcSource(self._dc_words)
        if self.longLists is not None:
            fw.setLongLists(int(self.longLists.get("threshold", 2048)), int(self.longLists.get("maxItems", 0)), int(self.longLists.get("maxRows", 0)))
        return fw

    def _grow_long_lists(self) -> None:
        import warnings
        cap_items, cap_rows = int((self.longLists or {}).get("maxItemsCap", 8192)), int((self.longLists or {}).get("maxRowsCap", 65536))
        have_items = have_rows = need_items = need_rows = 0
        for fw in self._forward_passes():
            st = fw.longListStats()
            if not st["threshold"]:
                continue
            if st["stalled"]:
                warnings.warn(f"a long-list task gave up waiting (code {st['stalled']:#x}): the frame's long tiles are not to be trusted", RuntimeWarning, stacklevel=3)
            have_items, have_rows = max(have_items, st["maxItems"]), max(have_rows, st["maxRows"])
            if st["itemsWanted"] <= cap_items:
                need_items, need_rows = max(need_items, st["itemsWanted"]), max(need_rows, st["rowsWanted"])
        items = max(have_items, min(int(need_items * 1.5), cap_items)) if need_items > have_items else have_items
        rows = max(have_rows, min(int(need_rows * 1.5), cap_rows)) if need_rows > have_rows else have_rows
        if (items, rows) == (have_items, have_rows):
            return
        self.longLists = dict(self.longLists or {}, maxItems=items, maxRows=rows)
        warnings.warn(f"long-list scratch enlarged to {self.longLists['maxItems']} chunk slots and {self.longLists['maxRows']} rows", RuntimeWarning, stacklevel=3)
        self._invalidate_command_buffers()
        for fw in self._forward_passes():
            fw.setLongLists(int(self.longLists.get("threshold", 2048)), self.longLists["maxItems"], self.longLists["maxRows"])

    def ensurePipelines(self, width: int, height: int) -> None:
        if (max(1, int(width)), max(1, int(height))) != (self.lastViewportWidth, self.lastViewportHeight):
            self._invalidate_command_buffers()
        self.lastViewportWidth, self.lastViewportHeight = max(1, int(width)), max(1, int(height))
        w, h = self.lastViewportWidth, self.lastViewportHeight
        if self.forwardPass is None:
            self.forwardPass = self._new_forward_pass(self.cameraBuffer, w, h)
        else:
            self.forwardPass.setViewport(w, h)
        if self.rasterizer is None:
            self.rasterizer = ops.TiledRasterizer(dict(device=self.device, forwardPass=self.forwardPass, format="rgba8unorm"))
        if self.backwardPass is None:
            self.backwardPass = ops.TiledBackwardPass(self.device, self.pointCloud, dict(viewportWidth=w, viewportHeight=h, trainingConfig=self.trainingConfig))
            self._gradient_output_applied = None
        else:
            self.backwardPass.setViewport(w, h)
        for more in self._more_op_sets:
            more[0].setViewport(w, h)
            more[2].setViewport(w, h)
        while len(self._more_op_sets) < self._op_sets - 1:
            fw = self._new_forward_pass(self.cameraBuffer, w, h)
            self._more_op_sets.append([fw, ops.TiledRasterizer(dict(device=self.device, forwardPass=fw, format="rgba8unorm")),
                                       ops.TiledBackwardPass(self.device, self.pointCloud, dict(viewportWidth=w, viewportHeight=h, trainingConfig=self.trainingConfig))])
        if self.optimizer is not None and self.world_size * self.views_per_rank == 1:
            self.optimizer.setGuard(self.forwardPass.getStatsBuffer(), 8)

    def ensureMetricsPipelines(self, baseWidth: int, baseHeight: int) -> tuple[int, int]:
        down = max(1, int(self.densifyPruneConfig["metricDownscale"]))
        w, h = max(1, baseWidth // down), max(1, baseHeight // down)
        if self.metricsForwardPass and self.metricsViewportWidth == w and self.metricsViewportHeight == h:
            return w, h
        for name in ("metricsForwardPass", "metricsRasterizer", "metricsPass"):
            op = getattr(self, name)
            if op is not None:
                op.destroy()
            setattr(self, name, None)
        self._destroy_more_metric_sets()
        self.metricsViewportWidth, self.metricsViewportHeight = w, h
        self.metricsForwardPass = self._new_forward_pass(self.metricsCameraBuffer, w, h)
        self.metricsRasterizer = ops.TiledRasterizer(dict(device=self.device, forwardPass=self.metricsForwardPass, format="rgba8unorm"))
        self.metricsPass = ops.TiledBackwardPass(self.device, self.pointCloud, dict(viewportWidth=w, viewportHeight=h, trainingConfig=self.trainingConfig))
        self.metricsTarget = self.device.createBuffer(4 * w * h, "metrics-gt-downsampled")
        return w, h

    def _metric_set(self, k: int) -> tuple:
        if k == 0:
            return self.metricsForwardPass, self.metricsRasterizer, self.metricsPass, self.metricsTarget, self.metricsCameraBuffer
        w, h = self.metricsViewportWidth, self.metricsViewportHeight
        while len(self._more_metric_sets) < k:
            cam = self.device.createBuffer(272, "metrics camera uniform")
            fw = self._new_forward_pass(cam, w, h)
            self._more_metric_sets.append([fw, ops.TiledRasterizer(dict(device=self.device, forwardPass=fw, format="rgba8unorm")),
                                           ops.TiledBackwardPass(self.device, self.pointCloud, dict(viewportWidth=w, viewportHeight=h, trainingConfig=self.trainingConfig)),
                                           self.device.createBuffer(4 * w * h, "metrics-gt-downsampled"), cam])
        return tuple(self._more_metric_sets[k - 1])

    @staticmethod
    def metrics_camera(camera: np.ndarray, width: int, height: int) -> np.ndarray:
        from . import synth
        cam = np.asarray(camera, np.float32)
        fov_y = 2.0 * math.atan(float(cam[65]) / (2.0 * float(cam[67])))
        focal = 0.5 * height / math.tan(fov_y * 0.5)
        fov_x = 2.0 * math.atan(width / (2.0 * focal))
        znear, zfar = 0.01, 100.0
        top, right = math.tan(fov_y / 2.0) * znear, math.tan(fov_x / 2.0) * znear
        out = np.zeros(68, np.float32)
        out[0:16] = cam[0:16]
        out[32], out[37] = 2.0 * znear / (2.0 * right), -2.0 * znear / (2.0 * top)
        out[42], out[43], out[46] = zfar / (zfar - znear), 1.0, -(zfar * znear) / (zfar - znear)
        out[16:32] = synth.mat4_inverse(out[0:16])
        out[48:64] = synth.mat4_inverse(out[32:48])
        out[64:68] = (width, height, focal, focal)
        return out

    def _ops_of(self, op_set: int) -> tuple:
        return tuple(self._more_op_sets[op_set - 1]) if op_set > 0 else (self.forwardPass, self.rasterizer, self.backwardPass)

    def _encode_view(self, encoder, index: int, op_set: int = 0, geometry: bool = True, projected: bool = False) -> None:
        forwardPass, rasterizer, backwardPass = self._ops_of(op_set)
        image = self.images[index]
        cam = self._camera_buffers[index]
        forwardPass.setCameraBuffer(cam)
        if projected:
            forwardPass.encodeProjected(encoder)
        else:
            forwardPass.encode(encoder)
        rasterizer.encode(encoder, image["width"], image["height"])
        res = dict(splatBuffer=forwardPass.getResources()["splatBuffer"], tileOffsetsBuffer=rasterizer.getTileOffsetsBuffer(),
                   tileIndicesBuffer=forwardPass.getSortedIndicesBuffer(), cameraBuffer=cam,
                   alphaTexture=rasterizer.getAlphaTextureView(), nContribTexture=rasterizer.getNContribTextureView())
        if geometry:
            backwardPass.encode(encoder, rasterizer.getOutputTextureView(), image["texture"], res)
        else:
            backwardPass.encodeRaster(encoder, rasterizer.getOutputTextureView(), image["texture"], res)

    def warmupCommandBuffers(self) -> int:
        if not self.use_command_buffers or not self.isTraining or self.pointCloud is None:
            return 0
        n_views, taken = self.world_size * self.views_per_rank, 0
        for v in range(len(self.trainCameras)):
            for _ in range(2 if v == 0 else 1):
                self.step([v] * n_views)
                taken += 1
        return taken

    def step(self, view_ids: Optional[list] = None) -> None:
        try:
            self._step(view_ids)
        except ops.CapacityError as e:
            if not self._grow_tile_entry_capacity(e):
                raise

    def _tile_entries(self) -> int:
        return self.maxTileEntries or self._grown_tile_entries

    def _grow_tile_entry_capacity(self, error) -> bool:
        import re
        import warnings
        if self.maxTileEntries != 0 or not self.device.handle:
            return False
        mine = self._own_overflow(error) or []
        now = max([int(fw.getResources()["maxTileEntries"]) for fw in self._forward_passes()] + [self._grown_tile_entries, 1 << 20])
        new = min(max(2 * now, int(max(mine) * 1.5) if mine else 0), 0xFFFFF000)
        if new <= now:
            return False
        warnings.warn(f"tile-entry lists grown from {now} to {new} entries after an overflow ({error}); the step that overflowed was skipped", RuntimeWarning, stacklevel=3)
        self._grown_tile_entries = new
        self._tickets = []
        try:
            self.device.synchronize()
        except ops.CapacityError:
            pass
        self._invalidate_command_buffers()
        for name in self._OP_NAMES:
            if name != "optimizer" and getattr(self, name) is not None:
                getattr(self, name).destroy()
                setattr(self, name, None)
        self._destroy_more_op_sets()
        self._destroy_more_metric_sets()
        self._gradient_output_applied = None
        self.ensurePipelines(self.lastViewportWidth, self.lastViewportHeight)
        for fw in self._forward_passes():
            fw.setDcSource(self._dc_words)
        return True

    def _step(self, view_ids: Optional[list] = None) -> None:
        if not self.isTraining or self.pointCloud is None:
            return
        stepStart = time.perf_counter()
        n_views = self.world_size * self.views_per_rank
        if view_ids is None:
            view_ids = [self._rng.randrange(len(self.trainCameras)) for _ in range(n_views)]
        mine = parallel.shard_views(view_ids, self.rank, self.world_size)
        image0 = self.images[mine[0]]
        self.ensurePipelines(image0["width"], image0["height"])

        s = self.densifyPruneConfig["schedule"]
        nextIteration = self.iteration + 1
        warmup, interval, stop = s["warmupIterations"], max(1, s["interval"]), s["stopIterations"]
        shouldDensify = s["enabled"] and warmup <= nextIteration <= stop and (nextIteration == warmup or (nextIteration - warmup) % interval == 0)

        try:
            if n_views == 1:
                self._step_single_view(mine[0])
            else:
                self._step_batched(mine)
        except BaseException as orig:
            if self.device.handle:
                self.device.lib.wdgs_encoder_abort(self.device.handle)
            try:
                self._invalidate_command_buffers()
            except ops.CapacityError as deferred:
                raise orig from deferred
            finally:
                self._tickets = []
            raise
        try:
            self._finish_step(n_views)
        except BaseException:
            self._tickets = []
            raise

        self.iteration += 1
        self.stepMs = (time.perf_counter() - stepStart) * 1000.0
        inst = 1000.0 / self.stepMs if self.stepMs > 0 else 0.0
        self.stepItersPerSec = inst if self.stepItersPerSec == 0 else self.stepItersPerSec * 0.9 + inst * 0.1
        if shouldDensify:
            self.drain()
            self._grow_long_lists()
            self.runDensifyPruneMultiView()
            req = self.consumePointCloudSwapRequest()
            if req is not None:
                self.applyPointCloudSwap(req)
        if self.iteration >= self.maxIterations:
            self.stop()
            self.drain()

    def _run(self, key: tuple, encode) -> bool:
        cmd = self._cmd_cache.get(key)
        if cmd is not None:
            self.device.queue.submit([cmd])
            return True
        record = self.use_command_buffers and self._eager_steps >= 1
        with self.device.createCommandEncoder("trainer-" + str(key[0]), record=record) as encoder:
            encode(encoder)
            cmd = encoder.finish()
        if record:
            self._cmd_cache[key] = cmd
        self.device.queue.submit([cmd])
        return False

    def _apply_gradient_output(self) -> None:
        want = bool(self.keep_gradients or not self.fuse_geometry_adam)
        if self._gradient_output_applied is want:
            return
        if self._gradient_output_applied is not None:
            self._invalidate_command_buffers()
        self.backwardPass.setGradientOutput(want)
        self._gradient_output_applied = want

    def _step_single_view(self, view: int) -> None:
        self._apply_gradient_output()
        tileCounts = self.forwardPass.getResources()["tileCountsBuffer"]

        def encode(encoder):
            if self.fuse_geometry_adam:
                self._encode_view(encoder, view, geometry=False)
                self.optimizer.stepWithGeometry(encoder, self.pointCloud, self.backwardPass, self._camera_buffers[view], tileCounts)
            else:
                self._encode_view(encoder, view)
                self.optimizer.step(encoder, self.pointCloud, self.backwardPass.getGradientsBuffer(), tileCounts)
        if self._run(("step", view), encode):
            self.optimizer.advanceIteration(1)
        elif not self.use_command_buffers or self._eager_steps < 1:
            self._eager_steps += 1

    def _step_batched(self, mine: list) -> None:
        n, w = self.pointCloud.num_points, self.world_size
# ... 381 lines not shown
```

Baseline: 1245.

## Disarm long-list machinery when the first eager steps show no long tiles

Adds an armed flag to the forward pass so long-list building in the segment sort, rasterizer and backward can be switched off. The trainer checks long-list stats after the first eager step and disarms it when no tile needs long-list work. The segment sort kernel is templated so the disarmed path compiles out the flag check and long_list_build call. Command buffers record a long-list generation and are rejected if replayed after the state changes, at the cost of extra bookkeeping and a host-side scan of the ranges for stats while disarmed.

```diff
diff --git a/bindings/napi/webdgs_napi.cc b/bindings/napi/webdgs_napi.cc
--- a/bindings/napi/webdgs_napi.cc
+++ b/bindings/napi/webdgs_napi.cc
@@ -289,6 +289,15 @@
     napi_value o; napi_create_object(env, &o);
     for (int i = 0; i < 12; i++) if (keys[i]) set_prop(env, o, keys[i], make_u32(env, st[i]));
     return o;
+}
+static napi_value tiledForwardArmLongLists(napi_env env, napi_callback_info info) {
+    ARGS(2);
+    WDGS_OK_OR_THROW(wdgs_tiled_forward_arm_long_lists((wdgs_tiled_forward*)get_ptr(env, argv[0]), (int)get_u32(env, argv[1])));
+    return js_undefined(env);
+}
+static napi_value tiledForwardLongListsArmed(napi_env env, napi_callback_info info) {
+    ARGS(1);
+    return make_u32(env, (uint32_t)wdgs_tiled_forward_long_lists_armed((wdgs_tiled_forward*)get_ptr(env, argv[0])));
 }
 static napi_value tiledRasterizerBlit(napi_env env, napi_callback_info info) {
     ARGS(4);
@@ -862,7 +871,7 @@
     EXPORT_FN(tiledRasterizerCreate); EXPORT_FN(tiledRasterizerEncode); EXPORT_FN(tiledRasterizerGet); EXPORT_FN(tiledRasterizerDestroy);
     EXPORT_FN(tiledBackwardCreate); EXPORT_FN(tiledBackwardEncode); EXPORT_FN(tiledBackwardGradients); EXPORT_FN(tiledBackwardDestroy);
     EXPORT_FN(optimizerCreate); EXPORT_FN(optimizerStep); EXPORT_FN(optimizerGetIteration); EXPORT_FN(optimizerDestroy);
-    EXPORT_FN(tiledForwardSet); EXPORT_FN(tiledForwardCheck); EXPORT_FN(tiledForwardSetLongLists); EXPORT_FN(tiledForwardLongListStats); EXPORT_FN(tiledRasterizerBlit); EXPORT_FN(bufferClear);
+    EXPORT_FN(tiledForwardSet); EXPORT_FN(tiledForwardCheck); EXPORT_FN(tiledForwardSetLongLists); EXPORT_FN(tiledForwardLongListStats); EXPORT_FN(tiledForwardArmLongLists); EXPORT_FN(tiledForwardLongListsArmed); EXPORT_FN(tiledRasterizerBlit); EXPORT_FN(bufferClear);
     EXPORT_FN(tiledRasterizerEncodeDepth); EXPORT_FN(tiledRasterizerGetDepth); EXPORT_FN(depthToRgba8);
     EXPORT_FN(encoderBegin); EXPORT_FN(encoderFinish); EXPORT_FN(queueSubmit); EXPORT_FN(commandBufferDestroy); EXPORT_FN(queueOnSubmittedWorkDone);
     EXPORT_FN(tiledBackwardMetric); EXPORT_FN(tiledBackwardGet); EXPORT_FN(downsampleRGBA8); EXPORT_FN(imageSSE); EXPORT_FN(imageSSIM);
diff --git a/include/webdgs.h b/include/webdgs.h
--- a/include/webdgs.h
+++ b/include/webdgs.h
@@ -126,6 +126,8 @@
 int wdgs_tiled_forward_check(wdgs_tiled_forward* op, uint32_t* stats_out);
 int wdgs_tiled_forward_set_long_lists(wdgs_tiled_forward* op, uint32_t threshold, uint32_t max_items, uint32_t max_rows);
 int wdgs_tiled_forward_long_list_stats(wdgs_tiled_forward* op, uint32_t stats_out[12]);
+int wdgs_tiled_forward_arm_long_lists(wdgs_tiled_forward* op, int armed);
+int wdgs_tiled_forward_long_lists_armed(wdgs_tiled_forward* op);
 
 int wdgs_tiled_rasterizer_create(wdgs_device* dev, wdgs_tiled_forward* forward, uint32_t compat_caps, wdgs_tiled_rasterizer** out);
 int wdgs_tiled_rasterizer_destroy(wdgs_tiled_rasterizer* op);
diff --git a/webdgs_amd/_lib.py b/webdgs_amd/_lib.py
--- a/webdgs_amd/_lib.py
+++ b/webdgs_amd/_lib.py
@@ -183,6 +183,8 @@
     "wdgs_tiled_forward_check": (_I, [_P, C.POINTER(_U)]),
     "wdgs_tiled_forward_set_long_lists": (_I, [_P, _U, _U, _U]),
     "wdgs_tiled_forward_long_list_stats": (_I, [_P, C.POINTER(_U)]),
+    "wdgs_tiled_forward_arm_long_lists": (_I, [_P, _I]),
+    "wdgs_tiled_forward_long_lists_armed": (_I, [_P]),
     "wdgs_tiled_rasterizer_create": (_I, [_P, _P, _U, C.POINTER(_P)]),
     "wdgs_tiled_rasterizer_destroy": (_I, [_P]),
     "wdgs_tiled_rasterizer_encode": (_I, [_P, _U, _U]),
diff --git a/webdgs_amd/csrc/api.hip b/webdgs_amd/csrc/api.hip
--- a/webdgs_amd/csrc/api.hip
+++ b/webdgs_amd/csrc/api.hip
@@ -168,6 +168,8 @@
     u32 nf_capacity;
     LongWork long_lists;
     u32 long_flags_capacity;
+    bool long_armed;
+    u32 long_generation;
     u32* host_stats;
     u32* splats;
     u32* depths;
@@ -471,7 +473,11 @@
 
 static bool forward_holds_projection(const wdgs_tiled_forward* f);
 static void forward_consume_projection(wdgs_tiled_forward* f);
-struct wdgs_command_buffer_impl { hipGraph_t graph; hipGraphExec_t exec; std::vector<wdgs_tiled_forward*> consumes; wdgs_device* dev; };
+static u32 forward_long_generation(const wdgs_tiled_forward* f);
+struct wdgs_command_buffer_impl {
+    hipGraph_t graph; hipGraphExec_t exec; std::vector<wdgs_tiled_forward*> consumes; wdgs_device* dev;
+    std::vector<std::pair<wdgs_tiled_forward*, u32>> long_states;
+};
 static void command_buffer_release(wdgs_command_buffer_impl* c) {
     (void)hipGraphExecDestroy(c->exec);
     (void)hipGraphDestroy(c->graph);
@@ -490,6 +496,7 @@
     WDGS_CHECK_HIP(hipStreamBeginCapture(d->stream, hipStreamCaptureModeRelaxed));
     d->capturing = true;
     d->capture_consumes.clear();
+    d->capture_long_states.clear();
     return WDGS_OK;
 }
 int wdgs_encoder_finish(wdgs_device* d, wdgs_command_buffer** out) {
@@ -500,9 +507,10 @@
     WDGS_CHECK_HIP(hipStreamEndCapture(d->stream, &graph));
     hipGraphExec_t exec = nullptr;
     hipError_t e = hipGraphInstantiate(&exec, graph, nullptr, nullptr, 0);
-    if (e != hipSuccess) { (void)hipGraphDestroy(graph); d->capture_consumes.clear(); wdgs_set_error("hipGraphInstantiate failed: %s", hipGetErrorString(e)); return WDGS_E_HIP; }
-    auto* c = new wdgs_command_buffer_impl{graph, exec, std::move(d->capture_consumes), d};
+    if (e != hipSuccess) { (void)hipGraphDestroy(graph); d->capture_consumes.clear(); d->capture_long_states.clear(); wdgs_set_error("hipGraphInstantiate failed: %s", hipGetErrorString(e)); return WDGS_E_HIP; }
+    auto* c = new wdgs_command_buffer_impl{graph, exec, std::move(d->capture_consumes), d, std::move(d->capture_long_states)};
     d->capture_consumes.clear();
+    d->capture_long_states.clear();
     *out = reinterpret_cast<wdgs_command_buffer*>(c);
     return WDGS_OK;
 }
@@ -511,6 +519,7 @@
     if (!d->capturing) return WDGS_OK;
     d->capturing = false;
     d->capture_consumes.clear();
+    d->capture_long_states.clear();
     hipGraph_t graph = nullptr;
     const hipError_t e = hipStreamEndCapture(d->stream, &graph);
     if (graph) (void)hipGraphDestroy(graph);
@@ -529,6 +538,10 @@
                      "wdgs_queue_submit: the command buffer starts at the scan of a projected forward pass (wdgs_tiled_forward_encode_projected), but the pass holds no "
                      "projection: run wdgs_tiled_forward_project_views before every submit, and no other encode of the pass in between");
     }
+    for (const auto& ls : c->long_states)
+        WDGS_REQUIRE(std::find(d->forwards.begin(), d->forwards.end(), ls.first) == d->forwards.end() || forward_long_generation(ls.first) == ls.second, WDGS_E_STATE,
+                     "wdgs_queue_submit: the command buffer was recorded in another long-list state of its forward pass (wdgs_tiled_forward_arm_long_lists / "
+                     "wdgs_tiled_forward_set_long_lists since): record it again");
     WDGS_CHECK_HIP(hipGraphLaunch(c->exec, d->stream));
     for (wdgs_tiled_forward* f : c->consumes) forward_consume_projection(f);
     reap_command_buffers(d, 1);
@@ -719,6 +732,18 @@
     return WDGS_OK;
 }
 
+static u32 forward_long_generation(const wdgs_tiled_forward* f) { return f->long_generation; }
+static u32 next_long_generation() { static u32 next = 0u; return ++next; }
+static const LongWork* forward_long_work(wdgs_tiled_forward* f) {
+    wdgs_device* d = f->dev;
+    if (d->capturing) {
+        auto& v = d->capture_long_states;
+        const std::pair<wdgs_tiled_forward*, u32> now{f, f->long_generation};
+        if (std::find(v.begin(), v.end(), now) == v.end()) v.push_back(now);
+    }
+    return (f->long_lists.hdr && f->long_armed) ? &f->long_lists : nullptr;
+}
+
 static void forward_free_long_lists(wdgs_tiled_forward* op) {
     LongWork& lw = op->long_lists;
     free_dev(lw.hdr);
@@ -729,6 +754,7 @@
 static int forward_alloc_long_lists(wdgs_tiled_forward* op, u32 threshold, u32 items, u32 rows) {
     wdgs_device* d = op->dev;
     forward_free_long_lists(op);
+    op->long_generation = next_long_generation();
     if (threshold == 0u) return WDGS_OK;
     LongWork lw{};
     lw.threshold = threshold;
@@ -772,6 +798,8 @@
     op->nf_capacity = 0;
     op->long_lists = LongWork{};
     op->long_flags_capacity = 0;
+    op->long_armed = true;
+    op->long_generation = next_long_generation();
     op->host_stats = nullptr;
     op->scanner = nullptr;
     op->sorter = nullptr;
@@ -873,7 +901,8 @@
     wdgs_device* d = op->dev;
     const u32 n = op->cfg.num_points;
     const TileInfo& ti = op->tile_info;
-    const ScanStatsEpilogue ep{op->stats, op->stats + 4, op->host_stats, op->tile_info.max_tile_entries, op->stats + FRAME_WORD, op->long_lists.hdr};
+    const LongWork* const lw = forward_long_work(op);
+    const ScanStatsEpilogue ep{op->stats, op->stats + 4, op->host_stats, op->tile_info.max_tile_entries, op->stats + FRAME_WORD, lw ? lw->hdr : nullptr};
     if (columns) {
         WDGS_TRY(forward_scan(d, op->block_counts, ceil_div(n, 256), op->column_counts, op->column_totals, ti.num_tiles_x, ep));
     } else if (n > 0) {
@@ -898,7 +927,7 @@
     if (columns) {
         WDGS_TRY(launch_emit_scatter(d, n, op->splats, op->depths, op->scanner->input, op->scanner->output, op->block_counts, op->settings, op->tile_info,
                                      op->column_counts, op->column_totals, wdgs_sorter_keys(op->sorter, 0), wdgs_sorter_values(op->sorter, 0), op->tile_info.max_tile_entries));
-        WDGS_TRY(sorter_sort_rows(op->sorter, ti.num_tiles_x, ti.num_tiles_y, op->ranges, op->long_lists.hdr ? &op->long_lists : nullptr));
+        WDGS_TRY(sorter_sort_rows(op->sorter, ti.num_tiles_x, ti.num_tiles_y, op->ranges, lw));
         op->ranges_valid = true;
     } else {
         WDGS_TRY(launch_emit(d, n, op->splats, op->depths, op->scanner->input, op->scanner->output, op->block_counts, op->settings, op->tile_info,
@@ -908,7 +937,7 @@
             if (op->cfg.compat_caps) {
                 WDGS_TRY(wdgs_sorter_sort(op->sorter, 32u));
             } else {
-                WDGS_TRY(sorter_sort_segmented(op->sorter, bits_for(op->tile_info.total_tiles), op->tile_info.total_tiles, op->ranges, op->long_lists.hdr ? &op->long_lists : nullptr));
+                WDGS_TRY(sorter_sort_segmented(op->sorter, bits_for(op->tile_info.total_tiles), op->tile_info.total_tiles, op->ranges, lw));
                 op->ranges_valid = true;
             }
         }
@@ -1040,12 +1069,35 @@
     const LongWork& now = op->long_lists;
     return forward_alloc_long_lists(op, threshold, max_items ? max_items : (now.hdr ? now.max_items : LONG_LIST_ITEMS), max_rows ? max_rows : (now.hdr ? now.max_rows : LONG_LIST_ROWS));
 }
+int wdgs_tiled_forward_arm_long_lists(wdgs_tiled_forward* op, int armed) {
+    WDGS_REQUIRE(op, WDGS_E_INVALID, "wdgs_tiled_forward_arm_long_lists: null op");
+    WDGS_REQUIRE(!op->dev->capturing, WDGS_E_STATE, "wdgs_tiled_forward_arm_long_lists while recording a command buffer");
+    if (op->long_armed == (armed != 0)) return WDGS_OK;
+    op->long_armed = armed != 0;
+    op->long_generation = next_long_generation();
+    return WDGS_OK;
+}
+int wdgs_tiled_forward_long_lists_armed(wdgs_tiled_forward* op) { return (op && op->long_armed) ? 1 : 0; }
 int wdgs_tiled_forward_long_list_stats(wdgs_tiled_forward* op, uint32_t stats_out[12]) {
     WDGS_REQUIRE(op && stats_out, WDGS_E_INVALID, "wdgs_tiled_forward_long_list_stats: null argument");
     std::memset(stats_out, 0, sizeof(uint32_t) * 12);
     const LongWork& lw = op->long_lists;
     if (!lw.hdr) return WDGS_OK;
-    WDGS_TRY(wdgs_copy_to_host(op->dev, stats_out, lw.hdr, sizeof(u32) * LL_HDR_WORDS));
+    if (op->long_armed) {
+        WDGS_TRY(wdgs_copy_to_host(op->dev, stats_out, lw.hdr, sizeof(u32) * LL_HDR_WORDS));
+    } else if (lw.threshold && op->ranges_valid && op->ranges) {
+        const u32 tiles = op->tile_info.total_tiles;
+        std::vector<u32> r((size_t)tiles + 1u);
+        WDGS_TRY(wdgs_copy_to_host(op->dev, r.data(), op->ranges, sizeof(u32) * r.size()));
+        u32 end = r[tiles];
+        for (u32 t = tiles; t-- > 0u;) {
+            const u32 start = r[t];
+            if (start == 0xFFFFFFFFu) continue;
+            const u32 n = end > start ? end - start : 0u;
+            if (n > lw.threshold) { stats_out[LL_BLOCKS] += 4u; stats_out[LL_ITEMS] += 4u * ((n + 63u) >> 6); }
+            end = start;
+        }
+    }
     stats_out[8] = lw.max_items; stats_out[9] = lw.max_blocks; stats_out[10] = lw.max_rows; stats_out[11] = lw.threshold;
     return WDGS_OK;
 }
@@ -1110,7 +1162,7 @@
     }
     WDGS_TRY(launch_rasterize(d, f->settings, ti, f->splats, f->cfg.num_points, op->ranges_used, keys, vals, f->stats, op->compat_caps ? 32u : 0u, op->rgba8,
                               op->alpha, op->n_contrib, f->nf_stamp, f->stats + FRAME_WORD,
-                              (f->ranges_valid && f->long_lists.hdr && !op->compat_caps) ? &f->long_lists : nullptr));
+                              (f->ranges_valid && !op->compat_caps) ? forward_long_work(f) : nullptr));
     op->encoded = true;
     return WDGS_OK;
 }
@@ -1271,7 +1323,7 @@
     else WDGS_TRY(launch_acc_clear_if_dirty(d, op->acc, n, op->acc_dirty));
     const LongWork* lw = nullptr;
     auto owner = d->range_tables.find(res->tile_offsets_buffer);
-    if (owner != d->range_tables.end() && owner->second->ranges_valid && owner->second->long_lists.hdr) lw = &owner->second->long_lists;
+    if (owner != d->range_tables.end() && owner->second->ranges_valid) lw = forward_long_work(owner->second);
     return launch_backward_rasterize(d, op->settings, ceil_div(w, 16), ceil_div(h, 16), res->tile_offsets_buffer, res->tile_indices_buffer, res->splat_buffer,
                                      res->alpha_texture, res->n_contrib_texture, op->loss_image, op->acc, op->acc_dirty, lw);
 }
diff --git a/webdgs_amd/csrc/common.h b/webdgs_amd/csrc/common.h
--- a/webdgs_amd/csrc/common.h
+++ b/webdgs_amd/csrc/common.h
@@ -5,6 +5,7 @@
 #include <cstdio>
 #include <map>
 #include <string>
+#include <utility>
 #include <vector>
 
 #include "../../include/webdgs.h"
@@ -58,6 +59,7 @@
     std::vector<wdgs_tiled_forward*> forwards;
     std::map<const void*, wdgs_tiled_forward*> range_tables;
     std::vector<wdgs_tiled_forward*> capture_consumes;
+    std::vector<std::pair<wdgs_tiled_forward*, u32>> capture_long_states;
     std::vector<void*> dead_command_buffers;
     int num_cus = 256;
     double* ssim_partials = nullptr;
diff --git a/webdgs_amd/csrc/longlist.h b/webdgs_amd/csrc/longlist.h
--- a/webdgs_amd/csrc/longlist.h
+++ b/webdgs_amd/csrc/longlist.h
@@ -64,4 +64,7 @@
     return t < n_tasks ? t : 0xFFFFFFFFu;
 }
 WD_DEV u32 ll_batch(u32 n_tasks) { return min(max(n_tasks >> 11, 1u), 8u); }
+template <bool ON> struct LongArg { LongWork w; };
+template <> struct LongArg<false> {};
+
 WD_DEV bool ll_frame_on(const LongWork& lw, u32 blocks_wanted, u32 items_wanted) { return blocks_wanted != 0u && blocks_wanted <= lw.max_blocks && items_wanted <= lw.max_items; }
diff --git a/webdgs_amd/csrc/sort.hip b/webdgs_amd/csrc/sort.hip
--- a/webdgs_amd/csrc/sort.hip
+++ b/webdgs_amd/csrc/sort.hip
@@ -463,8 +463,9 @@
     if (threadIdx.x == 0u && ok) lw.flags[t] = 0xFu;
 }
 
+template <bool LONG>
 __global__ __launch_bounds__(SEG_THREADS, 6) void segment_sort_kernel(u32* __restrict__ cur_k, u32* __restrict__ cur_v, u32* __restrict__ alt_k,
-                                                                    u32* __restrict__ alt_v, const u32* __restrict__ ranges, u32 total_tiles, LongWork lw) {
+                                                                    u32* __restrict__ alt_v, const u32* __restrict__ ranges, u32 total_tiles, LongArg<LONG> la) {
     __shared__ u32 a_k[SEG_CAP], a_v[SEG_CAP];
     __shared__ seg_hist_t whist[SEG_THREADS / 64][SEG_BINS];
     __shared__ u32 s_base[RADIX];
@@ -475,7 +476,7 @@
     u32 end = ranges[t + 1u];
     if (start == 0xFFFFFFFFu) return;
     for (u32 nx = t + 1u; end == 0xFFFFFFFFu && nx < total_tiles;) { nx++; end = ranges[nx]; }
-    if (lw.flags) long_list_build(lw, t, (end != 0xFFFFFFFFu && end > start) ? end - start : 0u);
+    if constexpr (LONG) long_list_build(la.w, t, (end != 0xFFFFFFFFu && end > start) ? end - start : 0u);
     if (end <= start + 1u || end == 0xFFFFFFFFu) return;
     const u32 n = end - start;
     if (n <= SEG_CAP) {
@@ -629,9 +630,12 @@
     }
     if (passes != 2u)
         WDGS_LAUNCH(dev, "tile_ranges", tile_ranges_kernel, dim3(ceil_div(num_segments + 1, 4)), dim3(256), 0, s->keys[src], s->count_ptr, num_segments, ranges);
-    if (num_segments > 0)
-        WDGS_LAUNCH(dev, "sort_segments", segment_sort_kernel, dim3(num_segments), dim3(SEG_THREADS), 0, s->keys[src], s->vals[src], s->keys[src ^ 1],
-                    s->vals[src ^ 1], ranges, num_segments, lw ? *lw : LongWork{});
+    if (num_segments > 0) {
+        if (lw && lw->flags) WDGS_LAUNCH(dev, "sort_segments", segment_sort_kernel<true>, dim3(num_segments), dim3(SEG_THREADS), 0, s->keys[src], s->vals[src], s->keys[src ^ 1],
+                                         s->vals[src ^ 1], ranges, num_segments, LongArg<true>{*lw});
+        else WDGS_LAUNCH(dev, "sort_segments", segment_sort_kernel<false>, dim3(num_segments), dim3(SEG_THREADS), 0, s->keys[src], s->vals[src], s->keys[src ^ 1],
+                         s->vals[src ^ 1], ranges, num_segments, LongArg<false>{});
+    }
     WDGS_CHECK_HIP(hipGetLastError());
     s->final_out_index = src;
     return WDGS_OK;
@@ -658,7 +662,8 @@
         WDGS_LAUNCH(dev, "sort_scatter", sort_scatter_kernel<SORT_ITEMS_MAX>, dim3(s->num_parts), dim3(SORT_THREADS), 0, s->keys[0], s->vals[0], s->keys[1], s->vals[1], s->count_ptr, rows,
                     s->num_parts, s->counts, s->totals, ranges, 2u, tiles);
     }
-    WDGS_LAUNCH(dev, "sort_segments", segment_sort_kernel, dim3(tiles), dim3(SEG_THREADS), 0, s->keys[1], s->vals[1], s->keys[0], s->vals[0], ranges, tiles, lw ? *lw : LongWork{});
+    if (lw && lw->flags) WDGS_LAUNCH(dev, "sort_segments", segment_sort_kernel<true>, dim3(tiles), dim3(SEG_THREADS), 0, s->keys[1], s->vals[1], s->keys[0], s->vals[0], ranges, tiles, LongArg<true>{*lw});
+    else WDGS_LAUNCH(dev, "sort_segments", segment_sort_kernel<false>, dim3(tiles), dim3(SEG_THREADS), 0, s->keys[1], s->vals[1], s->keys[0], s->vals[0], ranges, tiles, LongArg<false>{});
     WDGS_CHECK_HIP(hipGetLastError());
     s->final_out_index = 1;
     return WDGS_OK;
diff --git a/webdgs_amd/ops.py b/webdgs_amd/ops.py
--- a/webdgs_amd/ops.py
+++ b/webdgs_amd/ops.py
@@ -412,6 +412,13 @@
 
     def setLongLists(self, threshold: int, maxItems: int = 0, maxRows: int = 0) -> None:
         check(self.device.lib.wdgs_tiled_forward_set_long_lists(self.handle, int(threshold), int(maxItems), int(maxRows)))
+
+    def armLongLists(self, armed: bool) -> None:
+        check(self.device.lib.wdgs_tiled_forward_arm_long_lists(self.handle, 1 if armed else 0))
+
+    @property
+    def longListsArmed(self) -> bool:
+        return bool(self.device.lib.wdgs_tiled_forward_long_lists_armed(self.handle))
 
     def longListStats(self) -> dict:
         st = (C.c_uint32 * 12)()
diff --git a/webdgs_amd/trainer.py b/webdgs_amd/trainer.py
--- a/webdgs_amd/trainer.py
+++ b/webdgs_amd/trainer.py
@@ -31,6 +31,7 @@
         self.use_command_buffers = bool(use_command_buffers)
         self._cmd_cache: dict = {}
         self._eager_steps = 0
+        self._long_lists_chosen = False
         if overlap_views is None:
             overlap_views = int(os.environ.get("WDGS_LANES", self.DEFAULT_LANES))
         elif isinstance(overlap_views, bool):
@@ -180,6 +181,7 @@
             c.destroy()
         self._cmd_cache = {}
         self._eager_steps = 0
+        self._long_lists_chosen = False
         if deferred is not None:
             raise deferred
 
@@ -305,6 +307,14 @@
         self._invalidate_command_buffers()
         for fw in self._forward_passes():
             fw.setLongLists(int(self.longLists.get("threshold", 2048)), self.longLists["maxItems"], self.longLists["maxRows"])
+
+    def _choose_long_lists(self) -> None:
+        if self._long_lists_chosen or self._eager_steps < 1:
+            return
+        self._long_lists_chosen = True
+        for fw in self._forward_passes():
+            st = fw.longListStats()
+            fw.armLongLists(bool(st["threshold"] and st["blocksWanted"]))
 
     def ensurePipelines(self, width: int, height: int) -> None:
         if (max(1, int(width)), max(1, int(height))) != (self.lastViewportWidth, self.lastViewportHeight):
@@ -461,6 +471,7 @@
         mine = parallel.shard_views(view_ids, self.rank, self.world_size)
         image0 = self.images[mine[0]]
         self.ensurePipelines(image0["width"], image0["height"])
+        self._choose_long_lists()
 
         s = self.densifyPruneConfig["schedule"]
         nextIteration = self.iteration + 1
```

Result: no change. 1246 (median of 3 runs) (+0.1%).
